# Urist-McDeveloper/nbody

Measured on AMD Instinct MI355X. Metric: particle-pair interactions/sec at N=2^20, higher is better.
Workload: dtype f32

## Files before the change

nbody_amd/__init__.py:

```python
import ctypes as C
import os

import numpy as np

PKG_DIR = os.path.dirname(os.path.abspath(__file__))
ROOT = os.path.dirname(PKG_DIR)
LIB_DIR = os.path.join(PKG_DIR, "lib")
HIP_SO = os.environ.get("NBODY_HIP_SO") or os.path.join(LIB_DIR, "libnbody_hip.so")
NBODY_SO = os.path.join(LIB_DIR, "libnbody.so")



def _nb_g_from_header():
    import re
    with open(os.path.join(ROOT, "include", "nbody.h")) as f:
        return float(re.search(r"^#define\s+NB_G\s+([0-9.eE+-]+)f?\s*$", f.read(), re.M).group(1))


NB_G = _nb_g_from_header()
UNIQUE_ID_BYTES = 128
CLOCK_SAMPLER_MAX_MS = 20000.0


class WorldData(C.Structure):
    _fields_ = [("total_len", C.c_uint32), ("mass_len", C.c_uint32), ("dt", C.c_float)]


class WorldEnergy(C.Structure):
    _fields_ = [("kinetic", C.c_double), ("potential", C.c_double), ("mass", C.c_double), ("momentum", C.c_double * 2),
                ("angular_momentum", C.c_double), ("center_of_mass", C.c_double * 2)]

    def as_dict(self):
        return {"kinetic": self.kinetic, "potential": self.potential, "total": self.kinetic + self.potential,
                "mass": self.mass, "momentum": (self.momentum[0], self.momentum[1]),
                "angular_momentum": self.angular_momentum,
                "center_of_mass": (self.center_of_mass[0], self.center_of_mass[1])}


def energy_row(row):
    e = WorldEnergy()
    C.memmove(C.byref(e), np.ascontiguousarray(row, dtype=np.float64).ctypes.data, C.sizeof(WorldEnergy))
    return e.as_dict()


def trace_rows(n, every):
    return int(hip_lib().nb_hip_ensemble_trace_rows(int(n), int(every)))


class RenderView(C.Structure):
    _fields_ = [("target", C.c_float * 2), ("offset", C.c_float * 2), ("zoom", C.c_float), ("width", C.c_uint32),
                ("height", C.c_uint32), ("core_mass", C.c_float)]

    @classmethod
    def make(cls, target, offset, zoom, width, height, core_mass):
        return cls((C.c_float * 2)(*target), (C.c_float * 2)(*offset), zoom, width, height, core_mass)

    def as_dict(self):
        return {"target": (self.target[0], self.target[1]), "offset": (self.offset[0], self.offset[1]), "zoom": self.zoom,
                "width": self.width, "height": self.height, "core_mass": self.core_mass}


class RenderPalette(C.Structure):
    _fields_ = [("background", C.c_uint8 * 4), ("color", (C.c_uint8 * 4) * 3), ("saturation", C.c_uint32)]

    @classmethod
    def make(cls, background, color, saturation):
        return cls((C.c_uint8 * 4)(*background), ((C.c_uint8 * 4) * 3)(*[(C.c_uint8 * 4)(*c) for c in color]), saturation)


def default_palette():
    p = RenderPalette()
    nbody_lib().DefaultRenderPalette(C.byref(p))
    return p


class NbAdaptive(C.Structure):
    _fields_ = [("eta", C.c_float), ("dt_min", C.c_float), ("dt_max", C.c_float), ("flags", C.c_uint32), ("span", C.c_double),
                ("chunk", C.c_uint32), ("reserved", C.c_uint32)]


class NbAdaptiveResult(C.Structure):
    _fields_ = [("elapsed", C.c_double), ("steps", C.c_uint32), ("idle_steps", C.c_uint32), ("dt_last", C.c_float),
                ("dt_smallest", C.c_float)]

    def as_dict(self):
        return {"elapsed": self.elapsed, "steps": int(self.steps), "idle_steps": int(self.idle_steps), "dt_last": self.dt_last,
                "dt_smallest": self.dt_smallest}


NB_ADAPT_PRIME = 1
NB_ADAPT_CONTINUE = 2
NB_ADAPT_LEAPFROG = 4


def adaptive_cfg(eta, dt_max, dt_min=0.0, span=float("inf"), prime=False, chunk=0, resume=False, leapfrog=False):
    flags = (NB_ADAPT_PRIME if prime else 0) | (NB_ADAPT_CONTINUE if resume else 0) | (NB_ADAPT_LEAPFROG if leapfrog else 0)
    return NbAdaptive(float(eta), float(dt_min), float(dt_max), flags, float(span), int(chunk), 0)


class NbShardPlan(C.Structure):
    _fields_ = [(n, C.c_uint32) for n in ("mass_chunk", "zero_chunk", "mass_begin", "mass_count",
                                          "zero_begin", "zero_count", "src_padded")]


ALLGATHER_FN = C.CFUNCTYPE(None, C.c_void_p, C.c_void_p, C.c_uint64, C.c_int, C.c_int)

HIP_API = {
    "CreateSimPipeline": (C.c_void_p, [WorldData]),
    "DestroySimPipeline": (None, [C.c_void_p]),
    "GetSimulationData": (None, [C.c_void_p, C.c_void_p]),
    "SetSimulationData": (None, [C.c_void_p, C.c_void_p]),
    "PerformSimUpdate": (None, [C.c_void_p, C.c_uint32, C.c_float]),
    "nb_hip_device_count": (C.c_int, []),
    "nb_hip_set_device": (None, [C.c_int]),
    "nb_hip_device_info": (None, [C.c_char_p, C.c_uint32]),
    "nb_hip_step_async": (None, [C.c_void_p, C.c_uint32, C.c_float]),
    "nb_hip_sync": (None, [C.c_void_p]),
    "nb_hip_last_step_ms": (C.c_double, [C.c_void_p, C.POINTER(C.c_uint32)]),
    "nb_hip_last_finish_launches": (C.c_uint32, [C.c_void_p]),
    "nb_hip_last_step_breakdown": (C.c_uint32, [C.c_void_p, C.POINTER(C.c_double), C.POINTER(C.c_double)]),
    "nb_hip_comm_info": (C.c_int, [C.c_void_p, C.POINTER(C.c_int), C.POINTER(C.c_int), C.POINTER(C.c_int),
                                   C.POINTER(C.c_int), C.POINTER(C.c_double), C.c_char_p, C.c_uint32]),
    "nb_hip_comm_bringup": (C.c_int, [C.c_void_p, C.POINTER(C.c_double), C.POINTER(C.c_double), C.POINTER(C.c_double)]),
    "nb_hip_preflight_peers": (C.c_int, [C.POINTER(C.c_int), C.c_int]),
    "nb_hip_preflight_ipc_export": (C.c_int, [C.c_void_p, C.c_uint32]),
    "nb_hip_preflight_ipc_open": (C.c_int, [C.c_void_p, C.c_uint32, C.POINTER(C.c_double)]),
    "nb_hip_preflight_ipc_release": (None, []),
    "nb_hip_error_string": (C.c_char_p, [C.c_int]),
    "nb_hip_graph_stats": (C.c_uint32, [C.c_void_p, C.POINTER(C.c_uint32)]),
    "nb_hip_runtime_version": (C.c_int, []),
    "nb_hip_probe_clock": (C.c_int, [C.c_double] + [C.POINTER(C.c_double)] * 5),
    "nb_hip_clock_sampler_begin": (C.c_int, [C.c_double, C.c_double]),
    "nb_hip_clock_sampler_end": (C.c_int, [C.POINTER(C.c_double)] * 6 + [C.POINTER(C.c_uint32)]),
    "nb_hip_note_host_array": (None, [C.c_void_p, C.c_void_p, C.c_uint64]),
    "nb_hip_configure": (C.c_int, [C.c_void_p, C.c_char_p, C.c_int]),
    "nb_hip_launch_shape": (None, [C.c_void_p, C.POINTER(C.c_int), C.POINTER(C.c_int), C.POINTER(C.c_int),
                                   C.POINTER(C.c_int), C.POINTER(C.c_uint32)]),
    "nb_hip_plan_launch": (None, [C.c_uint32, C.c_uint32, C.c_int, C.POINTER(C.c_int), C.POINTER(C.c_int),
                                  C.POINTER(C.c_int), C.POINTER(C.c_uint32)]),
    "nb_hip_comm_unique_id": (None, [C.c_void_p]),
    "CreateSimPipelineSharded": (C.c_void_p, [WorldData, C.c_int, C.c_int, C.c_void_p]),
    "CreateSimPipelineShardedWith": (C.c_void_p, [WorldData, C.c_int, C.c_int, ALLGATHER_FN, C.c_void_p]),
    "CreateSimPipelineShardedDirect": (C.c_void_p, [WorldData, C.c_int, C.c_int, ALLGATHER_FN, C.c_void_p]),
    "nb_hip_shard_plan": (NbShardPlan, [C.c_uint32, C.c_uint32, C.c_int, C.c_int]),
    "nb_hip_local_group_create": (C.c_int, [WorldData, C.c_int, C.POINTER(C.c_void_p)]),
    "nb_hip_local_group_step": (None, [C.POINTER(C.c_void_p), C.c_int, C.c_uint32, C.c_float]),
    "nb_hip_energy": (None, [C.c_void_p, C.POINTER(WorldEnergy)]),
    "nb_hip_potential": (None, [C.c_void_p, C.c_void_p]),
    "nb_hip_bounds": (None, [C.c_void_p, C.c_void_p]),
    "nb_hip_render_counts": (None, [C.c_void_p, C.POINTER(RenderView), C.c_void_p]),
    "nb_hip_render_rgba": (None, [C.c_void_p, C.POINTER(RenderView), C.POINTER(RenderPalette), C.c_void_p]),
    "nb_hip_potential_at": (None, [C.c_void_p, C.c_void_p, C.c_uint32, C.c_float, C.c_void_p]),
    "nb_hip_potential_map": (None, [C.c_void_p, C.POINTER(RenderView), C.c_float, C.c_void_p]),
    "nb_hip_acceleration_at": (None, [C.c_void_p, C.c_void_p, C.c_uint32, C.c_float, C.c_void_p]),
    "nb_hip_acceleration_map": (None, [C.c_void_p, C.POINTER(RenderView), C.c_float, C.c_void_p]),
    "nb_hip_batch_create": (C.c_void_p, [C.c_uint32, C.c_uint32, C.POINTER(C.c_uint32)]),
    "nb_hip_batch_destroy": (None, [C.c_void_p]),
    "nb_hip_batch_set_data": (None, [C.c_void_p, C.c_void_p]),
    "nb_hip_batch_get_data": (None, [C.c_void_p, C.c_void_p]),
    "nb_hip_batch_get_member": (None, [C.c_void_p, C.c_uint32, C.c_void_p]),
    "nb_hip_batch_update": (None, [C.c_void_p, C.c_uint32, C.c_float]),
    "nb_hip_batch_update_dts": (None, [C.c_void_p, C.c_uint32, C.POINTER(C.c_float)]),
    "nb_hip_batch_step_async": (None, [C.c_void_p, C.c_uint32, C.POINTER(C.c_float)]),
    "nb_hip_batch_sync": (None, [C.c_void_p]),
    "nb_hip_batch_last_ms": (C.c_double, [C.c_void_p]),
    "nb_hip_batch_dt_uploads": (C.c_uint32, [C.c_void_p]),
    "nb_hip_batch_launch_shape": (None, [C.c_void_p, C.POINTER(C.c_int), C.POINTER(C.c_int), C.POINTER(C.c_int),
                                         C.POINTER(C.c_int), C.POINTER(C.c_uint32)]),
    "nb_hip_ensemble_energy": (None, [C.c_void_p, C.POINTER(WorldEnergy)]),
    "nb_hip_ensemble_potential": (None, [C.c_void_p, C.c_void_p]),
    "nb_hip_ensemble_trace_rows": (C.c_uint32, [C.c_uint32, C.c_uint32]),
    "nb_hip_ensemble_trace": (None, [C.c_void_p, C.c_uint32, C.c_float, C.c_uint32, C.c_void_p]),
    "nb_hip_ensemble_trace_dts": (None, [C.c_void_p, C.c_uint32, C.POINTER(C.c_float), C.c_uint32, C.c_void_p]),
    "nb_hip_ensemble_bounds": (None, [C.c_void_p, C.c_void_p]),
    "nb_hip_ensemble_render_counts": (None, [C.c_void_p, C.POINTER(RenderView), C.c_void_p]),
    "nb_hip_ensemble_render_rgba": (None, [C.c_void_p, C.POINTER(RenderView), C.POINTER(RenderPalette), C.c_void_p]),
    "nb_hip_ragged_create": (C.c_void_p, [C.c_uint32, C.POINTER(C.c_uint32), C.POINTER(C.c_uint32)]),
    "nb_hip_ragged_layout": (None, [C.c_void_p, C.POINTER(C.c_uint32), C.POINTER(C.c_uint64)]),
    "nb_hip_ragged_launch_shape": (C.c_uint32, [C.c_void_p, C.c_uint32, C.POINTER(C.c_int), C.POINTER(C.c_int), C.POINTER(C.c_int),
                                                C.POINTER(C.c_int), C.POINTER(C.c_uint32), C.POINTER(C.c_uint32)]),
    "nb_hip_ragged_member_shape": (None, [C.c_void_p, C.c_uint32, C.POINTER(C.c_uint32), C.POINTER(C.c_int), C.POINTER(C.c_int),
                                          C.POINTER(C.c_int)]),
    "nb_hip_ensemble_potential_at": (None, [C.c_void_p, C.c_void_p, C.c_uint32, C.c_float, C.c_void_p]),
    "nb_hip_ensemble_potential_map": (None, [C.c_void_p, C.POINTER(RenderView), C.c_float, C.c_void_p]),
    "nb_hip_ensemble_acceleration_at": (None, [C.c_void_p, C.c_void_p, C.c_uint32, C.c_float, C.c_void_p]),
    "nb_hip_ensemble_acceleration_map": (None, [C.c_void_p, C.POINTER(RenderView), C.c_float, C.c_void_p]),
    "nb_hip_adaptive_steps": (None, [C.c_void_p, C.c_uint32, C.POINTER(NbAdaptive), C.c_void_p, C.POINTER(NbAdaptiveResult)]),
    "nb_hip_adaptive_steps_async": (None, [C.c_void_p, C.c_uint32, C.POINTER(NbAdaptive)]),
    "nb_hip_adaptive_collect": (None, [C.c_void_p, C.c_void_p, C.POINTER(NbAdaptiveResult)]),
    "nb_hip_timestep": (None, [C.c_void_p, C.POINTER(NbAdaptive), C.POINTER(C.c_float)]),
    "nb_hip_ensemble_adaptive_steps": (None, [C.c_void_p, C.c_uint32, C.POINTER(NbAdaptive), C.c_void_p, C.c_void_p]),
    "nb_hip_leapfrog_steps": (None, [C.c_void_p, C.c_uint32, C.c_float]),
    "nb_hip_leapfrog_steps_async": (None, [C.c_void_p, C.c_uint32, C.c_float]),
    "nb_hip_ensemble_leapfrog": (None, [C.c_void_p, C.c_uint32, C.c_float]),
    "nb_hip_ensemble_leapfrog_dts": (None, [C.c_void_p, C.c_uint32, C.POINTER(C.c_float)]),
    "nb_hip_version": (C.c_int, []),
}

TUNE_API = {
    "nb_hip_tune": (C.c_int, [C.c_void_p, C.c_char_p, C.c_int]),
    "nb_hip_tuning_build": (C.c_int, []),
    "nb_hip_launch_unit": (C.c_int, [C.c_void_p]),
    "nb_hip_last_fused_steps": (C.c_uint32, [C.c_void_p]),
    "nb_hip_launch_lanes": (C.c_int, [C.c_void_p]),
    "nb_hip_plan_launch_unit": (C.c_int, [C.c_uint32, C.c_uint32, C.c_int]),
    "nb_hip_plan_fused_finish": (C.c_int, [C.c_uint32, C.c_uint32, C.c_int]),
    "nb_hip_plan_launch_lanes": (C.c_int, [C.c_uint32, C.c_uint32, C.POINTER(C.c_int)]),
    "nb_hip_last_diag_ms": (C.c_double, [C.c_void_p]),
    "nb_hip_last_render_ms": (C.c_double, [C.c_void_p, C.POINTER(C.c_double)]),
    "nb_hip_ensemble_last_diag_ms": (C.c_double, [C.c_void_p]),
    "nb_hip_ensemble_trace_mode": (None, [C.c_void_p, C.c_int]),
    "nb_hip_ensemble_last_trace_info": (None, [C.c_void_p, C.POINTER(C.c_int), C.POINTER(C.c_uint32)]),
    "nb_hip_ensemble_render_mode": (None, [C.c_void_p, C.c_int]),
    "nb_hip_ensemble_last_render_info": (None, [C.c_void_p, C.POINTER(C.c_int), C.POINTER(C.c_uint32)]),
    "nb_hip_ensemble_last_render_ms": (C.c_double, [C.c_void_p]),
    "nb_hip_last_leapfrog_info": (None, [C.c_void_p, C.POINTER(C.c_uint32), C.POINTER(C.c_int)]),
    "nb_hip_ensemble_last_leapfrog_info": (None, [C.c_void_p, C.POINTER(C.c_uint32), C.POINTER(C.c_int)]),
    "nb_hip_live_resources": (None, [C.POINTER(C.c_uint32), C.POINTER(C.c_uint32)]),
}
PUBLIC_KNOBS = ("variant", "graph", "timing", "overlap", "sharded_graph")

NBODY_API = {
    "CreateWorld": (C.c_void_p, [C.c_void_p, C.c_uint32]),
    "DestroyWorld": (None, [C.c_void_p]),
    "GetWorldParticles": (C.c_void_p, [C.c_void_p, C.POINTER(C.c_uint32)]),
    "UpdateWorld_CPU": (None, [C.c_void_p, C.c_float, C.c_uint32]),
    "UpdateWorld_GPU": (None, [C.c_void_p, C.c_float, C.c_uint32]),
    "CreateWorldSharded": (C.c_void_p, [C.c_void_p, C.c_uint32, C.c_int, C.c_int, C.c_void_p]),
    "CreateWorldShardedWith": (C.c_void_p, [C.c_void_p, C.c_uint32, C.c_int, C.c_int, ALLGATHER_FN, C.c_void_p]),
    "CreateWorldShardedDirect": (C.c_void_p, [C.c_void_p, C.c_uint32, C.c_int, C.c_int, ALLGATHER_FN, C.c_void_p]),
    "GetWorldPipeline": (C.c_void_p, [C.c_void_p]),
    "MakeGalaxies": (C.c_void_p, [C.c_uint32, C.c_uint32]),
    "MakeGalaxiesSeeded": (C.c_void_p, [C.c_uint32, C.c_uint32, C.c_uint64]),
    "GetWorldEnergy": (None, [C.c_void_p, C.POINTER(WorldEnergy)]),
    "GetWorldPotential": (None, [C.c_void_p, C.c_void_p]),
    "DefaultRenderPalette": (None, [C.POINTER(RenderPalette)]),
    "GetWorldBounds": (None, [C.c_void_p, C.c_void_p]),
    "FitWorldView": (None, [C.c_void_p, C.c_uint32, C.c_uint32, C.POINTER(RenderView)]),
    "RenderWorldCounts": (None, [C.c_void_p, C.POINTER(RenderView), C.c_void_p]),
    "RenderWorld": (None, [C.c_void_p, C.POINTER(RenderView), C.POINTER(RenderPalette), C.c_void_p]),
    "GetWorldPotentialAt": (None, [C.c_void_p, C.c_void_p, C.c_uint32, C.c_float, C.c_void_p]),
    "RenderWorldPotential": (None, [C.c_void_p, C.POINTER(RenderView), C.c_float, C.c_void_p]),
    "GetWorldAccelerationAt": (None, [C.c_void_p, C.c_void_p, C.c_uint32, C.c_float, C.c_void_p]),
    "RenderWorldAcceleration": (None, [C.c_void_p, C.POINTER(RenderView), C.c_float, C.c_void_p]),
    "CreateWorldBatch": (C.c_void_p, [C.c_void_p, C.c_uint32, C.c_uint32]),
    "DestroyWorldBatch": (None, [C.c_void_p]),
    "GetWorldBatchParticles": (C.c_void_p, [C.c_void_p, C.c_uint32, C.POINTER(C.c_uint32)]),
    "UpdateWorldBatch_GPU": (None, [C.c_void_p, C.c_float, C.c_uint32]),
    "UpdateWorldBatch_GPU_dts": (None, [C.c_void_p, C.POINTER(C.c_float), C.c_uint32]),
    "GetWorldBatchEnergy": (None, [C.c_void_p, C.POINTER(WorldEnergy)]),
    "GetWorldBatchPotential": (None, [C.c_void_p, C.c_void_p]),
    "UpdateWorldBatch_GPU_Traced": (None, [C.c_void_p, C.c_float, C.c_uint32, C.c_uint32, C.c_void_p]),
    "UpdateWorldBatch_GPU_Traced_dts": (None, [C.c_void_p, C.POINTER(C.c_float), C.c_uint32, C.c_uint32, C.c_void_p]),
    "GetWorldBatchBounds": (None, [C.c_void_p, C.c_void_p]),
    "FitWorldBatchViews": (None, [C.c_void_p, C.c_uint32, C.c_uint32, C.POINTER(RenderView)]),
    "RenderWorldBatchCounts": (None, [C.c_void_p, C.POINTER(RenderView), C.c_void_p]),
    "RenderWorldBatch": (None, [C.c_void_p, C.POINTER(RenderView), C.POINTER(RenderPalette), C.c_void_p]),
    "CreateWorldBatchRagged": (C.c_void_p, [C.c_void_p, C.POINTER(C.c_uint32), C.c_uint32]),
    "GetWorldBatchPotentialAt": (None, [C.c_void_p, C.c_void_p, C.c_uint32, C.c_float, C.c_void_p]),
    "RenderWorldBatchPotential": (None, [C.c_void_p, C.POINTER(RenderView), C.c_float, C.c_void_p]),
    "GetWorldBatchAccelerationAt": (None, [C.c_void_p, C.c_void_p, C.c_uint32, C.c_float, C.c_void_p]),
    "RenderWorldBatchAcceleration": (None, [C.c_void_p, C.POINTER(RenderView), C.c_float, C.c_void_p]),
    "UpdateWorld_GPU_Adaptive": (None, [C.c_void_p, C.c_uint32, C.POINTER(NbAdaptive), C.c_void_p, C.POINTER(NbAdaptiveResult)]),
    "UpdateWorld_CPU_Adaptive": (None, [C.c_void_p, C.c_uint32, C.POINTER(NbAdaptive), C.c_void_p, C.POINTER(NbAdaptiveResult)]),
    "GetWorldTimestep": (None, [C.c_void_p, C.POINTER(NbAdaptive), C.POINTER(C.c_float)]),
    "AdvanceWorld_GPU": (None, [C.c_void_p, C.c_double, C.POINTER(NbAdaptive), C.c_uint32, C.c_void_p, C.POINTER(NbAdaptiveResult)]),
    "UpdateWorldBatch_GPU_Adaptive": (None, [C.c_void_p, C.c_uint32, C.POINTER(NbAdaptive), C.c_void_p, C.c_void_p]),
    "AdvanceWorldBatch_GPU": (None, [C.c_void_p, C.c_double, C.POINTER(NbAdaptive), C.c_uint32, C.c_void_p, C.c_void_p]),
    "UpdateWorld_GPU_Leapfrog": (None, [C.c_void_p, C.c_float, C.c_uint32]),
    "UpdateWorld_CPU_Leapfrog": (None, [C.c_void_p, C.c_float, C.c_uint32]),
    "UpdateWorldBatch_GPU_Leapfrog": (None, [C.c_void_p, C.c_float, C.c_uint32]),
    "UpdateWorldBatch_GPU_Leapfrog_dts": (None, [C.c_void_p, C.POINTER(C.c_float), C.c_uint32]),
}

_hip = None
_nbody = None


def _bind(lib, api):
    for name, (res, args) in api.items():
        f = getattr(lib, name)
        f.restype = res
        f.argtypes = args
    return lib


def _build_if_missing(path):
    if os.path.exists(path) or os.environ.get("NBODY_HIP_SO"):
        return
    import sys
    from . import build as _build
    print(f"[nbody_amd] {path} missing: building the product libraries (hipcc, gfx950)", file=sys.stderr, flush=True)
    _build.build_product()


def hip_lib():
    global _hip
    if _hip is None:
        _build_if_missing(HIP_SO)
        if not os.path.exists(HIP_SO):
            raise OSError(f"{HIP_SO} not built: run `python -c 'import __graft_entry__ as g; g.build()'`")
        _hip = _bind(_bind(C.CDLL(HIP_SO, mode=C.RTLD_GLOBAL), HIP_API), TUNE_API)
    return _hip


def nbody_lib():
    global _nbody
    if _nbody is None:
        hip_lib()
        _build_if_missing(NBODY_SO)
        if not os.path.exists(NBODY_SO):
            raise OSError(f"{NBODY_SO} not built: run `python -c 'import __graft_entry__ as g; g.build()'`")
        _nbody = _bind(C.CDLL(NBODY_SO, mode=C.RTLD_GLOBAL), NBODY_API)
    return _nbody


def as_particles(a):
    a = np.ascontiguousarray(a, dtype=np.float32)
    if a.ndim != 2 or a.shape[1] != 8:
        raise ValueError("particles must have shape (n, 8)")
    return a


def as_points(points):
    a = np.ascontiguousarray(points, dtype=np.float32)
    if a.ndim != 2 or a.shape[1] != 2:
        raise ValueError("points must have shape (n, 2)")
    return a


def device_count():
    return int(hip_lib().nb_hip_device_count())


def live_resources():
    buffers, events = C.c_uint32(0), C.c_uint32(0)
    hip_lib().nb_hip_live_resources(C.byref(buffers), C.byref(events))
    return int(buffers.value), int(events.value)


def device_info():
    buf = C.create_string_buffer(256)
    hip_lib().nb_hip_device_info(buf, 256)
    return buf.value.decode()


def probe_clock(target_ms=40.0):
    v = [C.c_double(0.0) for _ in range(5)]
    waves = hip_lib().nb_hip_probe_clock(float(target_ms), *[C.byref(x) for x in v])
    return {"clock_ghz": v[0].value, "clock_ghz_min": v[1].value, "clock_ghz_max": v[2].value,
            "cycles_per_wave_interaction": v[3].value, "elapsed_ms": v[4].value, "waves": int(waves)}


def clock_sampler_begin(period_ms=0.5, max_ms=6000.0):
    return int(hip_lib().nb_hip_clock_sampler_begin(float(period_ms), float(max_ms)))


def clock_sampler_end():
    ghz, lo, hi, span = C.c_double(), C.c_double(), C.c_double(), C.c_double()
    per_xcd, profile = (C.c_double * 8)(), (C.c_double * 10)()
    dropped = C.c_uint32(0)
    n = hip_lib().nb_hip_clock_sampler_end(C.byref(ghz), C.byref(lo), C.byref(hi), per_xcd, profile, C.byref(span), C.byref(dropped))
    return {"clock_ghz": ghz.value, "clock_ghz_min": lo.value, "clock_ghz_max": hi.value, "per_xcd_ghz": [float(v) for v in per_xcd],
            "profile_ghz": [float(v) for v in profile], "span_ms": span.value, "intervals": int(n), "dropped_intervals": int(dropped.value)}


def preflight_peers(max_devices=16):
    row = (C.c_int * max_devices)()
    count = int(hip_lib().nb_hip_preflight_peers(row, max_devices))
    return count, [int(v) for v in row[:min(count, max_devices)]]


def preflight_ipc_export(tag):
    buf = (C.c_ubyte * 64)()
    rc = int(hip_lib().nb_hip_preflight_ipc_export(buf, int(tag) & 0xffffffff))
    return rc, bytes(buf)


def preflight_ipc_open(handle, expect_tag):
    ms = C.c_double(0.0)
    buf = (C.c_ubyte * 64).from_buffer_copy(handle)
    rc = int(hip_lib().nb_hip_preflight_ipc_open(buf, int(expect_tag) & 0xffffffff, C.byref(ms)))
    return rc, float(ms.value)


def hip_error_string(code):
    return hip_lib().nb_hip_error_string(int(code)).decode(errors="replace")


def shard_plan(total_len, mass_len, rank, nranks):
    p = hip_lib().nb_hip_shard_plan(total_len, mass_len, rank, nranks)
    return {n: int(getattr(p, n)) for n, _ in NbShardPlan._fields_}


def plan_launch(n_recv, n_src, compute_units=256):
    k, w, sp, g, lw = C.c_int(), C.c_int(), C.c_int(), C.c_uint32(), C.c_int()
    hip_lib().nb_hip_plan_launch(n_recv, n_src, compute_units, C.byref(k), C.byref(w), C.byref(sp), C.byref(g))
    lanes = int(hip_lib().nb_hip_plan_launch_lanes(n_recv, n_src, C.byref(lw)))
    return {"k": k.value, "w": w.value, "split": sp.value, "workgroups": g.value,
            "unit": int(hip_lib().nb_hip_plan_launch_unit(n_recv, n_src, compute_units)), "lanes": lanes, "lanes_w": lw.value,
            "fused_finish": int(hip_lib().nb_hip_plan_fused_finish(n_recv, n_src, compute_units))}


def comm_unique_id():
    buf = (C.c_ubyte * UNIQUE_ID_BYTES)()
    hip_lib().nb_hip_comm_unique_id(buf)
    return bytes(buf)


class SimPipeline:

    def __init__(self, total_len, mass_len, rank=0, nranks=1, unique_id=None, allgather=None, direct=False):
        L = hip_lib()
        wd = WorldData(total_len, mass_len, 0.0)
        self._cb = None
        if allgather is not None:
            def thunk(_ctx, buf, bytes_per_rank, r, n):
                try:
                    rows = np.ctypeslib.as_array(C.cast(buf, C.POINTER(C.c_uint8)), shape=(n, int(bytes_per_rank)))
                    allgather(rows, r, n)
                except BaseException:
                    import sys
                    import traceback
                    traceback.print_exc()
                    print(f"[nbody_amd] rank {r} of {n}: the caller-supplied all-gather raised; exiting (5)", file=sys.stderr,
                          flush=True)
                    os._exit(5)
            self._cb = ALLGATHER_FN(thunk)
            create = L.CreateSimPipelineShardedDirect if direct else L.CreateSimPipelineShardedWith
            self._h = create(wd, rank, nranks, self._cb, None)
        elif nranks > 1 or unique_id is not None:
            idbuf = (C.c_ubyte * UNIQUE_ID_BYTES).from_buffer_copy(unique_id)
            self._h = L.CreateSimPipelineSharded(wd, rank, nranks, idbuf)
        else:
            self._h = L.CreateSimPipeline(wd)
        self.total_len, self.mass_len = total_len, mass_len
        self.rank, self.nranks = rank, nranks
        self.configure(timing=1)

    def close(self):
        if self._h:
            hip_lib().DestroySimPipeline(self._h)
            self._h = None

    def __del__(self):
        try:
            self.close()
        except Exception:
            pass

    def set_data(self, particles):
        a = as_particles(particles)
        assert a.shape[0] == self.total_len
        hip_lib().SetSimulationData(self._h, a.ctypes.data)

    def get_data(self):
        out = np.empty((self.total_len, 8), dtype=np.float32)
        hip_lib().GetSimulationData(self._h, out.ctypes.data)
        return out

    def update(self, n, dt):
        hip_lib().PerformSimUpdate(self._h, n, dt)

    def step_async(self, n, dt):
        hip_lib().nb_hip_step_async(self._h, n, dt)

    def update_leapfrog(self, n, dt):
        hip_lib().nb_hip_leapfrog_steps(self._h, n, dt)

    def update_leapfrog_async(self, n, dt):
        hip_lib().nb_hip_leapfrog_steps_async(self._h, n, dt)

    def last_leapfrog_info(self):
        k, primed = C.c_uint32(0), C.c_int(0)
        hip_lib().nb_hip_last_leapfrog_info(self._h, C.byref(k), C.byref(primed))
        return int(k.value), bool(primed.value)

    def update_adaptive(self, n, eta, dt_max, dt_min=0.0, span=float("inf"), prime=False, resume=False, leapfrog=False):
        cfg, res, log = adaptive_cfg(eta, dt_max, dt_min, span, prime, resume=resume, leapfrog=leapfrog), NbAdaptiveResult(), np.zeros(n, dtype=np.float32)
        hip_lib().nb_hip_adaptive_steps(self._h, n, C.byref(cfg), log.ctypes.data, C.byref(res))
        return log, res.as_dict()

    def update_adaptive_async(self, n, eta, dt_max, dt_min=0.0, span=float("inf"), prime=False, resume=False, leapfrog=False):
        cfg = adaptive_cfg(eta, dt_max, dt_min, span, prime, resume=resume, leapfrog=leapfrog)
        hip_lib().nb_hip_adaptive_steps_async(self._h, n, C.byref(cfg))

    def adaptive_collect(self, n):
        res, log = NbAdaptiveResult(), np.zeros(n, dtype=np.float32)
        hip_lib().nb_hip_adaptive_collect(self._h, log.ctypes.data, C.byref(res))
        return log, res.as_dict()

    def timestep(self, eta, dt_max, dt_min=0.0):
        cfg, dt = adaptive_cfg(eta, dt_max, dt_min), C.c_float(0.0)
        hip_lib().nb_hip_timestep(self._h, C.byref(cfg), C.byref(dt))
        return float(dt.value)

    def sync(self):
        hip_lib().nb_hip_sync(self._h)

    def last_step_ms(self):
        launches = C.c_uint32(0)
        ms = hip_lib().nb_hip_last_step_ms(self._h, C.byref(launches))
        return float(ms), int(launches.value)

    def finish_launches(self):
        return int(hip_lib().nb_hip_last_finish_launches(self._h))

    def step_breakdown(self):
        k, c = C.c_double(0.0), C.c_double(0.0)
        steps = hip_lib().nb_hip_last_step_breakdown(self._h, C.byref(k), C.byref(c))
        return int(steps), float(k.value), float(c.value)

    def comm_info(self):
        n, r, d, v, ms = C.c_int(), C.c_int(), C.c_int(), C.c_int(), C.c_double()
        path = C.create_string_buffer(256)
        own = hip_lib().nb_hip_comm_info(self._h, C.byref(n), C.byref(r), C.byref(d), C.byref(v), C.byref(ms), path, 256)
        return {"owns_comm": bool(own), "nranks": n.value, "rank": r.value, "device": d.value, "rccl_version": v.value,
                "first_gather_ms": ms.value, "rccl_lib": path.value.decode()}

    def comm_bringup(self):
        a, b, c = C.c_double(), C.c_double(), C.c_double()
        own = hip_lib().nb_hip_comm_bringup(self._h, C.byref(a), C.byref(b), C.byref(c))
        return {"owns_comm": bool(own), "comm_init_ms": a.value, "first_gather_ms": b.value, "small_gather_us": c.value}

    def graph_stats(self):
        uploads = C.c_uint32(0)
        cached = hip_lib().nb_hip_graph_stats(self._h, C.byref(uploads))
        return {"cached": int(cached), "dt_uploads": int(uploads.value)}

    def energy(self):
        e = WorldEnergy()
        hip_lib().nb_hip_energy(self._h, C.byref(e))
        return e.as_dict()

    def potential(self):
        out = np.empty(self.total_len, dtype=np.float32)
        hip_lib().nb_hip_potential(self._h, out.ctypes.data)
        return out

    def potential_at(self, points, softening):
        pts = as_points(points)
        out = np.empty(pts.shape[0], dtype=np.float32)
        hip_lib().nb_hip_potential_at(self._h, pts.ctypes.data, pts.shape[0], softening, out.ctypes.data)
        return out

    def potential_map(self, view, softening):
        out = np.empty((view.height, view.width), dtype=np.float32)
        hip_lib().nb_hip_potential_map(self._h, C.byref(view), softening, out.ctypes.data)
        return out

    def acceleration_at(self, points, softening):
        pts = as_points(points)
        out = np.empty((pts.shape[0], 2), dtype=np.float32)
        hip_lib().nb_hip_acceleration_at(self._h, pts.ctypes.data, pts.shape[0], softening, out.ctypes.data)
        return out

    def acceleration_map(self, view, softening):
        out = np.empty((view.height, view.width, 2), dtype=np.float32)
        hip_lib().nb_hip_acceleration_map(self._h, C.byref(view), softening, out.ctypes.data)
        return out

    def last_diag_ms(self):
        return float(hip_lib().nb_hip_last_diag_ms(self._h))

    def bounds(self):
        out = np.empty(4, dtype=np.float32)
        hip_lib().nb_hip_bounds(self._h, out.ctypes.data)
        return out

    def render_counts(self, view):
        out = np.empty((3, view.height, view.width), dtype=np.uint32)
        hip_lib().nb_hip_render_counts(self._h, C.byref(view), out.ctypes.data)
        return out

    def render(self, view, palette=None):
        out = np.empty((view.height, view.width, 4), dtype=np.uint8)
        pal = palette if palette is not None else default_palette()
        hip_lib().nb_hip_render_rgba(self._h, C.byref(view), C.byref(pal), out.ctypes.data)
        return out

    def last_render_ms(self):
        parts = (C.c_double * 4)()
        total = hip_lib().nb_hip_last_render_ms(self._h, parts)
        return float(total), [float(v) for v in parts]

    def fused_steps(self):
        return int(hip_lib().nb_hip_last_fused_steps(self._h))

    def configure(self, **knobs):
        for k, v in knobs.items():
            fn = hip_lib().nb_hip_configure if k in PUBLIC_KNOBS else hip_lib().nb_hip_tune
            fn(self._h, k.encode(), int(v))

    def launch_shape(self):
        k, w, v, sp, g = C.c_int(), C.c_int(), C.c_int(), C.c_int(), C.c_uint32()
        hip_lib().nb_hip_launch_shape(self._h, C.byref(k), C.byref(w), C.byref(v), C.byref(sp), C.byref(g))
        return {"k": k.value, "w": w.value, "variant": "smem" if v.value else "lds", "split": sp.value,
                "workgroups": g.value, "unit": int(hip_lib().nb_hip_launch_unit(self._h)),
                "lanes": int(hip_lib().nb_hip_launch_lanes(self._h))}


def as_ensemble(a):
    a = np.ascontiguousarray(a, dtype=np.float32)
    if a.ndim != 3 or a.shape[2] != 8:
        raise ValueError("an ensemble must have shape (members, n, 8)")
    return a


def _packed(members):
    parts = [as_particles(m) for m in members]
    sizes = np.array([p.shape[0] for p in parts], dtype=np.uint32)
    flat = np.concatenate(parts, axis=0) if parts else np.zeros((0, 8), np.float32)
    return np.ascontiguousarray(flat, dtype=np.float32), sizes


def _unpacked(flat, offsets):
    return [flat[int(offsets[b]):int(offsets[b + 1])].copy() for b in range(len(offsets) - 1)]


def _dt_array(dts, count):
    a = np.ascontiguousarray(dts, dtype=np.float32)
    if a.shape != (count,):
        raise ValueError(f"expected {count} step sizes")
    return a


def _member_points(points, count):
    a = np.asarray(points, dtype=np.float32)
    if a.ndim == 2:
        a = np.broadcast_to(a, (count,) + a.shape)
    if a.ndim != 3 or a.shape[0] != count or a.shape[2] != 2:
        raise ValueError(f"points must have shape (n, 2) or ({count}, n, 2)")
    return np.ascontiguousarray(a)


def _ensemble_field(fn, handle, count, components, softening, points=None, views=None):
    tail = (2,) if components == 2 else ()
    if points is not None:
        pts = _member_points(points, count)
        out = np.empty((count, pts.shape[1]) + tail, dtype=np.float32)
        fn(handle, pts.ctypes.data, pts.shape[1], softening, out.ctypes.data)
        return out
    arr, w, h = _view_array(views, count)
    out = np.empty((count, h, w) + tail, dtype=np.float32)
    fn(handle, arr, softening, out.ctypes.data)
    return out


def _view_array(views, count):
    if isinstance(views, RenderView):
        views = [views] * count
    views = list(views)
    if len(views) != count:
        raise ValueError(f"expected one RenderView or {count} of them")
    arr = (RenderView * count)()
    for b, v in enumerate(views):
        C.memmove(C.byref(arr[b]), C.byref(v), C.sizeof(RenderView))
    return arr, int(arr[0].width), int(arr[0].height)


def contact_sheet(frames, columns):
    frames = np.asarray(frames)
    if frames.ndim != 4 or columns < 1:
        raise ValueError("frames must have shape (B, h, w, channels) and columns must be at least 1")
    count, h, w, ch = frames.shape
    rows = -(-count // columns)
    sheet = np.zeros((rows * columns, h, w, ch), dtype=frames.dtype)
    sheet[:count] = frames
    return sheet.reshape(rows, columns, h, w, ch).transpose(0, 2, 1, 3, 4).reshape(rows * h, columns * w, ch)


class SimBatch:

    is_ragged = False

    def __init__(self, total_len, mass_len):
        m = np.ascontiguousarray(mass_len, dtype=np.uint32)
        if m.ndim != 1:
            raise ValueError("mass_len must be a sequence with one entry per member")
        self.count, self.total_len, self.mass_len = int(m.shape[0]), int(total_len), m.copy()
        self._h = hip_lib().nb_hip_batch_create(self.count, self.total_len, m.ctypes.data_as(C.POINTER(C.c_uint32)))

    @classmethod
    def ragged(cls, total_lens, mass_lens):
        n = np.ascontiguousarray(total_lens, dtype=np.uint32)
        m = np.ascontiguousarray(mass_lens, dtype=np.uint32)
        if n.ndim != 1 or m.shape != n.shape:
            raise ValueError("total_lens and mass_lens must be sequences with one entry per member")
        self = cls.__new__(cls)
        self.is_ragged = True
        self.count, self.total_lens, self.mass_len = int(n.shape[0]), n.copy(), m.copy()
        self.total_len = int(n.max()) if n.size else 0
        self._h = hip_lib().nb_hip_ragged_create(self.count, n.ctypes.data_as(C.POINTER(C.c_uint32)),
                                                 m.ctypes.data_as(C.POINTER(C.c_uint32)))
        self.offsets = self.layout()[1]
        return self

    def layout(self):
        sizes, offsets = np.empty(self.count, np.uint32), np.empty(self.count + 1, np.uint64)
        hip_lib().nb_hip_ragged_layout(self._h, sizes.ctypes.data_as(C.POINTER(C.c_uint32)), offsets.ctypes.data_as(C.POINTER(C.c_uint64)))
        return sizes, offsets

    def sizes(self):
        return [int(x) for x in self.layout()[0]]

    def close(self):
        if self._h:
            hip_lib().nb_hip_batch_destroy(self._h)
            self._h = None

    def __del__(self):
        try:
            self.close()
        except Exception:
            pass

    def set_data(self, particles):
        if self.is_ragged:
            flat, sizes = _packed(particles)
            assert np.array_equal(sizes, self.total_lens)
            hip_lib().nb_hip_batch_set_data(self._h, flat.ctypes.data)
            return
        a = as_ensemble(particles)
        assert a.shape[:2] == (self.count, self.total_len)
        hip_lib().nb_hip_batch_set_data(self._h, a.ctypes.data)

    def get_data(self):
        if self.is_ragged:
            flat = np.empty((int(self.offsets[-1]), 8), dtype=np.float32)
            hip_lib().nb_hip_batch_get_data(self._h, flat.ctypes.data)
            return _unpacked(flat, self.offsets)
        out = np.empty((self.count, self.total_len, 8), dtype=np.float32)
        hip_lib().nb_hip_batch_get_data(self._h, out.ctypes.data)
        return out

    def get_member(self, b):
        n = int(self.total_lens[b]) if self.is_ragged and 0 <= int(b) < self.count else self.total_len
        out = np.empty((n, 8), dtype=np.float32)
        hip_lib().nb_hip_batch_get_member(self._h, int(b), out.ctypes.data)
        return out

    def update(self, n, dt):
        if np.ndim(dt) == 0:
            hip_lib().nb_hip_batch_update(self._h, n, float(dt))
        else:
            hip_lib().nb_hip_batch_update_dts(self._h, n, _dt_array(dt, self.count).ctypes.data_as(C.POINTER(C.c_float)))

    def step_async(self, n, dts):
        hip_lib().nb_hip_batch_step_async(self._h, n, _dt_array(dts, self.count).ctypes.data_as(C.POINTER(C.c_float)))

    def update_leapfrog(self, n, dt):
        if np.ndim(dt) == 0:
            hip_lib().nb_hip_ensemble_leapfrog(self._h, n, float(dt))
        else:
            hip_lib().nb_hip_ensemble_leapfrog_dts(self._h, n, _dt_array(dt, self.count).ctypes.data_as(C.POINTER(C.c_float)))

    def last_leapfrog_info(self):
        k, primed = C.c_uint32(0), C.c_int(0)
        hip_lib().nb_hip_ensemble_last_leapfrog_info(self._h, C.byref(k), C.byref(primed))
        return int(k.value), bool(primed.value)

    def update_adaptive(self, n, eta, dt_max, dt_min=0.0, span=float("inf"), prime=False, resume=False, leapfrog=False):
        cfg, res = adaptive_cfg(eta, dt_max, dt_min, span, prime, resume=resume, leapfrog=leapfrog), (NbAdaptiveResult * self.count)()
        log = np.zeros((n, self.count), dtype=np.float32)
        hip_lib().nb_hip_ensemble_adaptive_steps(self._h, n, C.byref(cfg), log.ctypes.data, C.byref(res))
        return log, [r.as_dict() for r in res]

    def sync(self):
        hip_lib().nb_hip_batch_sync(self._h)

    def last_ms(self):
        return float(hip_lib().nb_hip_batch_last_ms(self._h))

    def dt_uploads(self):
        return int(hip_lib().nb_hip_batch_dt_uploads(self._h))

    def trace(self, n, dt, every):
        out = np.empty((trace_rows(n, every), self.count, 8), dtype=np.float64)
        if np.ndim(dt) == 0:
            hip_lib().nb_hip_ensemble_trace(self._h, n, float(dt), every, out.ctypes.data)
        else:
            hip_lib().nb_hip_ensemble_trace_dts(self._h, n, _dt_array(dt, self.count).ctypes.data_as(C.POINTER(C.c_float)), every,
                                             out.ctypes.data)
        return out

    def trace_mode(self, mode):
        hip_lib().nb_hip_ensemble_trace_mode(self._h, int(mode))

    def last_trace_info(self):
        fused, launches = C.c_int(0), C.c_uint32(0)
        hip_lib().nb_hip_ensemble_last_trace_info(self._h, C.byref(fused), C.byref(launches))
        return {"fused": fused.value, "launches": launches.value}

    def energy(self):
        out = (WorldEnergy * self.count)()
        hip_lib().nb_hip_ensemble_energy(self._h, out)
        return [e.as_dict() for e in out]

    def potential(self):
        if self.is_ragged:
            flat = np.empty(int(self.offsets[-1]), dtype=np.float32)
            hip_lib().nb_hip_ensemble_potential(self._h, flat.ctypes.data)
            return _unpacked(flat, self.offsets)
        out = np.empty((self.count, self.total_len), dtype=np.float32)
        hip_lib().nb_hip_ensemble_potential(self._h, out.ctypes.data)
        return out

    def potential_at(self, points, softening):
        return _ensemble_field(hip_lib().nb_hip_ensemble_potential_at, self._h, self.count, 1, softening, points=points)

    def potential_map(self, views, softening):
        return _ensemble_field(hip_lib().nb_hip_ensemble_potential_map, self._h, self.count, 1, softening, views=views)

    def acceleration_at(self, points, softening):
        return _ensemble_field(hip_lib().nb_hip_ensemble_acceleration_at, self._h, self.count, 2, softening, points=points)

    def acceleration_map(self, views, softening):
        return _ensemble_field(hip_lib().nb_hip_ensemble_acceleration_map, self._h, self.count, 2, softening, views=views)

    def last_diag_ms(self):
        return float(hip_lib().nb_hip_ensemble_last_diag_ms(self._h))

    def bounds(self):
        out = np.empty((self.count, 4), dtype=np.float32)
        hip_lib().nb_hip_ensemble_bounds(self._h, out.ctypes.data)
        return out

    def render_counts(self, views):
        arr, w, h = _view_array(views, self.count)
        out = np.empty((self.count, 3, h, w), dtype=np.uint32)
        hip_lib().nb_hip_ensemble_render_counts(self._h, arr, out.ctypes.data)
        return out

    def render(self, views, palette=None):
        arr, w, h = _view_array(views, self.count)
        out = np.empty((self.count, h, w, 4), dtype=np.uint8)
        pal = palette if palette is not None else default_palette()
        hip_lib().nb_hip_ensemble_render_rgba(self._h, arr, C.byref(pal), out.ctypes.data)
        return out

    def render_mode(self, mode):
        hip_lib().nb_hip_ensemble_render_mode(self._h, int(mode))

    def last_render_info(self):
        tile, launches = C.c_int(0), C.c_uint32(0)
        hip_lib().nb_hip_ensemble_last_render_info(self._h, C.byref(tile), C.byref(launches))
        return {"tile_path": tile.value, "launches": launches.value}

    def last_render_ms(self):
        return float(hip_lib().nb_hip_ensemble_last_render_ms(self._h))

    def launch_shape(self):
        path, k, w, lanes, g = C.c_int(), C.c_int(), C.c_int(), C.c_int(), C.c_uint32()
        if self.is_ragged:
            groups, i, total = [], 0, 1
            members = C.c_uint32()
            while i < total:
                total = int(hip_lib().nb_hip_ragged_launch_shape(self._h, i, C.byref(path), C.byref(k), C.byref(w), C.byref(lanes),
                                                                 C.byref(members), C.byref(g)))
                groups.append({"path": "lanes" if path.value else "chain", "k": k.value, "w": w.value, "lanes": lanes.value,
                               "members": members.value, "workgroups": g.value})
                i += 1
            per = []
            grp = C.c_uint32()
            for b in range(self.count):
                hip_lib().nb_hip_ragged_member_shape(self._h, b, C.byref(grp), C.byref(k), C.byref(w), C.byref(lanes))
                per.append((grp.value, k.value, w.value, lanes.value))
            return {"groups": groups, "members": per}
        hip_lib().nb_hip_batch_launch_shape(self._h, C.byref(path), C.byref(k), C.byref(w), C.byref(lanes), C.byref(g))
        return {"path": "lanes" if path.value else "chain", "k": k.value, "w": w.value, "lanes": lanes.value,
                "workgroups": g.value}

    def pinned_knobs(self):
        s = self.launch_shape()
        if s["path"] == "chain":
            return dict(k=s["k"], w=s["w"], split=1, unit=8, fused_chain=0)
        return dict(lanes=s["lanes"], w=s["w"], fused_chain=0)


class WorldBatch:

    is_ragged = False

    def __init__(self, particles):
        a = as_ensemble(particles)
        self.count, self.size = int(a.shape[0]), int(a.shape[1])
        self._h = nbody_lib().CreateWorldBatch(a.ctypes.data, self.size, self.count)

    @classmethod
    def ragged(cls, members):
        flat, sizes = _packed(members)
        self = cls.__new__(cls)
        self.is_ragged = True
        self.count, self._sizes = int(sizes.shape[0]), sizes
        self.size = int(sizes.max()) if sizes.size else 0
        self.offsets = np.concatenate([[0], np.cumsum(sizes, dtype=np.uint64)]).astype(np.uint64)
        self._h = nbody_lib().CreateWorldBatchRagged(flat.ctypes.data, sizes.ctypes.data_as(C.POINTER(C.c_uint32)), self.count)
        return self

    def sizes(self):
        return [int(x) for x in self._sizes] if self.is_ragged else [self.size] * self.count

    def close(self):
        if self._h:
            nbody_lib().DestroyWorldBatch(self._h)
            self._h = None

    def __del__(self):
        try:
            self.close()
        except Exception:
            pass

    def member(self, b):
        n = C.c_uint32(0)
        p = nbody_lib().GetWorldBatchParticles(self._h, int(b), C.byref(n))
        return np.ctypeslib.as_array(C.cast(p, C.POINTER(C.c_float)), shape=(n.value, 8)).copy()

    def particles(self):
        if self.is_ragged:
            return [self.member(b) for b in range(self.count)]
        return np.stack([self.member(b) for b in range(self.count)])

    def update_gpu(self, dt, n):
        if np.ndim(dt) == 0:
            nbody_lib().UpdateWorldBatch_GPU(self._h, float(dt), n)
        else:
            nbody_lib().UpdateWorldBatch_GPU_dts(self._h, _dt_array(dt, self.count).ctypes.data_as(C.POINTER(C.c_float)), n)

    def update_gpu_leapfrog(self, dt, n):
        if np.ndim(dt) == 0:
            nbody_lib().UpdateWorldBatch_GPU_Leapfrog(self._h, float(dt), n)
        else:
            nbody_lib().UpdateWorldBatch_GPU_Leapfrog_dts(self._h, _dt_array(dt, self.count).ctypes.data_as(C.POINTER(C.c_float)), n)

    def update_gpu_adaptive(self, n, eta, dt_max, dt_min=0.0, span=float("inf"), prime=False, leapfrog=False):
        cfg, res = adaptive_cfg(eta, dt_max, dt_min, span, prime, leapfrog=leapfrog), (NbAdaptiveResult * self.count)()
        log = np.zeros((n, self.count), dtype=np.float32)
        nbody_lib().UpdateWorldBatch_GPU_Adaptive(self._h, n, C.byref(cfg), log.ctypes.data, C.byref(res))
        return log, [r.as_dict() for r in res]

    def advance_gpu(self, span, eta, dt_max, dt_min=0.0, prime=False, chunk=0, max_steps=4096, leapfrog=False):
        cfg, res = adaptive_cfg(eta, dt_max, dt_min, prime=prime, chunk=chunk, leapfrog=leapfrog), (NbAdaptiveResult * self.count)()
        log = np.zeros((max_steps, self.count), dtype=np.float32)
        nbody_lib().AdvanceWorldBatch_GPU(self._h, float(span), C.byref(cfg), max_steps, log.ctypes.data, C.byref(res))
        made = max((r.steps + r.idle_steps for r in res), default=0)
        return log[:made].copy(), [r.as_dict() for r in res]

    def update_gpu_traced(self, dt, n, every):
        out = np.empty((trace_rows(n, every), self.count, 8), dtype=np.float64)
        if np.ndim(dt) == 0:
            nbody_lib().UpdateWorldBatch_GPU_Traced(self._h, float(dt), n, every, out.ctypes.data)
        else:
            nbody_lib().UpdateWorldBatch_GPU_Traced_dts(self._h, _dt_array(dt, self.count).ctypes.data_as(C.POINTER(C.c_float)), n,
                                                        every, out.ctypes.data)
        return out

    def energy(self):
        out = (WorldEnergy * self.count)()
        nbody_lib().GetWorldBatchEnergy(self._h, out)
        return [e.as_dict() for e in out]

    def potential(self):
        if self.is_ragged:
            flat = np.empty(int(self.offsets[-1]), dtype=np.float32)
            nbody_lib().GetWorldBatchPotential(self._h, flat.ctypes.data)
            return _unpacked(flat, self.offsets)
        out = np.empty((self.count, self.size), dtype=np.float32)
        nbody_lib().GetWorldBatchPotential(self._h, out.ctypes.data)
        return out

    def potential_at(self, points, softening):
        return _ensemble_field(nbody_lib().GetWorldBatchPotentialAt, self._h, self.count, 1, softening, points=points)

    def potential_map(self, views, softening):
        return _ensemble_field(nbody_lib().RenderWorldBatchPotential, self._h, self.count, 1, softening, views=views)

    def acceleration_at(self, points, softening):
        return _ensemble_field(nbody_lib().GetWorldBatchAccelerationAt, self._h, self.count, 2, softening, points=points)

    def acceleration_map(self, views, softening):
        return _ensemble_field(nbody_lib().RenderWorldBatchAcceleration, self._h, self.count, 2, softening, views=views)

    def bounds(self):
        out = np.empty((self.count, 4), dtype=np.float32)
        nbody_lib().GetWorldBatchBounds(self._h, out.ctypes.data)
        return out

    def fit_views(self, width, height):
        arr = (RenderView * self.count)()
        nbody_lib().FitWorldBatchViews(self._h, width, height, arr)
        return [RenderView.from_buffer_copy(v) for v in arr]

    def render_counts(self, views):
        arr, w, h = _view_array(views, self.count)
        out = np.empty((self.count, 3, h, w), dtype=np.uint32)
        nbody_lib().RenderWorldBatchCounts(self._h, arr, out.ctypes.data)
        return out

    def render(self, views, palette=None):
        arr, w, h = _view_array(views, self.count)
        out = np.empty((self.count, h, w, 4), dtype=np.uint8)
        nbody_lib().RenderWorldBatch(self._h, arr, C.byref(palette) if palette is not None else None, out.ctypes.data)
        return out


class LocalShardGroup:

    def __init__(self, total_len, mass_len, nranks, **knobs):
        L = hip_lib()
        self.nranks = nranks
        self._arr = (C.c_void_p * nranks)()
        L.nb_hip_local_group_create(WorldData(total_len, mass_len, 0.0), nranks, self._arr)
        self.members = []
        for r in range(nranks):
            m = SimPipeline.__new__(SimPipeline)
            m._h = self._arr[r]
            m.total_len, m.mass_len, m.rank, m.nranks = total_len, mass_len, r, nranks
            m.configure(timing=1, **knobs)
            self.members.append(m)

    def set_data(self, particles):
        for m in self.members:
            m.set_data(particles)

    def step(self, n, dt):
        hip_lib().nb_hip_local_group_step(self._arr, self.nranks, n, dt)

    def get_data(self, rank=0):
        return self.members[rank].get_data()

    def close(self):
        for m in self.members:
            m.close()
        self.members = []


class World:

    def __init__(self, particles, rank=None, nranks=1, unique_id=None):
        a = as_particles(particles)
        self.size = a.shape[0]
        if rank is None:
            self._h = nbody_lib().CreateWorld(a.ctypes.data, self.size)
        else:
            idbuf = (C.c_ubyte * UNIQUE_ID_BYTES).from_buffer_copy(unique_id) if unique_id is not None else None
            self._h = nbody_lib().CreateWorldSharded(a.ctypes.data, self.size, rank, nranks, idbuf)

    def close(self):
        if self._h:
            nbody_lib().DestroyWorld(self._h)
            self._h = None

    def __del__(self):
        try:
            self.close()
        except Exception:
            pass

    def particles(self):
        n = C.c_uint32(0)
        p = nbody_lib().GetWorldParticles(self._h, C.byref(n))
        if n.value == 0:
            return np.empty((0, 8), dtype=np.float32)
        return np.ctypeslib.as_array(C.cast(p, C.POINTER(C.c_float)), shape=(n.value, 8)).copy()

    def pipeline(self):
        return nbody_lib().GetWorldPipeline(self._h)

    def tune(self, **knobs):
        old = {}
        for k, v in knobs.items():
            fn = hip_lib().nb_hip_configure if k in PUBLIC_KNOBS else hip_lib().nb_hip_tune
            old[k] = int(fn(self.pipeline(), k.encode(), int(v)))
        return old

    def update_cpu(self, dt, n):
        nbody_lib().UpdateWorld_CPU(self._h, dt, n)

    def update_gpu(self, dt, n):
        nbody_lib().UpdateWorld_GPU(self._h, dt, n)

    def _adaptive(self, fn, n, cfg):
        res, log = NbAdaptiveResult(), np.zeros(n, dtype=np.float32)
        fn(self._h, n, C.byref(cfg), log.ctypes.data, C.byref(res))
        return log, res.as_dict()

    def update_gpu_leapfrog(self, dt, n):
        nbody_lib().UpdateWorld_GPU_Leapfrog(self._h, dt, n)

    def update_cpu_leapfrog(self, dt, n):
        nbody_lib().UpdateWorld_CPU_Leapfrog(self._h, dt, n)

    def update_gpu_adaptive(self, n, eta, dt_max, dt_min=0.0, span=float("inf"), prime=False, leapfrog=False):
        return self._adaptive(nbody_lib().UpdateWorld_GPU_Adaptive, n, adaptive_cfg(eta, dt_max, dt_min, span, prime, leapfrog=leapfrog))

    def update_cpu_adaptive(self, n, eta, dt_max, dt_min=0.0, span=float("inf"), prime=False, leapfrog=False):
        return self._adaptive(nbody_lib().UpdateWorld_CPU_Adaptive, n, adaptive_cfg(eta, dt_max, dt_min, span, prime, leapfrog=leapfrog))

    def timestep(self, eta, dt_max, dt_min=0.0):
        cfg, dt = adaptive_cfg(eta, dt_max, dt_min), C.c_float(0.0)
        nbody_lib().GetWorldTimestep(self._h, C.byref(cfg), C.byref(dt))
        return float(dt.value)

    def advance_gpu(self, span, eta, dt_max, dt_min=0.0, prime=False, chunk=0, max_steps=4096, leapfrog=False):
        cfg, res = adaptive_cfg(eta, dt_max, dt_min, prime=prime, chunk=chunk, leapfrog=leapfrog), NbAdaptiveResult()
        log = np.zeros(max_steps, dtype=np.float32)
        nbody_lib().AdvanceWorld_GPU(self._h, float(span), C.byref(cfg), max_steps, log.ctypes.data, C.byref(res))
        return log[:res.steps + res.idle_steps].copy(), res.as_dict()

    def energy(self):
        e = WorldEnergy()
        nbody_lib().GetWorldEnergy(self._h, C.byref(e))
        return e.as_dict()

    def potential(self):
        out = np.empty(self.size, dtype=np.float32)
        nbody_lib().GetWorldPotential(self._h, out.ctypes.data)
        return out

    def potential_at(self, points, softening):
        pts = as_points(points)
        out = np.empty(pts.shape[0], dtype=np.float32)
        nbody_lib().GetWorldPotentialAt(self._h, pts.ctypes.data, pts.shape[0], softening, out.ctypes.data)
        return out

    def potential_map(self, view, softening):
        out = np.empty((view.height, view.width), dtype=np.float32)
        nbody_lib().RenderWorldPotential(self._h, C.byref(view), softening, out.ctypes.data)
        return out

    def acceleration_at(self, points, softening):
        pts = as_points(points)
        out = np.empty((pts.shape[0], 2), dtype=np.float32)
        nbody_lib().GetWorldAccelerationAt(self._h, pts.ctypes.data, pts.shape[0], softening, out.ctypes.data)
        return out

    def acceleration_map(self, view, softening):
        out = np.empty((view.height, view.width, 2), dtype=np.float32)
        nbody_lib().RenderWorldAcceleration(self._h, C.byref(view), softening, out.ctypes.data)
        return out

    def bounds(self):
        out = np.empty(4, dtype=np.float32)
        nbody_lib().GetWorldBounds(self._h, out.ctypes.data)
        return out

    def fit_view(self, width, height):
        v = RenderView()
        nbody_lib().FitWorldView(self._h, width, height, C.byref(v))
        return v

    def render_counts(self, view):
        out = np.empty((3, view.height, view.width), dtype=np.uint32)
        nbody_lib().RenderWorldCounts(self._h, C.byref(view), out.ctypes.data)
        return out

    def render(self, view, palette=None):
        out = np.empty((view.height, view.width, 4), dtype=np.uint8)
        nbody_lib().RenderWorld(self._h, C.byref(view), C.byref(palette) if palette is not None else None, out.ctypes.data)
        return out


_cpu_best = None


def cpu_best_lib():
    global _cpu_best
    if _cpu_best is None:
        path = os.path.join(LIB_DIR, "libnbody_cpu_best.so")
        _build_if_missing(path)
        lib = C.CDLL(path)
        lib.nb_cpu_variant_count.restype = C.c_int
        lib.nb_cpu_variant_name.restype = C.c_char_p
        lib.nb_cpu_variant_name.argtypes = [C.c_int, C.POINTER(C.c_int), C.POINTER(C.c_char_p)]
        lib.nb_cpu_variant_update.restype = C.c_int
        lib.nb_cpu_variant_update.argtypes = [C.c_char_p, C.c_void_p, C.c_uint32, C.c_uint32, C.c_float, C.c_uint32]
        _cpu_best = lib
    return _cpu_best


def cpu_variants():
    lib, out = cpu_best_lib(), []
    for i in range(lib.nb_cpu_variant_count()):
        ok, what = C.c_int(0), C.c_char_p()
        name = lib.nb_cpu_variant_name(i, C.byref(ok), C.byref(what))
        out.append((name.decode(), bool(ok.value), what.value.decode()))
    return out


def cpu_variant_update(isa, particles, mass_len, dt, n=1):
    a = as_particles(particles).copy()
    if cpu_best_lib().nb_cpu_variant_update(isa.encode(), a.ctypes.data, a.shape[0], mass_len, dt, n) != 0:
        raise RuntimeError(f"CPU variant {isa!r} is unknown or not supported by this CPU")
    return a


def make_galaxies(particle_count, galaxy_count, seed=None, own_rng=False):
    L = nbody_lib()
    libc = C.CDLL(None)
    libc.free.argtypes = [C.c_void_p]
    if own_rng:
        p = L.MakeGalaxiesSeeded(particle_count, galaxy_count, int(seed))
    else:
        if seed is not None:
            libc.srand(C.c_uint(seed))
        p = L.MakeGalaxies(particle_count, galaxy_count)
    a = np.ctypeslib.as_array(C.cast(p, C.POINTER(C.c_float)), shape=(particle_count, 8)).copy()
    libc.free(p)
    return a
```

nbody_amd/csrc/kernels.h:

```cpp
#pragma once

#include <hip/hip_runtime.h>
#include <stdint.h>

namespace nb {

enum : uint32_t {
    STEP_ACC_IN = 1u,
    STEP_NO_FINALIZE = 2u,
};

enum : int {
    VARIANT_LDS = 0,
    VARIANT_SMEM = 1,
};

struct StepParams {
    const float2 *src_pos;
    const float *src_gm;
    uint32_t src_begin[2];
    uint32_t src_end[2];
    const float2 *pos_in;
    float2 *pos_out;
    float2 *vel;
    float2 *acc;
    const float *radius;
    uint32_t n_recv;
    uint32_t recv_split;
    uint32_t recv_gap;
    float2 *mirror;
    uint32_t n_mirror;
    const float *dt;
    uint32_t flags;
    float2 *parts;
    uint32_t split;
    uint32_t *tickets;
    uint32_t unit;
};

__host__ __device__ inline StepParams plain_step(const float2 *src_pos, const float *src_gm, uint32_t n_src, const float2 *pos_in,
                                                 float2 *pos_out, float2 *vel, float2 *acc, const float *radius, uint32_t n_recv,
                                                 const float *dt, uint32_t unit) {
    return StepParams{.src_pos = src_pos, .src_gm = src_gm, .src_begin = {0, 0}, .src_end = {n_src, 0}, .pos_in = pos_in,
                      .pos_out = pos_out, .vel = vel, .acc = acc, .radius = radius, .n_recv = n_recv, .recv_split = n_recv,
                      .dt = dt, .split = 1, .unit = unit};
}

struct ChainParams {
    float2 *pos;
    float2 *vel;
    float2 *acc;
    const float *radius;
    const float *src_gm;
    uint32_t n_recv;
    uint32_t n_src;
    uint32_t steps;
    uint32_t tiles;
    const float *dt;
};

constexpr uint32_t CHAIN_K = 2;
constexpr uint32_t CHAIN_MAX_RECV = 512;

struct BatchParams {
    float2 *pos_in;
    float2 *pos_out;
    float2 *vel;
    float2 *acc;
    const float *radius;
    const float *gm;
    const uint32_t *mass_len;
    const float *dt;
    uint32_t n_recv;
    uint32_t stride;
    uint32_t steps;
    uint32_t tiles;
};

struct RaggedParams : BatchParams {
    const uint32_t *n_len;
    const uint32_t *members;
};

struct TraceParams {
    const float *mass;
    double *rows;
    uint32_t count;
    uint32_t every;
    uint32_t done;
};

constexpr int MAX_SPLIT = 16;

struct LaunchShape;

const void *step_kernel_fn(LaunchShape s);
const void *step_kernel_fused_fn(LaunchShape s);
const void *finish_kernel_fn();

void launch_chain(hipStream_t st, const ChainParams &p);

const void *batch_lane_split_fn(int w, int lanes, bool listed);
void launch_batch_chain(hipStream_t st, const RaggedParams &p, uint32_t workgroups);
void launch_batch_trace_chain(hipStream_t st, const RaggedParams &p, const TraceParams &t, uint32_t workgroups);

}
```

nbody_amd/csrc/kernels.hip:

```cpp
#include "kernels.h"
#include "diag_common.h"
#include "interaction_asm.h"
#include "launch_shape.h"

#include <hip/hip_runtime.h>

#include <type_traits>

namespace nb {
namespace {

constexpr int WAVE = 64;
constexpr int CHUNK = 64;
constexpr int CLOSE_EVERY = 4;

typedef float v16f __attribute__((ext_vector_type(16)));
typedef float v8f __attribute__((ext_vector_type(8)));
typedef float v4f __attribute__((ext_vector_type(4)));

typedef float f2v __attribute__((ext_vector_type(2)));

template <int K>
struct Receivers {
    f2v p[K];
    float r[K];
    f2v a[K];
    f2v s[K];
    f2v c[K];
    __device__ __forceinline__ void clear() {
#pragma unroll
        for (int k = 0; k < K; k++) a[k] = s[k] = c[k] = f2v{0.0f, 0.0f};
    }
    __device__ __forceinline__ void close_chunk() {
#pragma unroll
        for (int k = 0; k < K; k++) {
            const f2v y = a[k] - c[k];
            const f2v t = s[k] + y;
            const f2v cn = (t - s[k]) - y;
            const bool lx = a[k].x != 0.0f, ly = a[k].y != 0.0f;
            const bool fx = __builtin_fabsf(t.x) < __builtin_inff(), fy = __builtin_fabsf(t.y) < __builtin_inff();
            c[k].x = lx ? (fx ? cn.x : 0.0f) : c[k].x;
            c[k].y = ly ? (fy ? cn.y : 0.0f) : c[k].y;
            s[k].x = lx ? t.x : s[k].x;
            s[k].y = ly ? t.y : s[k].y;
            a[k] = f2v{0.0f, 0.0f};
        }
    }
};


#define NB_INTERACT2(SRC)                                                                                                       \
    asm(NB_INTERACTION2_ASM                                                                                                     \
        : [ax0] "+v"(R.a[0].x), [ay0] "+v"(R.a[0].y), [ax1] "+v"(R.a[1].x), [ay1] "+v"(R.a[1].y)                                \
        : [sx] SRC(sxy.x), [sy] SRC(sxy.y), [g] SRC(sg), [px0] "v"(R.p[0].x), [py0] "v"(R.p[0].y), [r0] "v"(R.r[0]),            \
          [px1] "v"(R.p[1].x), [py1] "v"(R.p[1].y), [r1] "v"(R.r[1])                                                            \
        : NB_CLOBBERS2)
#define NB_INTERACT1(SRC)                                                                                                       \
    asm(NB_INTERACTION_ASM                                                                                                      \
        : [ax] "+v"(R.a[k].x), [ay] "+v"(R.a[k].y)                                                                              \
        : [sx] SRC(sxy.x), [sy] SRC(sxy.y), [g] SRC(sg), [px] "v"(R.p[k].x), [py] "v"(R.p[k].y), [r] "v"(R.r[k])                \
        : NB_CLOBBERS)
template <int K, bool SRC_IN_SGPR>
__device__ __forceinline__ void interact(Receivers<K> &R, f2v sxy, float sg) {
    if constexpr (K == 2) {
        if constexpr (SRC_IN_SGPR) NB_INTERACT2("s");
        else NB_INTERACT2("v");
        return;
    }
#pragma unroll
    for (int k = 0; k < K; k++) {
        if constexpr (SRC_IN_SGPR) NB_INTERACT1("s");
        else NB_INTERACT1("v");
    }
}
#undef NB_INTERACT2
#undef NB_INTERACT1

#ifndef NB_INTERACT8_OVERRIDE
template <int K, bool SRC_IN_SGPR, typename VP, typename VG>
__device__ __forceinline__ void interact8(Receivers<K> &R, const VP &P, const VG &G) {
#pragma unroll
    for (int u = 0; u < 8; u++) interact<K, SRC_IN_SGPR>(R, f2v{P[2 * u], P[2 * u + 1]}, G[u]);
}
#else
NB_INTERACT8_OVERRIDE
#endif

template <typename V>
__device__ __forceinline__ V src_load(const float *ptr) {
    return *reinterpret_cast<const V *>(ptr);
}

__device__ __forceinline__ uint32_t receiver_slot(const StepParams &p, uint32_t i) {
    return i + (i >= p.recv_split ? p.recv_gap : 0u);
}

__device__ __forceinline__ uint32_t source_index(const StepParams &p, uint32_t v, uint32_t n0) {
    return v < n0 ? p.src_begin[0] + v : p.src_begin[1] + (v - n0);
}


__device__ __forceinline__ float2 add_rn(float2 a, float2 b) { return make_float2(__fadd_rn(a.x, b.x), __fadd_rn(a.y, b.y)); }

__device__ __forceinline__ void integrate(float2 a, float dt, float2 &v, float2 &q) {
    v.x = __fadd_rn(v.x, __fmul_rn(a.x, dt));
    v.y = __fadd_rn(v.y, __fmul_rn(a.y, dt));
    q.x = __fadd_rn(q.x, __fmul_rn(v.x, dt));
    q.y = __fadd_rn(q.y, __fmul_rn(v.y, dt));
}

__device__ __forceinline__ void store_moved(const StepParams &p, uint32_t i, float2 v, float2 q) {
    p.vel[i] = v;
    p.pos_out[i] = q;
    if (i < p.n_mirror) p.mirror[i] = q;
}

__device__ __forceinline__ void finish_loaded(const StepParams &p, uint32_t i, float2 a, float2 a0, float2 v, float2 q, float dt) {
    if (p.flags & STEP_ACC_IN) a = add_rn(a0, a);
    p.acc[i] = a;
    if (p.flags & STEP_NO_FINALIZE) return;
    integrate(a, dt, v, q);
    store_moved(p, i, v, q);
}

__device__ __forceinline__ void add_part(float &sx, float &sy, float2 part, bool live) {
    const float nx = __fadd_rn(sx, part.x), ny = __fadd_rn(sy, part.y);
    sx = live ? nx : sx;
    sy = live ? ny : sy;
}

__device__ __forceinline__ float2 wave_sum(const float2 *first, uint32_t stride, uint32_t n) {
    float sx = 0.0f, sy = 0.0f;
    for (uint32_t s = 0; s < n; s++) {
        const float2 t = first[s * stride];
        sx = __fadd_rn(sx, t.x);
        sy = __fadd_rn(sy, t.y);
    }
    return make_float2(sx, sy);
}

struct SourceSlice {
    uint32_t lo, hi;
};
__device__ __forceinline__ SourceSlice source_slice(uint32_t total, uint32_t unit, uint32_t parts, uint32_t part, uint32_t n,
                                                    uint32_t i) {
    const uint32_t nunits = (total + unit - 1) / unit;
    const uint32_t per_part = (nunits + parts - 1) / parts;
    const uint32_t part_lo = min(part * per_part, nunits);
    const uint32_t part_hi = min(part_lo + per_part, nunits);
    const uint32_t per = (part_hi - part_lo + n - 1) / n;
    const uint32_t u_lo = min(part_lo + i * per, part_hi);
    const uint32_t u_hi = min(u_lo + per, part_hi);
    const uint32_t lo = u_lo * unit;
    return {lo, max(min(u_hi * unit, total), lo)};
}

__device__ __forceinline__ void finish_receiver(const StepParams &p, uint32_t logical, float sx, float sy, float dt) {
    if (logical >= p.n_recv) return;
    const uint32_t i = receiver_slot(p, logical);
    float2 a = make_float2(sx, sy);
    if (p.flags & STEP_ACC_IN) a = add_rn(p.acc[i], a);
    p.acc[i] = a;
    if (p.flags & STEP_NO_FINALIZE) return;
    float2 v = p.vel[i], q = p.pos_in[i];
    integrate(a, dt, v, q);
    store_moved(p, i, v, q);
}

__global__ __launch_bounds__(256) void finish_kernel(const StepParams p) {
    const uint32_t logical = blockIdx.x * blockDim.x + threadIdx.x;
    if (logical >= p.n_recv) return;
    const uint32_t i = receiver_slot(p, logical);
    float2 part[MAX_SPLIT];
#pragma unroll
    for (uint32_t s = 0; s < (uint32_t)MAX_SPLIT; s++)
        part[s] = p.parts[(size_t)(s < p.split ? s : p.split - 1) * p.n_recv + logical];
    const float2 a0 = p.acc[i];
    const float2 v0 = p.vel[i];
    const float2 q0 = p.pos_in[i];
    const float dt = *p.dt;
    float sx = 0.0f, sy = 0.0f;
#pragma unroll
    for (uint32_t s = 0; s < (uint32_t)MAX_SPLIT; s++) add_part(sx, sy, part[s], s < p.split);
    finish_loaded(p, i, make_float2(sx, sy), a0, v0, q0, dt);
}

template <int K, int W, int VARIANT, bool FUSED = false>
__global__ __launch_bounds__(WAVE *W, 8) void step_kernel(const StepParams p) {
    const uint32_t tid = threadIdx.x;
    const uint32_t lane = tid & (WAVE - 1);
    const uint32_t wid = __builtin_amdgcn_readfirstlane(tid >> 6);
    const uint32_t tile_x = blockIdx.x, part_y = blockIdx.y;

    __shared__ __attribute__((aligned(16))) float tile[VARIANT == VARIANT_LDS ? W : 1][2][3 * CHUNK];
    __shared__ float2 partial[W > 1 ? W : 1][W > 1 ? WAVE * K : 1];

    const float dt = *p.dt;

    const uint32_t recv_base = tile_x * (WAVE * K);
    Receivers<K> R;
#pragma unroll
    for (int k = 0; k < K; k++) {
        uint32_t i = recv_base + k * WAVE + lane;
        i = i < p.n_recv ? i : p.n_recv - 1;
        i = receiver_slot(p, i);
        const float2 q = p.pos_in[i];
        R.p[k] = f2v{q.x, q.y};
        R.r[k] = p.radius[i];
    }
    R.clear();

    const uint32_t n0 = p.src_end[0] - p.src_begin[0];
    const uint32_t n1 = p.src_end[1] - p.src_begin[1];
    const uint32_t total = n0 + n1;
    const SourceSlice wave_src = source_slice(total, p.unit, p.split, part_y, W, wid);
    const uint32_t v_lo = wave_src.lo;
    const uint32_t v_hi = wave_src.hi;

    if constexpr (VARIANT == VARIANT_LDS) {
        float(*T)[3 * CHUNK] = tile[wid];
        float2 sp = make_float2(0.f, 0.f);
        float sg = 0.f;
        auto fetch = [&](uint32_t c) {
            const uint32_t v = c * CHUNK + lane;
            const bool live = v < total;
            const uint32_t j = source_index(p, live ? v : total - 1, n0);
            sp = p.src_pos[j];
            sg = live ? p.src_gm[j] : 0.0f;
        };
        const uint32_t c_lo = v_lo / CHUNK, c_hi = (v_hi + CHUNK - 1) / CHUNK;
        if (c_lo < c_hi) fetch(c_lo);
        int buf = 0;
        for (uint32_t c = c_lo; c < c_hi; c++) {
            *reinterpret_cast<float2 *>(&T[buf][2 * lane]) = sp;
            T[buf][2 * CHUNK + lane] = sg;
            if (c + 1 < c_hi) fetch(c + 1);
            __builtin_amdgcn_fence(__ATOMIC_RELEASE, "wavefront");
            __builtin_amdgcn_wave_barrier();
            __builtin_amdgcn_fence(__ATOMIC_ACQUIRE, "wavefront");
            for (int jj = 0; jj < CHUNK; jj += 4) {
                const v8f P = *reinterpret_cast<const v8f *>(&T[buf][2 * jj]);
                const v4f G = *reinterpret_cast<const v4f *>(&T[buf][2 * CHUNK + jj]);
#pragma unroll
                for (int u = 0; u < 4; u++) interact<K, false>(R, f2v{P[2 * u], P[2 * u + 1]}, G[u]);
            }
            if (((c - c_lo) & (CLOSE_EVERY - 1)) == CLOSE_EVERY - 1) R.close_chunk();
            buf ^= 1;
        }
        if ((c_hi - c_lo) & (CLOSE_EVERY - 1)) R.close_chunk();
    } else {
#pragma unroll
        for (int range = 0; range < 2; range++) {
            const uint32_t r_lo = range == 0 ? 0u : n0;
            const uint32_t r_hi = range == 0 ? n0 : total;
            const uint32_t a = max(v_lo, r_lo), b = min(v_hi, r_hi);
            if (a >= b) continue;
            uint32_t j = p.src_begin[range] + (a - r_lo);
            const uint32_t j_end = p.src_begin[range] + (b - r_lo);
            const float *sp = reinterpret_cast<const float *>(p.src_pos), *sg = p.src_gm;
            const uint32_t groups = (j_end - j) / 8;
            const uint32_t g0 = (a - v_lo) / 8;
            if (groups > 0) {
                const uint32_t j_last = j + (groups - 1) * 8;
                v16f PA = src_load<v16f>(sp + 2 * (size_t)j);
                v8f GA = src_load<v8f>(sg + j);
                uint32_t g = 0;
                while (g + 2 <= groups) {
                    const uint32_t to_close = (8u * CLOSE_EVERY - ((g0 + g) & (8u * CLOSE_EVERY - 1))) / 2;
                    const uint32_t pairs = min(to_close, (groups - g) / 2);
                    for (uint32_t i = 0; i < pairs; i++) {
                        asm("" : "+s"(j) : "s"(PA), "s"(GA));
                        const v16f PB = src_load<v16f>(sp + 2 * (size_t)(j + 8));
                        const v8f GB = src_load<v8f>(sg + j + 8);
                        __builtin_amdgcn_sched_barrier(0);
                        interact8<K, true>(R, PA, GA);
                        __builtin_amdgcn_sched_barrier(0);
                        j = min(j + 16, j_last);
                        asm("" : "+s"(j) : "s"(PB), "s"(GB));
                        PA = src_load<v16f>(sp + 2 * (size_t)j);
                        GA = src_load<v8f>(sg + j);
                        __builtin_amdgcn_sched_barrier(0);
                        interact8<K, true>(R, PB, GB);
                    }
                    g += 2 * pairs;
                    if (pairs == to_close) R.close_chunk();
                }
                if (g < groups) interact8<K, true>(R, PA, GA);
                j = j_last + 8;
            }
            for (; j < j_end; j++) interact<K, true>(R, f2v{sp[2 * (size_t)j], sp[2 * (size_t)j + 1]}, sg[j]);
        }
        if ((v_hi - v_lo) & (CHUNK * CLOSE_EVERY - 1)) R.close_chunk();
    }

    auto finish = [&](uint32_t logical, float sx, float sy) {
        if (p.split > 1) {
            if (logical < p.n_recv) {
                float2 *slot = &p.parts[(size_t)part_y * p.n_recv + logical];
                if constexpr (FUSED) {
                    const uint64_t bits = (uint64_t)__float_as_uint(sx) | ((uint64_t)__float_as_uint(sy) << 32);
                    __hip_atomic_store(reinterpret_cast<uint64_t *>(slot), bits, __ATOMIC_RELAXED, __HIP_MEMORY_SCOPE_AGENT);
                } else {
                    *slot = make_float2(sx, sy);
                }
            }
        } else {
            finish_receiver(p, logical, sx, sy, dt);
        }
    };

    if constexpr (W == 1) {
#pragma unroll
        for (int k = 0; k < K; k++) finish(recv_base + k * WAVE + lane, R.s[k].x, R.s[k].y);
    } else {
#pragma unroll
        for (int k = 0; k < K; k++) partial[wid][k * WAVE + lane] = make_float2(R.s[k].x, R.s[k].y);
        __syncthreads();
#pragma unroll
        for (uint32_t slot = tid; slot < WAVE * K; slot += WAVE * W) {
            const float2 a = wave_sum(&partial[0][slot], WAVE * K, W);
            finish(recv_base + slot, a.x, a.y);
        }
    }

    if constexpr (FUSED) {
        if (p.split > 1) {
            __shared__ uint32_t is_last;
            asm volatile("s_waitcnt vmcnt(0)" ::: "memory");
            __syncthreads();
            if (tid == 0) {
                const uint32_t t = __hip_atomic_fetch_add(&p.tickets[tile_x], 1u, __ATOMIC_RELAXED, __HIP_MEMORY_SCOPE_AGENT);
                is_last = t == p.split - 1 ? 1u : 0u;
                if (is_last) __hip_atomic_store(&p.tickets[tile_x], 0u, __ATOMIC_RELAXED, __HIP_MEMORY_SCOPE_AGENT);
            }
            __syncthreads();
            if (is_last) {
                for (uint32_t slot = tid; slot < WAVE * K; slot += WAVE * W) {
                    const uint32_t logical = recv_base + slot;
                    if (logical >= p.n_recv) continue;
                    float2 part[MAX_SPLIT];
#pragma unroll
                    for (uint32_t s = 0; s < (uint32_t)MAX_SPLIT; s++) {
                        const uint64_t bits = __hip_atomic_load(reinterpret_cast<const uint64_t *>(&p.parts[(size_t)(s < p.split ? s : p.split - 1) * p.n_recv + logical]),
                                                                __ATOMIC_RELAXED, __HIP_MEMORY_SCOPE_AGENT);
                        part[s] = make_float2(__uint_as_float((uint32_t)bits), __uint_as_float((uint32_t)(bits >> 32)));
                    }
                    const uint32_t i = receiver_slot(p, logical);
                    const float2 a0 = p.acc[i], v0 = p.vel[i], q0 = p.pos_in[i];
                    float sx = 0.0f, sy = 0.0f;
#pragma unroll
                    for (uint32_t s = 0; s < (uint32_t)MAX_SPLIT; s++) add_part(sx, sy, part[s], s < p.split);
                    finish_loaded(p, i, make_float2(sx, sy), a0, v0, q0, dt);
                }
            }
        }
    }
}

template <int W, int H>
__device__ __forceinline__ void lane_split_body(const StepParams &p) {
    constexpr uint32_t R = WAVE / H;
    constexpr uint32_t V = W * H;
    constexpr uint32_t T = 2 * WAVE * W;
    extern __shared__ __attribute__((aligned(16))) unsigned char lds_raw[];
    float2 *sxy = reinterpret_cast<float2 *>(lds_raw);
    float *sgm = reinterpret_cast<float *>(sxy + T);
    float2 *partial = reinterpret_cast<float2 *>(sgm + T);
    const uint32_t n0 = p.src_end[0] - p.src_begin[0];
    const uint32_t ntiles = (n0 + T - 1) / T;

    const uint32_t tid = threadIdx.x;
    const uint32_t lane = tid & (WAVE - 1);
    const uint32_t wid = tid >> 6;
    const uint32_t r = lane % R, h = lane / R;
    const uint32_t v = wid * H + h;
    const float dt = *p.dt;

    float2 q0 = make_float2(0.f, 0.f), q1 = q0;
    float m0 = 0.f, m1 = 0.f;
    auto fetch = [&](uint32_t t) {
        const uint32_t last = p.src_begin[0] + n0 - 1;
        const uint32_t j0 = min(p.src_begin[0] + t * T + tid, last), j1 = min(j0 + WAVE * W, last);
        q0 = p.src_pos[j0];
        q1 = p.src_pos[j1];
        m0 = p.src_gm[j0];
        m1 = p.src_gm[j1];
    };
    if (ntiles > 0) fetch(0);

    Receivers<1> Rv;
    {
        uint32_t i = blockIdx.x * R + r;
        i = i < p.n_recv ? i : p.n_recv - 1;
        i = receiver_slot(p, i);
        const float2 q = p.pos_in[i];
        Rv.p[0] = f2v{q.x, q.y};
        Rv.r[0] = p.radius[i];
    }
    Rv.clear();
    const uint32_t my_logical = blockIdx.x * R + lane;
    const bool integrates = wid == 0 && lane < R && my_logical < p.n_recv && p.flags == 0;
    float2 vel0 = make_float2(0.f, 0.f);
    if (integrates) vel0 = p.vel[receiver_slot(p, my_logical)];
    uint32_t open_groups = 0;

    for (uint32_t t = 0; t < ntiles; t++) {
        if (t > 0) __syncthreads();
        sxy[tid] = q0;
        sxy[tid + WAVE * W] = q1;
        sgm[tid] = m0;
        sgm[tid + WAVE * W] = m1;
        if (t + 1 < ntiles) fetch(t + 1);
        __syncthreads();

        const SourceSlice lane_src = source_slice(min(T, n0 - t * T), 8u, 1, 0, V, v);
        const uint32_t v_lo = lane_src.lo, v_hi = lane_src.hi;

        uint32_t j = v_lo;
        const uint32_t groups = (v_hi - v_lo) / 4u;
        v4f P01 = {0.f, 0.f, 0.f, 0.f}, P23 = {0.f, 0.f, 0.f, 0.f}, G4 = {0.f, 0.f, 0.f, 0.f};
        if (groups > 0) {
            P01 = *reinterpret_cast<const v4f *>(&sxy[j]);
            P23 = *reinterpret_cast<const v4f *>(&sxy[j + 2]);
            G4 = *reinterpret_cast<const v4f *>(&sgm[j]);
        }
        for (uint32_t g = 0; g < groups; g++) {
            const v4f A01 = P01, A23 = P23, AG = G4;
            const uint32_t jn = g + 1 < groups ? j + 4 : j;
            P01 = *reinterpret_cast<const v4f *>(&sxy[jn]);
            P23 = *reinterpret_cast<const v4f *>(&sxy[jn + 2]);
            G4 = *reinterpret_cast<const v4f *>(&sgm[jn]);
            interact<1, false>(Rv, f2v{A01[0], A01[1]}, AG[0]);
            interact<1, false>(Rv, f2v{A01[2], A01[3]}, AG[1]);
            interact<1, false>(Rv, f2v{A23[0], A23[1]}, AG[2]);
            interact<1, false>(Rv, f2v{A23[2], A23[3]}, AG[3]);
            j += 4;
            if (++open_groups == 32) {
                Rv.close_chunk();
                open_groups = 0;
            }
        }
        for (; j < v_hi; j++) {
            const float2 a0 = sxy[j];
            interact<1, false>(Rv, f2v{a0.x, a0.y}, sgm[j]);
        }
    }
    Rv.close_chunk();

    partial[v * R + r] = make_float2(Rv.s[0].x, Rv.s[0].y);
    __syncthreads();
    constexpr uint32_t S = WAVE / R;
    constexpr uint32_t PER = V / S;
    if (wid == 0) {
        const uint32_t c = lane / R, rr = lane % R;
        float sx = 0.0f, sy = 0.0f;
#pragma unroll
        for (uint32_t s2 = 0; s2 < PER; s2++) {
            const float2 t = partial[(c * PER + s2) * R + rr];
            sx = __fadd_rn(sx, t.x);
            sy = __fadd_rn(sy, t.y);
        }
        __builtin_amdgcn_fence(__ATOMIC_RELEASE, "wavefront");
        partial[V * R + lane] = make_float2(sx, sy);
        __builtin_amdgcn_fence(__ATOMIC_RELEASE, "wavefront");
        __builtin_amdgcn_wave_barrier();
        __builtin_amdgcn_fence(__ATOMIC_ACQUIRE, "wavefront");
        if (lane < R) {
            float ax = 0.0f, ay = 0.0f;
#pragma unroll
            for (uint32_t c2 = 0; c2 < S; c2++) {
                const float2 t = partial[V * R + c2 * R + lane];
                ax = __fadd_rn(ax, t.x);
                ay = __fadd_rn(ay, t.y);
            }
            if (integrates) {
                finish_loaded(p, receiver_slot(p, my_logical), make_float2(ax, ay), make_float2(0.f, 0.f), vel0,
                              make_float2(Rv.p[0].x, Rv.p[0].y), dt);
            } else {
                finish_receiver(p, my_logical, ax, ay, dt);
            }
        }
    }
}

template <int W, int H>
__global__ __launch_bounds__(WAVE *W) void lane_split_kernel(const StepParams p) {
    lane_split_body<W, H>(p);
}

struct ChainTrace {
    const float *mass;
    double *row;
    size_t pitch;
    uint32_t until;
    uint32_t every;
    bool entry;
};

template <bool TRACE>
__device__ __forceinline__ void chain_body(const ChainParams &p, const ChainTrace &tr) {
    constexpr int K = CHAIN_K;
    static_assert(CHAIN_K == nbd::K && WAVE * CHAIN_K == nbd::TILE, "a chain tile is a diagnostics tile");
    __shared__ __attribute__((aligned(16))) float spos[2][2 * CHAIN_MAX_RECV];
    __shared__ __attribute__((aligned(16))) float sgm[CHAIN_MAX_RECV];
    __shared__ float2 partial[16][WAVE * K];
    __shared__ float smass[TRACE ? CHAIN_MAX_RECV : 1];
    __shared__ float2 svel[TRACE ? CHAIN_MAX_RECV : 1];
    __shared__ double srow[TRACE ? CHAIN_MAX_RECV / (WAVE * K) : 1][nbd::QTY];

    const uint32_t tid = threadIdx.x;
    const uint32_t lane = tid & (WAVE - 1);
    const uint32_t wid = __builtin_amdgcn_readfirstlane(tid >> 6);
    const uint32_t W = 16u / p.tiles;
    const uint32_t tile = wid / W, slice = wid % W;
    const uint32_t tile_base = tile * (WAVE * K);
    const float dt = *p.dt;

    for (uint32_t i = tid; i < p.n_recv; i += 1024) {
        const float2 q = p.pos[i];
        spos[0][2 * i] = q.x;
        spos[0][2 * i + 1] = q.y;
        if (i < p.n_src) sgm[i] = p.src_gm[i];
        if constexpr (TRACE)
            if (i < p.n_src) smass[i] = tr.mass[i];
    }
    Receivers<K> R;
    uint32_t ridx[K];
#pragma unroll
    for (int k = 0; k < K; k++) {
        uint32_t i = tile_base + k * WAVE + lane;
        i = i < p.n_recv ? i : p.n_recv - 1;
        ridx[k] = i;
        R.r[k] = p.radius[i];
    }
    const uint32_t local = tid - tile * W * WAVE;
    const uint32_t mine = tile_base + local;
    const bool integrates = local < WAVE * K && mine < p.n_recv;
    float2 v = make_float2(0.f, 0.f), a = make_float2(0.f, 0.f);
    if (integrates) v = p.vel[mine];

    const SourceSlice wave_src = source_slice(p.n_src, 8u, 1, 0, W, slice);
    const uint32_t v_lo = wave_src.lo, v_hi = wave_src.hi;

    double *row = tr.row;
    auto record = [&](const float *S) {
        const uint32_t rb = tile_base;
        if (slice == 0 && rb < p.n_src) {
            float px[K], py[K];
            uint32_t ri[K];
#pragma unroll
            for (int k = 0; k < K; k++) {
                const uint32_t i = rb + k * WAVE + lane;
                ri[k] = i < p.n_src ? i : p.n_src - 1;
                px[k] = S[2 * ri[k]];
                py[k] = S[2 * ri[k] + 1];
            }
            double sum[K], e[K][nbd::QTY], t[nbd::QTY];
            nbd::tile_potential(sum, px, py, R.r, ri, rb, p.n_src, nbd::LdsSources{S, sgm});
#pragma unroll
            for (int k = 0; k < K; k++) {
                const uint32_t i = rb + k * WAVE + lane;
                nbd::energy_terms(e[k], i < p.n_src, -sum[k], smass, reinterpret_cast<const float2 *>(S), svel, i);
            }
            nbd::tile_tree(t, e);
            if (lane == 0) {
#pragma unroll
                for (int q = 0; q < nbd::QTY; q++) srow[tile][q] = t[q];
            }
        }
        __syncthreads();
        if (tid < (uint32_t)nbd::REDUCE_THREADS)
            nbd::reduce_rows_shfl(&srow[0][0], (p.n_src + nbd::TILE - 1) / nbd::TILE, row, tid);
        row += tr.pitch;
    };
    uint32_t until = tr.until;
    if constexpr (TRACE)
        if (tr.entry && integrates) svel[mine] = v;
    __syncthreads();
    if constexpr (TRACE)
        if (tr.entry) record(spos[0]);

    int cur = 0;
    for (uint32_t step = 0; step < p.steps; step++) {
        const bool due = TRACE && --until == 0;
        const float *S = spos[cur];
#pragma unroll
        for (int k = 0; k < K; k++) R.p[k] = f2v{S[2 * ridx[k]], S[2 * ridx[k] + 1]};
        R.clear();
        uint32_t j = v_lo;
        const uint32_t groups = (v_hi - v_lo) / 8u;
        for (uint32_t g = 0; g < groups; g++, j += 8) {
            const v16f P = *reinterpret_cast<const v16f *>(&S[2 * j]);
            const v8f G = *reinterpret_cast<const v8f *>(&sgm[j]);
            interact8<K, false>(R, P, G);
            if ((g & (8u * CLOSE_EVERY - 1)) == 8u * CLOSE_EVERY - 1) R.close_chunk();
        }
        for (; j < v_hi; j++) interact<K, false>(R, f2v{S[2 * j], S[2 * j + 1]}, sgm[j]);
        if ((v_hi - v_lo) & (CHUNK * CLOSE_EVERY - 1)) R.close_chunk();
#pragma unroll
        for (int k = 0; k < K; k++) partial[wid][k * WAVE + lane] = make_float2(R.s[k].x, R.s[k].y);
        __syncthreads();
        if (integrates) {
            a = wave_sum(&partial[tile * W][local], WAVE * K, W);
            float2 q = make_float2(S[2 * mine], S[2 * mine + 1]);
            integrate(a, dt, v, q);
            spos[cur ^ 1][2 * mine] = q.x;
            spos[cur ^ 1][2 * mine + 1] = q.y;
            if constexpr (TRACE)
                if (due) svel[mine] = v;
        }
        __syncthreads();
        cur ^= 1;
        if constexpr (TRACE) {
            if (due) {
                record(spos[cur]);
                until = tr.every;
            }
        }
    }
    if (integrates && (!TRACE || p.steps > 0)) {
        p.pos[mine] = make_float2(spos[cur][2 * mine], spos[cur][2 * mine + 1]);
        p.vel[mine] = v;
        p.acc[mine] = a;
    }
}

__global__ __launch_bounds__(1024) void chain_kernel(const ChainParams p) { chain_body<false>(p, ChainTrace{}); }

__device__ __forceinline__ uint32_t uniform_u32(uint32_t v) { return __builtin_amdgcn_readfirstlane(v); }

struct Member {
    uint32_t index, n, tiles;
};

__device__ __forceinline__ Member member_of(const BatchParams &bp, uint32_t block) { return {block, bp.n_recv, bp.tiles}; }

__device__ __forceinline__ Member member_of(const RaggedParams &rp, uint32_t block) {
    const uint32_t index = uniform_u32(rp.members[block]);
    const uint32_t n = uniform_u32(rp.n_len[index]);
    return {index, n, n <= WAVE * CHAIN_K ? 1u : n <= 2 * WAVE * CHAIN_K ? 2u : 4u};
}

__device__ __forceinline__ ChainParams member_chain(const BatchParams &bp, const Member &m) {
    const size_t base = (size_t)m.index * bp.stride;
    ChainParams p;
    p.pos = bp.pos_in + base;
    p.vel = bp.vel + base;
    p.acc = bp.acc + base;
    p.radius = bp.radius + base;
    p.src_gm = bp.gm + base;
    p.n_recv = m.n;
    p.n_src = uniform_u32(bp.mass_len[m.index]);
    p.steps = bp.steps;
    p.tiles = m.tiles;
    p.dt = bp.dt + m.index;
    return p;
}

template <class P>
__global__ __launch_bounds__(1024) void batch_chain_kernel(const P bp) {
    chain_body<false>(member_chain(bp, member_of(bp, blockIdx.x)), ChainTrace{});
}

template <class P>
__global__ __launch_bounds__(1024) void batch_trace_chain_kernel(const P bp, const TraceParams tp) {
    const Member m = member_of(bp, blockIdx.x);
    ChainTrace tr;
    tr.mass = tp.mass + (size_t)m.index * bp.stride;
    tr.pitch = (size_t)tp.count * nbd::QTY;
    tr.entry = tp.done == 0;
    tr.every = tp.every;
    tr.until = tp.every - tp.done % tp.every;
    tr.row = tp.rows + ((size_t)(tp.done == 0 ? 0u : 1u + tp.done / tp.every) * tp.count + m.index) * nbd::QTY;
    chain_body<true>(member_chain(bp, m), tr);
}

template <int W, int H, class P>
__global__ __launch_bounds__(WAVE *W) void batch_lane_split_kernel(const P bp) {
    const Member m = member_of(bp, blockIdx.y);
    if constexpr (std::is_same_v<P, RaggedParams>)
        if (blockIdx.x * (WAVE / H) >= m.n) return;
    const size_t base = (size_t)m.index * bp.stride;
    const StepParams p = plain_step(bp.pos_in + base, bp.gm + base, uniform_u32(bp.mass_len[m.index]), bp.pos_in + base,
                                    bp.pos_out + base, bp.vel + base, bp.acc + base, bp.radius + base, m.n, bp.dt + m.index, 8);
    lane_split_body<W, H>(p);
}

#define NB_CASE(KERNEL, A, B, ...) \
    if (a == A && b == B) return reinterpret_cast<const void *>(&KERNEL<A, B, ##__VA_ARGS__>);

template <int VARIANT>
const void *pick(int a, int b) {
    NB_CASE(step_kernel, 1, 1, VARIANT) NB_CASE(step_kernel, 1, 4, VARIANT) NB_CASE(step_kernel, 1, 8, VARIANT) NB_CASE(step_kernel, 1, 16, VARIANT)
    NB_CASE(step_kernel, 2, 1, VARIANT) NB_CASE(step_kernel, 2, 4, VARIANT) NB_CASE(step_kernel, 2, 8, VARIANT) NB_CASE(step_kernel, 2, 16, VARIANT)
#ifdef NB_TUNING_SHAPES
    NB_CASE(step_kernel, 1, 2, VARIANT) NB_CASE(step_kernel, 2, 2, VARIANT) NB_CASE(step_kernel, 4, 1, VARIANT) NB_CASE(step_kernel, 4, 2, VARIANT)
    NB_CASE(step_kernel, 4, 4, VARIANT) NB_CASE(step_kernel, 4, 8, VARIANT) NB_CASE(step_kernel, 4, 16, VARIANT)
#endif
    return nullptr;
}

const void *pick_fused(int a, int b) {
    NB_CASE(step_kernel, 1, 4, VARIANT_SMEM, true) NB_CASE(step_kernel, 1, 8, VARIANT_SMEM, true) NB_CASE(step_kernel, 1, 16, VARIANT_SMEM, true)
    NB_CASE(step_kernel, 2, 4, VARIANT_SMEM, true) NB_CASE(step_kernel, 2, 8, VARIANT_SMEM, true) NB_CASE(step_kernel, 2, 16, VARIANT_SMEM, true)
    return nullptr;
}

const void *pick_lane_split(int a, int b) {
    NB_CASE(lane_split_kernel, 4, 2) NB_CASE(lane_split_kernel, 8, 2) NB_CASE(lane_split_kernel, 16, 2) NB_CASE(lane_split_kernel, 4, 4)
    NB_CASE(lane_split_kernel, 8, 4) NB_CASE(lane_split_kernel, 16, 4) NB_CASE(lane_split_kernel, 8, 8) NB_CASE(lane_split_kernel, 16, 8)
    return nullptr;
}

}

const void *step_kernel_fn(LaunchShape s) {
    if (s.lanes > 1) return pick_lane_split(s.w, s.lanes);
    return s.variant == VARIANT_SMEM ? pick<VARIANT_SMEM>(s.k, s.w) : pick<VARIANT_LDS>(s.k, s.w);
}

const void *step_kernel_fused_fn(LaunchShape s) {
    if (s.lanes > 1 || s.variant != VARIANT_SMEM) return nullptr;
    return pick_fused(s.k, s.w);
}

const void *finish_kernel_fn() { return reinterpret_cast<const void *>(&finish_kernel); }

const void *batch_lane_split_fn(int a, int b, bool listed) {
    if (listed) {
        NB_CASE(batch_lane_split_kernel, 8, 8, RaggedParams) NB_CASE(batch_lane_split_kernel, 16, 4, RaggedParams)
    } else {
        NB_CASE(batch_lane_split_kernel, 8, 8, BatchParams) NB_CASE(batch_lane_split_kernel, 16, 4, BatchParams)
    }
    return nullptr;
}
#undef NB_CASE

void launch_chain(hipStream_t st, const ChainParams &p) {
    hipLaunchKernelGGL(chain_kernel, dim3(1), dim3(1024), 0, st, p);
}

void launch_batch_chain(hipStream_t st, const RaggedParams &p, uint32_t workgroups) {
    if (p.members)
        hipLaunchKernelGGL(batch_chain_kernel<RaggedParams>, dim3(workgroups), dim3(1024), 0, st, p);
    else
        hipLaunchKernelGGL(batch_chain_kernel<BatchParams>, dim3(workgroups), dim3(1024), 0, st, static_cast<const BatchParams &>(p));
}

void launch_batch_trace_chain(hipStream_t st, const RaggedParams &p, const TraceParams &t, uint32_t workgroups) {
    if (p.members)
        hipLaunchKernelGGL(batch_trace_chain_kernel<RaggedParams>, dim3(workgroups), dim3(1024), 0, st, p, t);
    else
        hipLaunchKernelGGL(batch_trace_chain_kernel<BatchParams>, dim3(workgroups), dim3(1024), 0, st, static_cast<const BatchParams &>(p), t);
}

}
```

nbody_amd/csrc/launch_shape.h:

```cpp
#pragma once

#include "kernels.h"

namespace nb {

constexpr uint32_t BATCH_MAX_RECV = 3000;

struct LaunchShape {
    int k = 0;
    int w = 0;
    int variant = VARIANT_SMEM;
    int split = 0;
    int unit = 0;
    int lanes = 0;
};

inline bool operator==(const LaunchShape &a, const LaunchShape &b) {
    return a.k == b.k && a.w == b.w && a.variant == b.variant && a.split == b.split && a.unit == b.unit && a.lanes == b.lanes;
}

inline bool shape_on_auto(const LaunchShape &want) { return want == LaunchShape{}; }

constexpr uint32_t LANE_SPLIT_MAX_SRC = 1u << 18;

int lane_split_rule(uint32_t n_recv, uint32_t n_src, int *w);

LaunchShape choose_shape(LaunchShape want, uint32_t n_recv, uint32_t n_src, int compute_units);

bool fused_finish_rule(uint32_t n_recv, uint32_t n_src);

dim3 step_grid(LaunchShape s, uint32_t n_recv);
dim3 step_block(LaunchShape s);
size_t step_lds_bytes(LaunchShape s, uint32_t n_src);
dim3 finish_grid(uint32_t n_recv);
dim3 finish_block();

uint32_t chain_tiles(uint32_t n_recv);

int batch_lane_shape(uint32_t n_recv, int *w);

}
```

nbody_amd/csrc/launch_shape.hip:

```cpp
#include "launch_shape.h"

namespace nb {
namespace {

constexpr int WAVE = 64;
constexpr int CHUNK = 64;

double small_launch_cost_us(uint32_t n_recv, uint32_t n_src, int k, int w, int sp, int unit, int cus) {
    constexpr double LAT = 1.575, THR = 0.7545, K1 = 0.987, K1A = 0.178, A = 0.179, MIX = 0.874;
    constexpr double FINISH = 2.08, W4 = 1.035, UFIX = 0.15, BASE = 2.27;
    const uint32_t granules = (n_src + unit - 1) / unit;
    const uint64_t groups = ((uint64_t)n_recv + WAVE * k - 1) / (WAVE * k) * (uint64_t)sp;
    const uint64_t capacity = (uint64_t)cus * (32 / w);
    const uint64_t full = groups / capacity, left = groups % capacity;
    const uint32_t part_granules = (granules + sp - 1) / sp;
    const uint32_t wave_granules = (part_granules + w - 1) / w;
    const double units = (double)k * (wave_granules ? wave_granules : 1) * (double)unit / (double)CHUNK + UFIX;
    auto chunk_time = [&](double occ) {
        const double f = k == 1 ? K1 + K1A * (8.0 - occ) / 8.0 : 1.0;
        const double busy = occ * THR * f * (1.0 + A * (8.0 - occ) / 8.0);
        return LAT > busy ? LAT : busy;
    };
    double t = (double)full * units * chunk_time(8.0);
    if (left) {
        double occ = (w / 4.0) * (double)((left + cus - 1) / cus);
        if (occ > 8.0) occ = 8.0;
        const double lock = units * chunk_time(occ);
        const double fluid = units * chunk_time(8.0) * (double)left / (double)capacity;
        t += full ? MIX * lock + (1.0 - MIX) * fluid : lock;
    }
    if (sp > 1) t += FINISH;
    if (w == 4) t *= W4;
    return t + BASE;
}

}

int lane_split_rule(uint32_t n_recv, uint32_t n_src, int *w) {
    const double pairs = (double)n_recv * (double)n_src;
    *w = 16;
    if (n_src == 0 || n_recv == 0 || n_src > LANE_SPLIT_MAX_SRC || pairs > 9.0e6) return 1;
    if (pairs <= 1.5e5) {
        *w = 8;
        return 4;
    }
    if (pairs <= 2.5e6) {
        *w = 8;
        return 8;
    }
    return 4;
}

LaunchShape choose_shape(LaunchShape want, uint32_t n_recv, uint32_t n_src, int compute_units) {
    if (compute_units <= 0) compute_units = 256;
    if (shape_on_auto(want)) {
        int w = 16;
        const int lanes = lane_split_rule(n_recv, n_src, &w);
        if (lanes > 1) {
            want.lanes = lanes;
            want.w = w;
        }
    }
    if (want.lanes > 1) {
        LaunchShape sh = want;
        sh.k = 1;
        sh.w = (want.w == 4 || want.w == 8 || want.w == 16) ? want.w : 16;
        if (sh.lanes == 8 && sh.w == 4) sh.w = 8;
        if (sh.lanes != 2 && sh.lanes != 4 && sh.lanes != 8) sh.lanes = 4;
        sh.split = 1;
        sh.unit = 8;
        sh.variant = VARIANT_LDS;
        return sh;
    }
    if (want.variant == VARIANT_LDS) want.unit = CHUNK;
    const uint32_t chunks = (n_src + CHUNK - 1) / CHUNK;
    const bool small = ((uint64_t)n_recv + 2 * WAVE - 1) / (2 * WAVE) < (uint64_t)compute_units * 2;
    LaunchShape best = want;
    best.lanes = 1;
    double best_cost = -1.0;
    for (int k = 2; k >= 1; k--) {
        if (want.k != 0 && want.k != k) continue;
        for (int w = 16; w >= 4; w /= 2) {
            if (want.w != 0 && want.w != w) continue;
            for (int sp = 1; sp <= MAX_SPLIT; sp++) {
                if (want.split != 0 && want.split != sp) continue;
                const bool few_unsplit_tiles = sp == 1 && ((uint64_t)n_recv + WAVE * k - 1) / (WAVE * k) <= 24;
                const int tiny_w = n_src <= 128 ? 8 : 16;
                if (small && want.w == 0 && (few_unsplit_tiles ? w != tiny_w : w == 16)) continue;
                for (int unit = CHUNK; unit >= 8; unit /= 2) {
                    if (want.unit != 0 && want.unit != unit) continue;
                    if (!small && want.unit == 0 && unit != CHUNK) continue;
                    double cost;
                    if (small) {
                        cost = small_launch_cost_us(n_recv, n_src, k, w, sp, unit, compute_units);
                    } else {
                        const uint64_t groups = ((uint64_t)n_recv + WAVE * k - 1) / (WAVE * k) * (uint64_t)sp;
                        const uint64_t capacity = (uint64_t)compute_units * (32 / w);
                        const uint64_t rounds = (groups + capacity - 1) / capacity;
                        const uint32_t part_chunks = (chunks + sp - 1) / sp;
                        const uint32_t wave_chunks = (part_chunks + w - 1) / w;
                        constexpr double TAIL = 0.13;
                        cost = ((double)rounds + TAIL) * ((double)k * (wave_chunks ? wave_chunks : 1) + 1.0);
                        if (sp > 1) cost += 3.0 + 0.02 * sp;
                        if (w < 16) cost *= 1.01;
                        if (k == 1) cost *= 1.02;
                    }
                    if (best_cost < 0.0 || cost < best_cost * 0.999) {
                        best_cost = cost;
                        best.k = k;
                        best.w = w;
                        best.split = sp;
                        best.unit = unit;
                    }
                }
            }
        }
    }
    if (best_cost < 0.0) {
        best.k = want.k ? want.k : 2;
        best.w = want.w ? want.w : 16;
        best.split = want.split ? want.split : 1;
        best.unit = want.unit ? want.unit : CHUNK;
    }
    return best;
}

dim3 step_grid(LaunchShape s, uint32_t n_recv) {
    if (s.lanes > 1) return dim3((n_recv + WAVE / s.lanes - 1) / (WAVE / s.lanes), 1);
    return dim3((n_recv + WAVE * s.k - 1) / (WAVE * s.k), s.split > 1 ? s.split : 1);
}

size_t step_lds_bytes(LaunchShape s, uint32_t n_src) {
    if (s.lanes <= 1) return 0;
    (void)n_src;
    return (size_t)2 * WAVE * s.w * 12 + ((size_t)s.w + 1) * WAVE * sizeof(float2);
}
dim3 finish_grid(uint32_t n_recv) { return dim3((n_recv + 255u) / 256u); }
dim3 finish_block() { return dim3(256); }
dim3 step_block(LaunchShape s) { return dim3(WAVE * s.w); }

uint32_t chain_tiles(uint32_t n_recv) {
    for (uint32_t t = 1; t <= 4; t *= 2)
        if (n_recv <= t * WAVE * CHAIN_K) return t;
    return 0;
}

int batch_lane_shape(uint32_t n_recv, int *w) { return lane_split_rule(n_recv, n_recv, w); }

constexpr double FUSED_FINISH_MIN_PAIRS = 4.0e7;
constexpr uint32_t FUSED_FINISH_MAX_RECV = 200000;

bool fused_finish_rule(uint32_t n_recv, uint32_t n_src) {
    return (double)n_recv * (double)n_src >= FUSED_FINISH_MIN_PAIRS && n_recv <= FUSED_FINISH_MAX_RECV;
}

}
```

nbody_amd/csrc/nbody_hip_tuning.h:

```cpp
#ifndef NBODY_AMD_NBODY_HIP_TUNING_H
#define NBODY_AMD_NBODY_HIP_TUNING_H

#include "nbody_hip.h"

#ifdef __cplusplus
extern "C" {
#endif

int nb_hip_tune(SimPipeline *sim, const char *key, int value);

int nb_hip_tuning_build(void);

uint32_t nb_hip_last_fused_steps(const SimPipeline *sim);

int nb_hip_launch_lanes(const SimPipeline *sim);
int nb_hip_launch_unit(const SimPipeline *sim);

int nb_hip_plan_launch_lanes(uint32_t n_recv, uint32_t n_src, int *w);
int nb_hip_plan_fused_finish(uint32_t n_recv, uint32_t n_src, int compute_units);
int nb_hip_plan_launch_unit(uint32_t n_recv, uint32_t n_src, int compute_units);

double nb_hip_last_diag_ms(SimPipeline *sim);

double nb_hip_ensemble_last_diag_ms(SimBatch *batch);

void nb_hip_ensemble_trace_mode(SimBatch *batch, int mode);
void nb_hip_ensemble_last_trace_info(const SimBatch *batch, int *fused, uint32_t *launches);

double nb_hip_last_render_ms(SimPipeline *sim, double *parts);

void nb_hip_ensemble_render_mode(SimBatch *batch, int mode);
void nb_hip_ensemble_last_render_info(const SimBatch *batch, int *tile_path, uint32_t *launches);
double nb_hip_ensemble_last_render_ms(SimBatch *batch);

void nb_hip_last_leapfrog_info(const SimPipeline *sim, uint32_t *force_launches, int *primed);
void nb_hip_ensemble_last_leapfrog_info(const SimBatch *batch, uint32_t *force_launches, int *primed);

void nb_hip_live_resources(uint32_t *buffers, uint32_t *events);

#ifdef __cplusplus
}
#endif

#endif
```

nbody_amd/csrc/pipeline.hip:

```cpp
#include "pipeline_internal.h"
#include "nbody_hip_tuning.h"

using namespace nbi;

namespace {

void unpin_host(SimPipeline *s) {
    if (s->host_pinned) {
        (void)hipHostUnregister(s->host_array);
        s->host_pinned = false;
        s->host_dev = nullptr;
        s->host_current = false;
    }
}

void pin_host(SimPipeline *s) {
    if (s->host_pinned || s->host_array == nullptr || s->host_bytes == 0) return;
    if (hipHostRegister(s->host_array, s->host_bytes, hipHostRegisterMapped | hipHostRegisterPortable) == hipSuccess) {
        s->host_pinned = true;
        if (hipHostGetDevicePointer(&s->host_dev, s->host_array, 0) != hipSuccess) {
            (void)hipGetLastError();
            s->host_dev = nullptr;
        }
    } else {
        (void)hipGetLastError();
    }
}

void release_device(SimPipeline *s) {
    if (!s->on_device) return;
    use_device();
    ASSERT_HIP(hipStreamSynchronize(s->stream), "sync before release");
    if (s->comm_stream) ASSERT_HIP(hipStreamSynchronize(s->comm_stream), "sync before release");
    if (s->direct) {
        uint64_t tag[64] = {0};
        tag[s->rank < 64 ? s->rank : 0] = ~0ull;
        s->host_gather(s->host_gather_ctx, tag, sizeof(uint64_t), s->rank, s->nranks);
        for (int b = 0; b < 2; b++)
            for (int q = 0; q < (int)s->peer_src[b].size(); q++)
                if (q != s->rank && s->peer_src[b][q]) ASSERT_HIP(hipIpcCloseMemHandle(s->peer_src[b][q]), "hipIpcCloseMemHandle(rank %d)", q);
        tag[s->rank < 64 ? s->rank : 0] = ~1ull;
        s->host_gather(s->host_gather_ctx, tag, sizeof(uint64_t), s->rank, s->nranks);
    }
    unpin_host(s);
    for (auto &g : s->graphs) destroy_graph(g);
    if (s->stage) ASSERT_HIP(hipHostFree(s->stage), "hipHostFree staging");
    if (s->comm_stream) ASSERT_HIP(hipStreamDestroy(s->comm_stream), "stream");
    if (!s->group) ASSERT_HIP(hipStreamDestroy(s->stream), "stream");
}

void set_simulation_data(SimPipeline *s, const Particle *ps);

void materialize(SimPipeline *s) {
    use_device();
    if (s->on_device) return;
    if (s->group)
        s->stream = s->group->stream;
    else
        ASSERT_HIP(hipStreamCreateWithFlags(&s->stream, hipStreamNonBlocking), "stream");

    const uint32_t N = s->data.total_len, M = s->data.mass_len;
    if (!s->sharded) {
        s->slots = N;
        s->n_real = N;
        s->n_src = M;
    } else {
        s->n_real = s->plan.mass_count + s->plan.zero_count;
        if (!s->group) ASSERT_HIP(hipStreamCreateWithFlags(&s->comm_stream, hipStreamNonBlocking), "comm stream");
        s->slots = s->plan.mass_chunk + s->plan.zero_chunk;
        s->n_src = s->plan.src_padded;
    }
    const uint32_t cap = s->slots ? s->slots : 1;
    for (int b = 0; b < 2; b++) s->pos[b].alloc(cap);
    s->vel.alloc(cap);
    s->acc.alloc(cap);
    s->radius.alloc(cap);
    s->mass.alloc(cap);
    s->src_gm.alloc(s->n_src);
    s->dt_dev.alloc(1);
    s->aos.alloc(N);
    if (!s->sharded) {
        s->src_pos[0] = s->pos[0];
        s->src_pos[1] = s->pos[1];
    } else {
        for (int b = 0; b < 2; b++) s->src_pos[b] = s->gathered[b].alloc(s->n_src);
        s->aos_shard.alloc((size_t)s->slots * (size_t)s->nranks);
        if (s->host_gather) {
            const size_t a = (size_t)s->n_src * sizeof(float2), b = (size_t)s->slots * (size_t)s->nranks * sizeof(Particle);
            s->stage_bytes = a > b ? a : b;
            ASSERT_HIP(hipHostMalloc(&s->stage, s->stage_bytes ? s->stage_bytes : 1, hipHostMallocDefault), "staging of %zu bytes",
                       s->stage_bytes);
        }
        if (s->direct) {
            NB_ASSERT(s->nranks <= 64, "direct transport: at most 64 ranks");
            struct Handles {
                hipIpcMemHandle_t h[2];
            };
            std::vector<Handles> all((size_t)s->nranks);
            for (int b = 0; b < 2; b++)
                ASSERT_HIP(hipIpcGetMemHandle(&all[(size_t)s->rank].h[b], s->src_pos[b]), "hipIpcGetMemHandle of the gathered array %d", b);
            s->host_gather(s->host_gather_ctx, all.data(), sizeof(Handles), s->rank, s->nranks);
            for (int b = 0; b < 2; b++) {
                s->peer_src[b].assign((size_t)s->nranks, nullptr);
                for (int q = 0; q < s->nranks; q++) {
                    if (q == s->rank) {
                        s->peer_src[b][(size_t)q] = s->src_pos[b];
                        continue;
                    }
                    void *mapped = nullptr;
                    ASSERT_HIP(hipIpcOpenMemHandle(&mapped, all[(size_t)q].h[b], hipIpcMemLazyEnablePeerAccess),
                               "hipIpcOpenMemHandle of rank %d's gathered array %d", q, b);
                    s->peer_src[b][(size_t)q] = static_cast<float2 *>(mapped);
                }
            }
        }
    }
    s->on_device = true;
    pin_host(s);
    static bool graph_machinery_warm = false;
    if (!graph_machinery_warm && s->use_graph != 0) {
        graph_machinery_warm = true;
        hipGraph_t g = nullptr;
        hipGraphExec_t e = nullptr;
        if (hipStreamBeginCapture(s->stream, hipStreamCaptureModeThreadLocal) == hipSuccess) {
            nb::launch_set_scalar(s->stream, s->dt_dev, 0.0f);
            if (hipStreamEndCapture(s->stream, &g) == hipSuccess && g != nullptr &&
                hipGraphInstantiate(&e, g, nullptr, nullptr, 0) == hipSuccess) {
                (void)hipGraphLaunch(e, s->stream);
                (void)hipStreamSynchronize(s->stream);
            }
        }
        if (e) (void)hipGraphExecDestroy(e);
        if (g) (void)hipGraphDestroy(g);
        (void)hipGetLastError();
    }
}

}

extern "C" {

SimPipeline *CreateSimPipeline(WorldData data) {
    NB_ASSERT(data.mass_len <= data.total_len, "mass_len %u > total_len %u", data.mass_len, data.total_len);
    SimPipeline *s = new SimPipeline();
    s->data = data;
    s->plan = nb_hip_shard_plan(data.total_len, data.mass_len, 0, 1);
    const char *v = getenv("NB_HIP_VARIANT");
    if (v) s->want.variant = atoi(v) ? nb::VARIANT_SMEM : nb::VARIANT_LDS;
    const char *gr = getenv("NB_HIP_GRAPH");
    if (gr) s->use_graph = atoi(gr) < 0 || atoi(gr) > 2 ? 2 : atoi(gr);
#ifdef NB_TUNING_SHAPES
    struct { const char *env, *key; } presets[] = {
        {"NB_HIP_K", "k"}, {"NB_HIP_W", "w"}, {"NB_HIP_SPLIT", "split"}, {"NB_HIP_UNIT", "unit"}, {"NB_HIP_PASSES", "passes"},
        {"NB_HIP_LANES", "lanes"}, {"NB_HIP_FUSED_CHAIN", "fused_chain"}, {"NB_HIP_FUSED_FINISH", "fused_finish"},
        {"NB_HIP_READBACK", "readback"}, {"NB_HIP_ZERO_COPY_UPLOAD", "zero_copy_upload"},
    };
    for (const auto &p : presets)
        if (const char *e = getenv(p.env)) nb_hip_tune(s, p.key, atoi(e));
    if (const char *tm = getenv("NB_HIP_TIMING")) s->timing = atoi(tm) ? 1 : 0;
#endif
    return s;
}

SimPipeline *CreateSimPipelineSharded(WorldData data, int rank, int nranks, const void *unique_id128) {
    NB_ASSERT(nranks >= 1 && rank >= 0 && rank < nranks, "rank %d of %d", rank, nranks);
    const char *force = getenv("NB_HIP_FORCE_SHARDED");
    if (nranks == 1 && !(force && atoi(force))) return CreateSimPipeline(data);
    NB_ASSERT(unique_id128 != nullptr, "sharded pipeline needs the RCCL unique id");
    SimPipeline *s = CreateSimPipeline(data);
    s->rank = rank;
    s->nranks = nranks;
    s->sharded = true;
    s->plan = nb_hip_shard_plan(data.total_len, data.mass_len, rank, nranks);
    const char *ov = getenv("NB_HIP_OVERLAP");
    if (ov) s->overlap = atoi(ov) ? 1 : 0;
    const char *sg = getenv("NB_HIP_SHARDED_GRAPH");
    if (sg) s->sharded_graph = atoi(sg) ? 1 : 0;
    comm_create(s, unique_id128);
    return s;
}

SimPipeline *CreateSimPipelineShardedWith(WorldData data, int rank, int nranks, NbAllGatherFn allgather, void *ctx) {
    NB_ASSERT(nranks >= 1 && rank >= 0 && rank < nranks, "rank %d of %d", rank, nranks);
    NB_ASSERT(allgather != nullptr, "NULL all-gather callback");
    SimPipeline *s = CreateSimPipeline(data);
    s->rank = rank;
    s->nranks = nranks;
    s->sharded = true;
    s->plan = nb_hip_shard_plan(data.total_len, data.mass_len, rank, nranks);
    s->host_gather = allgather;
    s->host_gather_ctx = ctx;
    const char *ov = getenv("NB_HIP_OVERLAP");
    if (ov) s->overlap = atoi(ov) ? 1 : 0;
    return s;
}

SimPipeline *CreateSimPipelineShardedDirect(WorldData data, int rank, int nranks, NbAllGatherFn control, void *ctx) {
    SimPipeline *s = CreateSimPipelineShardedWith(data, rank, nranks, control, ctx);
    s->direct = true;
    return s;
}

void nb_hip_plan_launch(uint32_t n_recv, uint32_t n_src, int compute_units, int *k, int *w, int *split, uint32_t *workgroups) {
    const nb::LaunchShape sh = nb::choose_shape({.lanes = 1}, n_recv, n_src, compute_units);
    if (k) *k = sh.k;
    if (w) *w = sh.w;
    if (split) *split = sh.split;
    if (workgroups) {
        const dim3 g = nb::step_grid(sh, n_recv);
        *workgroups = g.x * g.y;
    }
}

int nb_hip_plan_launch_lanes(uint32_t n_recv, uint32_t n_src, int *w) {
    int ww = 16;
    const int lanes = n_src <= nb::LANE_SPLIT_MAX_SRC ? nb::lane_split_rule(n_recv, n_src, &ww) : 1;
    if (w) *w = ww;
    return lanes;
}

int nb_hip_plan_fused_finish(uint32_t n_recv, uint32_t n_src, int compute_units) {
    const nb::LaunchShape sh = nb::choose_shape({.lanes = 1}, n_recv, n_src, compute_units);
    return sh.split > 1 && nb_hip_plan_launch_lanes(n_recv, n_src, nullptr) <= 1 && nb::fused_finish_rule(n_recv, n_src) ? 1 : 0;
}

int nb_hip_plan_launch_unit(uint32_t n_recv, uint32_t n_src, int compute_units) {
    return nb::choose_shape({.lanes = 1}, n_recv, n_src, compute_units).unit;
}

void DestroySimPipeline(SimPipeline *sim) {
    if (sim == nullptr) return;
    release_device(sim);
    if (sim->group) {
        LocalGroup *g = sim->group;
        for (auto &m : g->members)
            if (m == sim) m = nullptr;
        bool empty = true;
        for (auto m : g->members) empty = empty && m == nullptr;
        if (empty) {
            ASSERT_HIP(hipStreamDestroy(g->stream), "group stream");
            delete g;
        }
    }
    comm_destroy(sim);
    delete sim;
}

void SetSimulationData(SimPipeline *s, const Particle *ps) {
    NB_ASSERT(s != nullptr, "NULL pipeline");
    NB_ASSERT(ps != nullptr || s->data.total_len == 0, "NULL particle array");
    if (!s->on_device) {
        RandGuard keep_callers_rand_stream;
        materialize(s);
        set_simulation_data(s, ps);
        return;
    }
    use_device();
    set_simulation_data(s, ps);
}

}

namespace {

void set_simulation_data(SimPipeline *s, const Particle *ps) {
    const uint32_t N = s->data.total_len, M = s->data.mass_len;
    if (N == 0) return;
    hipStream_t st = s->stream;
    s->cur = 0;
    s->host_current = false;
    s->acc_current = false;
    s->updates_since_get = 0;
    zero_tickets(s);
    const bool zero_copy = !s->sharded && ps == s->host_array && s->host_dev != nullptr && s->zero_copy_upload &&
                           s->host_bytes >= (size_t)N * sizeof(Particle);
    if (!zero_copy)
        ASSERT_HIP(hipMemcpyAsync(s->aos, ps, (size_t)N * sizeof(Particle), hipMemcpyHostToDevice, st), "H2D of %u particles", N);
    if (!s->sharded) {
        nb::launch_split(st, zero_copy ? s->host_dev : s->aos, 0, N, s->pos[0], s->vel, s->acc, s->radius, s->mass, 0);
        nb::launch_make_gm(st, s->mass, s->src_gm, M, NB_G);
    } else {
        const NbShardPlan &pl = s->plan;
        nb::launch_fill_pad(st, s->pos[0], s->vel, s->acc, s->radius, s->mass, 0, s->slots);
        nb::launch_split(st, s->aos, pl.mass_begin, pl.mass_count, s->pos[0], s->vel, s->acc, s->radius, s->mass, 0);
        nb::launch_split(st, s->aos, pl.zero_begin, pl.zero_count, s->pos[0], s->vel, s->acc, s->radius, s->mass,
                         pl.mass_chunk);
        nb::launch_split_sources(st, s->aos, M, s->n_src, s->src_pos[0], s->src_pos[1], s->src_gm, NB_G);
        if (s->overlap) s->ev_gather.record(s->group ? s->stream : s->comm_stream);
    }
    ASSERT_HIP(hipStreamSynchronize(st), "sync after SetSimulationData");
    if (s->direct) {
        uint64_t ready[64] = {0};
        ready[s->rank] = 1;
        s->host_gather(s->host_gather_ctx, ready, sizeof(uint64_t), s->rank, s->nranks);
    }
    if (wants_canonical(s)) (void)find_or_build_graph(s, CANON_STEPS, 0.0f, resolve_shape(s));
}

}

extern "C" {

void GetSimulationData(const SimPipeline *cs, Particle *ps) {
    SimPipeline *s = const_cast<SimPipeline *>(cs);
    NB_ASSERT(s != nullptr && ps != nullptr, "NULL argument");
    NB_ASSERT(s->on_device, "GetSimulationData before SetSimulationData");
    const uint32_t N = s->data.total_len;
    if (N == 0) return;
    if (!s->sharded) {
        if (ps == s->host_array && s->updates_since_get == 1)
            s->frame_streak++;
        else
            s->frame_streak = 0;
        s->updates_since_get = 0;
        if (s->host_current) {
            if (ps != s->host_array) memcpy(ps, s->host_array, (size_t)N * sizeof(Particle));
            return;
        }
    }
    use_device();
    hipStream_t st = s->stream;
    if (!s->sharded) {
        nb::launch_merge(st, s->aos, 0, N, s->pos[s->cur], s->vel, s->acc, s->radius, s->mass, 0);
    } else {
        const NbShardPlan &pl = s->plan;
        Particle *shard = s->aos_shard;
        Particle *mine = shard + (size_t)s->rank * s->slots;
        if (s->group) {
            for (SimPipeline *q : s->group->members)
                nb::launch_merge(st, shard + (size_t)q->rank * s->slots, 0, q->slots, q->pos[q->cur], q->vel, q->acc,
                                 q->radius, q->mass, 0);
        } else {
            nb::launch_merge(st, mine, 0, s->slots, s->pos[s->cur], s->vel, s->acc, s->radius, s->mass, 0);
            const size_t floats = (size_t)s->slots * (sizeof(Particle) / sizeof(float));
            if (s->host_gather)
                host_allgather(s, shard, floats * sizeof(float), st);
            else
                comm_allgather_f32(s, shard, floats, st, "particle slices");
        }
        for (int q = 0; q < s->nranks; q++) {
            const NbShardPlan pq = nb_hip_shard_plan(N, s->data.mass_len, q, s->nranks);
            const Particle *from = shard + (size_t)q * s->slots;
            if (pq.mass_count)
                ASSERT_HIP(hipMemcpyAsync(s->aos + pq.mass_begin, from,
                                          (size_t)pq.mass_count * sizeof(Particle), hipMemcpyDeviceToDevice, st),
                           "unpack massive slice of rank %d", q);
            if (pq.zero_count)
                ASSERT_HIP(hipMemcpyAsync(s->aos + pq.zero_begin, from + pl.mass_chunk,
                                          (size_t)pq.zero_count * sizeof(Particle), hipMemcpyDeviceToDevice, st),
                           "unpack massless slice of rank %d", q);
        }
    }
    ASSERT_HIP(hipMemcpyAsync(ps, s->aos, (size_t)N * sizeof(Particle), hipMemcpyDeviceToHost, st), "D2H of %u particles", N);
    if (s->comm) {
        Watchdog dog("the collective GetSimulationData", s->rank, s->nranks);
        ASSERT_HIP(hipStreamSynchronize(st), "sync after GetSimulationData");
    } else {
        ASSERT_HIP(hipStreamSynchronize(st), "sync after GetSimulationData");
    }
}

void nb_hip_step_async(SimPipeline *s, uint32_t n, float dt) {
    NB_ASSERT(s != nullptr, "NULL pipeline");
    enqueue_steps(s, n, dt);
}

void nb_hip_sync(SimPipeline *s) {
    NB_ASSERT(s != nullptr, "NULL pipeline");
    if (!s->on_device) return;
    use_device();
    if (s->comm) {
        Watchdog dog("the step chain's all-gathers (stream sync)", s->rank, s->nranks);
        ASSERT_HIP(hipStreamSynchronize(s->stream), "stream sync");
        if (s->comm_stream) ASSERT_HIP(hipStreamSynchronize(s->comm_stream), "comm stream sync");
        return;
    }
    ASSERT_HIP(hipStreamSynchronize(s->stream), "stream sync");
    if (s->comm_stream) ASSERT_HIP(hipStreamSynchronize(s->comm_stream), "comm stream sync");
}

void PerformSimUpdate(SimPipeline *s, uint32_t n, float dt) {
    nb_hip_step_async(s, n, dt);
    if (n > 0 && s->on_device && !s->sharded && s->slots > 0) {
        if (s->updates_since_get > 0) s->frame_streak = 0;
        s->updates_since_get++;
        const bool eager = s->host_dev != nullptr && s->host_bytes >= (size_t)s->data.total_len * sizeof(Particle) &&
                           (s->readback == 1 || (s->readback == 2 && s->frame_streak >= 2));
        if (eager) {
            nb::launch_merge(s->stream, s->host_dev, 0, s->data.total_len, s->pos[s->cur], s->vel, s->acc, s->radius, s->mass, 0);
            s->host_current = true;
        }
    }
    nb_hip_sync(s);
}

double nb_hip_last_step_ms(SimPipeline *s, uint32_t *launches) {
    NB_ASSERT(s != nullptr, "NULL pipeline");
    if (launches) *launches = 0;
    if (!s->on_device || !s->step_iv.valid()) return 0.0;
    if (launches) *launches = s->timed_launches;
    return s->step_iv.ms();
}

uint32_t nb_hip_last_finish_launches(const SimPipeline *s) {
    NB_ASSERT(s != nullptr, "NULL pipeline");
    return s->step_iv.valid() ? s->timed_finish_launches : 0;
}

uint32_t nb_hip_last_step_breakdown(SimPipeline *s, double *kernel_ms, double *comm_ms) {
    NB_ASSERT(s != nullptr, "NULL pipeline");
    if (kernel_ms) *kernel_ms = 0.0;
    if (comm_ms) *comm_ms = 0.0;
    if (!s->on_device || (!s->step_iv.valid() && !s->group) || s->detail_steps == 0) return 0;
    use_device();
    ASSERT_HIP(hipStreamSynchronize(s->stream), "stream sync");
    if (s->comm_stream) ASSERT_HIP(hipStreamSynchronize(s->comm_stream), "comm stream sync");
    auto total = [](const std::vector<std::pair<hipEvent_t, hipEvent_t>> &iv) {
        double sum = 0.0;
        for (const auto &p : iv) sum += elapsed_ms(p.first, p.second);
        return sum;
    };
    if (kernel_ms) *kernel_ms = total(s->kernel_iv);
    if (comm_ms) *comm_ms = total(s->comm_iv);
    return s->detail_steps;
}

uint32_t nb_hip_graph_stats(const SimPipeline *s, uint32_t *dt_uploads) {
    NB_ASSERT(s != nullptr, "NULL pipeline");
    if (dt_uploads) *dt_uploads = s->dt_uploads;
    return (uint32_t)s->graphs.size();
}

uint32_t nb_hip_last_fused_steps(const SimPipeline *s) {
    NB_ASSERT(s != nullptr, "NULL pipeline");
    return s->fused_steps;
}

int nb_hip_launch_lanes(const SimPipeline *s) {
    NB_ASSERT(s != nullptr, "NULL pipeline");
    return s->last_shape.lanes > 1 ? s->last_shape.lanes : 1;
}

int nb_hip_launch_unit(const SimPipeline *s) {
    NB_ASSERT(s != nullptr, "NULL pipeline");
    return s->last_shape.unit;
}

void nb_hip_note_host_array(SimPipeline *s, void *array, uint64_t bytes) {
    NB_ASSERT(s != nullptr, "NULL pipeline");
    if (s->on_device) use_device();
    if (s->on_device) ASSERT_HIP(hipStreamSynchronize(s->stream), "sync before re-registering the host array");
    unpin_host(s);
    s->host_array = array;
    s->host_bytes = (size_t)bytes;
    if (s->on_device) pin_host(s);
}

int nb_hip_configure(SimPipeline *s, const char *key, int value) {
    NB_ASSERT(s != nullptr && key != nullptr, "NULL argument");
    int old = 0;
    if (!strcmp(key, "variant")) {
        NB_ASSERT(value == 0 || value == 1, "variant must be 0 (lds) or 1 (smem), got %d", value);
        old = s->want.variant;
        s->want.variant = value;
    } else if (!strcmp(key, "graph")) {
        NB_ASSERT(value >= 0 && value <= 2, "graph must be 0 (never), 1 (always) or 2 (from the second use), got %d", value);
        old = s->use_graph;
        s->use_graph = value;
    } else if (!strcmp(key, "timing")) {
        old = s->timing;
        s->timing = value ? 1 : 0;
    } else if (!strcmp(key, "sharded_graph")) {
        old = s->sharded_graph;
        s->sharded_graph = value ? 1 : 0;
    } else if (!strcmp(key, "overlap")) {
        old = s->overlap;
        if (s->on_device && s->sharded) nb_hip_sync(s);
        s->overlap = value ? 1 : 0;
        if (s->on_device && s->overlap && s->sharded)
            s->ev_gather.record(s->group ? s->stream : s->comm_stream);
    } else {
        NB_FAIL("unknown knob \"%s\" (include/nbody_hip.h lists the knobs; launch-shape hooks: nbody_hip_tuning.h)", key);
    }
    return old;
}

int nb_hip_tuning_build(void) {
#ifdef NB_TUNING_SHAPES
    return 1;
#else
    return 0;
#endif
}

int nb_hip_tune(SimPipeline *s, const char *key, int value) {
    NB_ASSERT(s != nullptr && key != nullptr, "NULL argument");
    int old = 0;
    if (!strcmp(key, "k")) {
        NB_ASSERT(value == 0 || value == 1 || value == 2 || value == 4, "k must be 0, 1, 2 or 4, got %d", value);
        old = s->want.k;
        s->want.k = value;
    } else if (!strcmp(key, "w")) {
        NB_ASSERT(value == 0 || value == 1 || value == 2 || value == 4 || value == 8 || value == 16,
                  "w must be 0, 1, 2, 4, 8 or 16, got %d", value);
        old = s->want.w;
        s->want.w = value;
    } else if (!strcmp(key, "split")) {
        NB_ASSERT(value >= 0 && value <= nb::MAX_SPLIT, "split must be 0 (auto) .. %d, got %d", nb::MAX_SPLIT, value);
        old = s->want.split;
        s->want.split = value;
    } else if (!strcmp(key, "unit")) {
        NB_ASSERT(value == 0 || value == 8 || value == 16 || value == 32 || value == 64, "unit must be 0, 8, 16, 32 or 64, got %d", value);
        old = s->want.unit;
        s->want.unit = value;
    } else if (!strcmp(key, "lanes")) {
        NB_ASSERT(value == 0 || value == 1 || value == 2 || value == 4 || value == 8, "lanes must be 0 (auto), 1, 2, 4 or 8, got %d", value);
        old = s->want.lanes;
        s->want.lanes = value;
    } else if (!strcmp(key, "fused_chain")) {
        NB_ASSERT(value >= 0 && value <= 2, "fused_chain must be 0 (never), 1 (whenever the world fits one workgroup) or 2 (auto), got %d", value);
        old = s->fused_chain;
        s->fused_chain = value;
    } else if (!strcmp(key, "fused_finish")) {
        NB_ASSERT(value >= 0 && value <= 2, "fused_finish must be 0 (never), 1 (whenever the shape allows) or 2 (auto), got %d", value);
        old = s->fused_finish;
        if (s->on_device && old != value) {
            ASSERT_HIP(hipStreamSynchronize(s->stream), "sync before switching the finish mode");
            for (auto &g : s->graphs) destroy_graph(g);
            s->graphs.clear();
        }
        s->fused_finish = value;
    } else if (!strcmp(key, "passes")) {
        NB_ASSERT(value >= 0 && value <= 64, "passes must be 0 (auto) .. 64, got %d", value);
        old = s->want_passes;
        s->want_passes = value;
    } else if (!strcmp(key, "readback")) {
        NB_ASSERT(value >= 0 && value <= 2, "readback must be 0 (lazy), 1 (eager) or 2 (auto), got %d", value);
        old = s->readback;
        s->readback = value;
        s->frame_streak = 0;
    } else if (!strcmp(key, "render_merge")) {
        NB_ASSERT(value == 0 || value == 1, "render_merge must be 0 (one atomic per lane) or 1 (merged), got %d", value);
        old = s->render_merge;
        s->render_merge = value;
    } else if (!strcmp(key, "field_shape")) {
        NB_ASSERT(value >= 0 && value <= 2, "field_shape must be 0 (auto), 1 (source split) or 2 (one wave per tile), got %d", value);
        old = s->field_shape;
        s->field_shape = value;
    } else if (!strcmp(key, "gravity_shape")) {
        NB_ASSERT(value >= 0 && value <= 2, "gravity_shape must be 0 (auto), 1 (source split) or 2 (one wave per tile), got %d", value);
        old = s->gravity_shape;
        s->gravity_shape = value;
    } else if (!strcmp(key, "render_detail")) {
        old = s->render_detail;
        s->render_detail = value ? 1 : 0;
    } else if (!strcmp(key, "zero_copy_upload")) {
        old = s->zero_copy_upload;
        s->zero_copy_upload = value ? 1 : 0;
    } else {
        NB_FAIL("unknown tuning hook \"%s\"", key);
    }
    return old;
}

void nb_hip_launch_shape(const SimPipeline *s, int *k, int *w, int *variant, int *split, uint32_t *workgroups) {
    NB_ASSERT(s != nullptr, "NULL pipeline");
    if (split) *split = s->last_shape.split;
    if (k) *k = s->last_shape.k;
    if (w) *w = s->last_shape.w;
    if (variant) *variant = s->last_shape.variant;
    if (workgroups) *workgroups = s->last_groups;
}

}
```

nbody_amd/csrc/pipeline_internal.h:

```cpp
#pragma once

#include <hip/hip_runtime.h>

#include <stdint.h>
#include <stdio.h>
#include <stdlib.h>
#include <string.h>

#include <atomic>
#include <condition_variable>
#include <mutex>
#include <thread>
#include <utility>
#include <vector>

#include "convert.h"
#include "kernels.h"
#include "launch_shape.h"
#include "nbody_hip.h"
#include "render_kernels.h"


#define NB_FAIL(...)                                                          \
    do {                                                                      \
        fprintf(stderr, "%s:%d [%s] ", __FILE__, __LINE__, __func__);         \
        fprintf(stderr, __VA_ARGS__);                                         \
        fprintf(stderr, "\n");                                                \
        abort();                                                              \
    } while (0)

#define NB_ASSERT(COND, ...)               \
    do {                                   \
        if (!(COND)) NB_FAIL(__VA_ARGS__); \
    } while (0)

#define ASSERT_HIP(X, ...)                                                                              \
    do {                                                                                                \
        hipError_t nb_e_ = (X);                                                                         \
        if (nb_e_ != hipSuccess) {                                                                      \
            fprintf(stderr, "%s:%d [%s] hipError_t = %d, str = %s\n", __FILE__, __LINE__, __func__,     \
                    (int)nb_e_, hipGetErrorString(nb_e_));                                              \
            NB_FAIL(__VA_ARGS__);                                                                       \
        }                                                                                               \
    } while (0)

#define NB_HIDDEN __attribute__((visibility("hidden")))

typedef struct ncclComm *ncclComm_t;

namespace nbi {


struct DeviceCtx {
    bool ready = false;
    int ordinal = -1;
    int compute_units = 0;
    char info[256] = {0};
};
extern DeviceCtx g_dev;
extern int g_requested_ordinal;

void ensure_device();
void use_device();
void *dev_alloc_bytes(size_t bytes);
void dev_free(void *p);
extern NB_HIDDEN std::atomic<uint32_t> g_live_buffers, g_live_events;

class RandGuard {
  public:
    RandGuard() {
        std::lock_guard<std::mutex> l(gate());
        if (alive()++ == 0) saved() = initstate(1u, private_state(), 128);
    }
    ~RandGuard() {
        std::lock_guard<std::mutex> l(gate());
        if (--alive() == 0 && saved()) {
            setstate(saved());
            saved() = nullptr;
        }
    }
    RandGuard(const RandGuard &) = delete;
    RandGuard &operator=(const RandGuard &) = delete;

  private:
    static std::mutex &gate() {
        static std::mutex m;
        return m;
    }
    static int &alive() {
        static int n = 0;
        return n;
    }
    static char *&saved() {
        static char *p = nullptr;
        return p;
    }
    static char *private_state() {
        static char buf[128];
        return buf;
    }
};

template <typename T>
T *dev_alloc(size_t count) {
    return static_cast<T *>(dev_alloc_bytes((count ? count : 1) * sizeof(T)));
}

inline uint32_t round_up(uint32_t v, uint32_t m) { return (v + m - 1) / m * m; }


template <typename T>
class NB_HIDDEN DevBuf {
  public:
    DevBuf() = default;
    DevBuf(DevBuf &&o) noexcept : p_(o.p_), n_(o.n_) { o.p_ = nullptr, o.n_ = 0; }
    DevBuf(const DevBuf &) = delete;
    DevBuf &operator=(const DevBuf &) = delete;
    ~DevBuf() { dev_free(p_); }

    operator T *() const { return p_; }
    size_t count() const { return n_; }

    T *alloc(size_t count) {
        NB_ASSERT(p_ == nullptr, "device array made twice");
        n_ = count;
        return p_ = dev_alloc<T>(count);
    }
    bool grown(hipStream_t st, size_t need) { return regrow(st, need, 0); }
    bool grown_carrying(hipStream_t st, size_t need, size_t head) { return regrow(st, need, head); }

  private:
    bool regrow(hipStream_t st, size_t need, size_t head) {
        if (p_ && n_ >= need) return false;
        T *old = p_;
        p_ = nullptr;
        if (old && head == 0) {
            ASSERT_HIP(hipStreamSynchronize(st), "sync before regrowing a scratch buffer");
            dev_free(old);
            old = nullptr;
        }
        alloc(need);
        if (old) {
            ASSERT_HIP(hipMemcpyAsync(p_, old, head, hipMemcpyDeviceToDevice, st), "carry the head of a regrown buffer over");
            ASSERT_HIP(hipStreamSynchronize(st), "sync before freeing the old buffer");
            dev_free(old);
        }
        return true;
    }
    T *p_ = nullptr;
    size_t n_ = 0;
};

class NB_HIDDEN DevEvent {
  public:
    explicit DevEvent(unsigned flags = hipEventDefault) : flags_(flags) {}
    DevEvent(DevEvent &&o) noexcept : ev_(o.ev_), flags_(o.flags_) { o.ev_ = nullptr; }
    DevEvent(const DevEvent &) = delete;
    DevEvent &operator=(const DevEvent &) = delete;
    ~DevEvent() {
        if (!ev_) return;
        ASSERT_HIP(hipEventDestroy(ev_), "event");
        g_live_events--;
    }
    hipEvent_t get() {
        if (!ev_) {
            ASSERT_HIP(hipEventCreateWithFlags(&ev_, flags_), "event");
            g_live_events++;
        }
        return ev_;
    }
    void record(hipStream_t st) { ASSERT_HIP(hipEventRecord(get(), st), "event record"); }

  private:
    hipEvent_t ev_ = nullptr;
    unsigned flags_;
};

inline double elapsed_ms(hipEvent_t ev0, hipEvent_t ev1) {
    ASSERT_HIP(hipEventSynchronize(ev1), "end event");
    float ms = 0.0f;
    ASSERT_HIP(hipEventElapsedTime(&ms, ev0, ev1), "elapsed time");
    return (double)ms;
}

class NB_HIDDEN Interval {
  public:
    void begin(hipStream_t st) { first.record(st); }
    void end(hipStream_t st) {
        last.record(st);
        valid_ = true;
    }
    void clear() { valid_ = false; }
    bool valid() const { return valid_; }
    double ms() { return valid_ ? elapsed_ms(first.get(), last.get()) : 0.0; }
    DevEvent first, last;

  private:
    bool valid_ = false;
};


class Watchdog {
  public:
    Watchdog(const char *what, int rank, int nranks);
    ~Watchdog();
    Watchdog(const Watchdog &) = delete;
    Watchdog &operator=(const Watchdog &) = delete;

  private:
    uint64_t seq_ = 0;
};

void comm_create(::SimPipeline *s, const void *unique_id128);
void comm_destroy(::SimPipeline *s);
void comm_allgather_f32(::SimPipeline *s, void *base, size_t count_per_rank, hipStream_t st, const char *what);


struct StepGraph {
    uint32_t n = 0;
    uint32_t passes = 1;
    hipGraph_t graph = nullptr;
    hipGraphExec_t exec = nullptr;
    std::vector<hipGraphNode_t> nodes;
    std::vector<nb::StepParams> params;
    int phase = -1;
    nb::LaunchShape shape;
    uint64_t last_use = 0;
};

struct EventPool {
    std::vector<DevEvent> ev;
    size_t used = 0;
    hipEvent_t next() {
        if (used == ev.size()) ev.emplace_back();
        return ev[used++].get();
    }
};

}

struct LocalGroup {
    std::vector<SimPipeline *> members;
    hipStream_t stream = nullptr;
};

struct SimPipeline {
    WorldData data;
    int rank = 0, nranks = 1;
    bool sharded = false;
    NbShardPlan plan;
    ncclComm_t comm = nullptr;
    struct LocalGroup *group = nullptr;
    NbAllGatherFn host_gather = nullptr;
    void *host_gather_ctx = nullptr;
    void *stage = nullptr;
    size_t stage_bytes = 0;
    bool direct = false;
    std::vector<float2 *> peer_src[2];
    uint64_t direct_steps = 0;

    bool on_device = false;
    uint32_t slots = 0;
    uint32_t n_real = 0;
    uint32_t n_src = 0;

    nbi::DevBuf<float2> pos[2];
    nbi::DevBuf<float2> vel, acc;
    nbi::DevBuf<float> radius, mass;
    float2 *src_pos[2] = {nullptr, nullptr};
    nbi::DevBuf<float2> gathered[2];
    nbi::DevBuf<float> src_gm;
    nbi::DevBuf<float> dt_dev;
    float dt_enqueued = 0.0f;
    bool dt_valid = false;
    uint32_t dt_uploads = 0;
    nbi::DevBuf<Particle> aos;
    nbi::DevBuf<Particle> aos_shard;
    void *host_array = nullptr;
    size_t host_bytes = 0;
    bool host_pinned = false;
    void *host_dev = nullptr;
    int readback = 2;
    int zero_copy_upload = 1;
    bool host_current = false;
    uint32_t updates_since_get = 0, frame_streak = 0;
    int timing = 0;
    nbi::DevBuf<float2> parts;
    nbi::DevBuf<uint32_t> tickets;
    int fused_finish = 2;
    int cur = 0;

    hipStream_t stream = nullptr;
    hipStream_t comm_stream = nullptr;
    nbi::Interval step_iv;
    nbi::DevEvent ev_local{hipEventDisableTiming}, ev_gather{hipEventDisableTiming};
    uint32_t timed_launches = 0;
    uint32_t timed_finish_launches = 0;
    nbi::EventPool pool;
    std::vector<std::pair<hipEvent_t, hipEvent_t>> kernel_iv, comm_iv;
    uint32_t detail_steps = 0;
    uint64_t use_clock = 0;

    nb::LaunchShape want;
    int use_graph = 2, overlap = 0, sharded_graph = 0;
    int fused_chain = 2;
    std::vector<uint32_t> seen_chains;
    int want_passes = 0;
    double first_gather_ms = 0.0;
    double comm_init_ms = 0.0;
    double small_gather_us = 0.0;
    nb::LaunchShape last_shape = {.variant = nb::VARIANT_LDS};
    uint32_t last_groups = 0;
    uint32_t fused_steps = 0;

    std::vector<nbi::StepGraph> graphs;

    nbi::DevBuf<double> diag;
    nbi::DevBuf<float> diag_phi;
    nbi::Interval diag_iv;

    nbi::DevBuf<uint32_t> render_counts;
    nbi::DevBuf<nb::render::Disc> render_discs;
    nbi::DevBuf<uint32_t> render_words;
    nbi::DevBuf<uint32_t> render_rgba;
    nbi::Interval render_iv, bounds_iv;
    nbi::DevEvent ev_splat, ev_disc;
    bool render_detailed = false;
    int render_merge = 1, render_detail = 0;

    nbi::DevBuf<float> sample_in;
    nbi::DevBuf<float> sample_out;
    int field_shape = 0;
    int gravity_shape = 0;

    nbi::DevBuf<char> adapt;
    bool adapt_armed = false;
    uint32_t adapt_logged = 0;
    std::vector<char> adapt_host;

    bool acc_current = false;
    uint32_t lf_force_launches = 0;
    bool lf_primed = false;
};

namespace nbi {


constexpr uint32_t CANON_STEPS = 32;
constexpr uint32_t CHAIN_MAX_STEPS_PER_LAUNCH = 1u << 16;
constexpr uint32_t DETAIL_STEPS_MAX = 256;

void destroy_graph(StepGraph &g);
nb::LaunchShape resolve_shape(SimPipeline *s);
bool wants_canonical(const SimPipeline *s);
StepGraph *find_graph(SimPipeline *s, uint32_t n, uint32_t passes, nb::LaunchShape sh, int phase);
StepGraph *find_or_build_graph(SimPipeline *s, uint32_t n, float dt, nb::LaunchShape sh);
void evict_for_one_more(SimPipeline *s);
constexpr uint32_t GRAPH_CHAIN_MAX = 64;
nb::StepParams whole_step(const SimPipeline *s, int in, float dt);
uint32_t passes_for(const SimPipeline *s, const nb::StepParams &p);
void launch_step(SimPipeline *s, nb::LaunchShape sh, const nb::StepParams &p, hipStream_t st);
void upload_dt(SimPipeline *s, float dt);
void zero_tickets(SimPipeline *s);
void begin_call(SimPipeline *s);
void end_call(SimPipeline *s, uint32_t launches);
void enqueue_steps(SimPipeline *s, uint32_t n, float dt);


void sharded_step(SimPipeline *s, nb::LaunchShape sh, float dt, hipStream_t cs, bool detail = false);
void host_allgather(SimPipeline *s, void *dev_base, size_t bytes_per_rank, hipStream_t st);
void enqueue_sharded(SimPipeline *s, uint32_t n, float dt);


void check_adaptive_cfg(const void *s, uint32_t n, const NbAdaptive *cfg, const char *what);


void check_diag(SimPipeline *s, const char *what);

}
```

nbody_amd/csrc/step_chain.hip:

```cpp
#include "pipeline_internal.h"

namespace nbi {

constexpr size_t GRAPH_CACHE_MAX = 8;
constexpr uint32_t GRAPH_AUTO_MIN_CHAIN = 16;

void evict_for_one_more(SimPipeline *s) {
    while (s->graphs.size() >= GRAPH_CACHE_MAX) {
        size_t victim = 0;
        for (size_t i = 1; i < s->graphs.size(); i++)
            if (s->graphs[i].last_use < s->graphs[victim].last_use) victim = i;
        ASSERT_HIP(hipStreamSynchronize(s->stream), "sync before evicting a cached chain");
        destroy_graph(s->graphs[victim]);
        s->graphs.erase(s->graphs.begin() + (long)victim);
    }
}

void destroy_graph(StepGraph &g) {
    if (g.exec) ASSERT_HIP(hipGraphExecDestroy(g.exec), "hipGraphExecDestroy");
    if (g.graph) ASSERT_HIP(hipGraphDestroy(g.graph), "hipGraphDestroy");
    g.exec = nullptr;
    g.graph = nullptr;
    g.nodes.clear();
    g.params.clear();
}

nb::LaunchShape resolve_shape(SimPipeline *s) {
    nb::LaunchShape want = s->want;
    nb::StepParams probe;
    memset(&probe, 0, sizeof probe);
    probe.src_end[0] = s->n_src;
    const uint32_t passes = (s->sharded && s->overlap) ? 1 : passes_for(s, probe);
    if (s->sharded || passes != 1 || s->n_src > nb::LANE_SPLIT_MAX_SRC || s->n_src == 0) want.lanes = 1;
    nb::LaunchShape sh = nb::choose_shape(want, s->n_real, (s->n_src + passes - 1) / passes, g_dev.compute_units);
    NB_ASSERT(nb::step_kernel_fn(sh) != nullptr, "no step kernel for k=%d w=%d variant=%d", sh.k, sh.w, sh.variant);
    if (sh.split > 1 && s->n_real > 0 && s->parts.grown(s->stream, (size_t)sh.split * s->n_real)) {
        if (!s->tickets) {
            s->tickets.alloc((size_t)s->n_real / 64 + 2);
            zero_tickets(s);
            ASSERT_HIP(hipStreamSynchronize(s->stream), "sync after zeroing the tickets");
        }
        for (auto &g : s->graphs) destroy_graph(g);
        s->graphs.clear();
    }
    s->last_shape = sh;
    s->last_groups = nb::step_grid(sh, s->n_real).x * nb::step_grid(sh, s->n_real).y;
    return sh;
}

nb::StepParams whole_step(const SimPipeline *s, int in, float dt) {
    (void)dt;
    nb::StepParams p = nb::plain_step(s->src_pos[in], s->src_gm, s->n_src, s->pos[in], s->pos[in ^ 1], s->vel, s->acc, s->radius,
                                      s->n_real, s->dt_dev, 64);
    if (s->sharded) {
        p.recv_split = s->plan.mass_count;
        p.recv_gap = s->plan.mass_chunk - s->plan.mass_count;
        p.mirror = s->src_pos[in ^ 1] + (size_t)s->rank * s->plan.mass_chunk;
        p.n_mirror = s->plan.mass_count;
    }
    return p;
}

bool fused_finish_applies(const SimPipeline *s, nb::LaunchShape sh) {
    if (s->fused_finish == 0 || s->sharded || sh.split <= 1 || sh.lanes > 1 || !s->tickets) return false;
    if (nb::step_kernel_fused_fn(sh) == nullptr) return false;
    return s->fused_finish == 1 || nb::fused_finish_rule(s->n_real, s->n_src);
}

nb::StepParams shaped(const SimPipeline *s, nb::StepParams p, nb::LaunchShape sh) {
    p.split = sh.split > 1 ? (uint32_t)sh.split : 1u;
    p.parts = p.split > 1 ? s->parts : nullptr;
    p.tickets = s->tickets;
    p.unit = (sh.unit >= 8 && sh.unit <= 64 && p.src_end[1] == p.src_begin[1]) ? (uint32_t)sh.unit : 64u;
    return p;
}

constexpr size_t L2_SOURCE_BUDGET = 3u << 20;

uint32_t passes_for(const SimPipeline *s, const nb::StepParams &p) {
    if (p.flags != 0 || p.src_end[1] != p.src_begin[1]) return 1;
    const uint32_t n = p.src_end[0] - p.src_begin[0];
    uint32_t want = (uint32_t)s->want_passes;
    if (want == 0) want = (uint32_t)(((size_t)n * 12 + L2_SOURCE_BUDGET - 1) / L2_SOURCE_BUDGET);
    const uint32_t chunks = (n + 63) / 64;
    if (want > chunks) want = chunks;
    return want ? want : 1;
}

std::vector<nb::StepParams> step_passes(const SimPipeline *s, const nb::StepParams &whole, nb::LaunchShape sh) {
    std::vector<nb::StepParams> out;
    const uint32_t P = passes_for(s, whole);
    const uint32_t lo = whole.src_begin[0], n = whole.src_end[0] - lo;
    const uint32_t per = ((n + 63) / 64 + P - 1) / P * 64;
    for (uint32_t q = 0; q < P; q++) {
        nb::StepParams p = shaped(s, whole, sh);
        if (P > 1) {
            p.src_begin[0] = lo + (q * per < n ? q * per : n);
            p.src_end[0] = lo + ((q + 1) * per < n ? (q + 1) * per : n);
            p.flags = (q > 0 ? nb::STEP_ACC_IN : 0u) | (q + 1 < P ? nb::STEP_NO_FINALIZE : 0u);
        }
        out.push_back(p);
    }
    return out;
}

void launch_step(SimPipeline *s, nb::LaunchShape sh, const nb::StepParams &p, hipStream_t st) {
    if (s->n_real == 0) return;
    const bool fused = fused_finish_applies(s, sh);
    for (nb::StepParams &copy : step_passes(s, p, sh)) {
        void *args[] = {&copy};
        ASSERT_HIP(hipLaunchKernel(fused ? nb::step_kernel_fused_fn(sh) : nb::step_kernel_fn(sh), nb::step_grid(sh, s->n_real), nb::step_block(sh), args,
                                   nb::step_lds_bytes(sh, copy.src_end[0] - copy.src_begin[0]), st),
                   "step kernel launch (k=%d w=%d variant=%d split=%d, %u receivers)", sh.k, sh.w, sh.variant, sh.split,
                   s->n_real);
        if (copy.split > 1 && !fused)
            ASSERT_HIP(hipLaunchKernel(nb::finish_kernel_fn(), nb::finish_grid(s->n_real), nb::finish_block(), args, 0, st),
                       "finish kernel launch (%u receivers, %u parts)", s->n_real, copy.split);
    }
}

void zero_tickets(SimPipeline *s) {
    if (s->tickets) ASSERT_HIP(hipMemsetAsync(s->tickets, 0, s->tickets.count() * sizeof(uint32_t), s->stream), "zero the tile tickets");
}

void upload_dt(SimPipeline *s, float dt) {
    if (s->dt_valid && memcmp(&dt, &s->dt_enqueued, sizeof dt) == 0) return;
    nb::launch_set_scalar(s->stream, s->dt_dev, dt);
    s->dt_enqueued = dt;
    s->dt_valid = true;
    s->dt_uploads++;
}


void fill_node(hipKernelNodeParams &kp, void **args, const void *fn, dim3 grid, dim3 block, size_t lds_bytes = 0) {
    memset(&kp, 0, sizeof kp);
    kp.func = const_cast<void *>(fn);
    kp.gridDim = grid;
    kp.blockDim = block;
    kp.sharedMemBytes = (unsigned int)lds_bytes;
    kp.kernelParams = args;
    kp.extra = nullptr;
}

StepGraph *find_graph(SimPipeline *s, uint32_t n, uint32_t passes, nb::LaunchShape sh, int phase) {
    for (auto &c : s->graphs)
        if (c.n == n && c.passes == passes && c.phase == phase && c.shape == sh) return &c;
    return nullptr;
}

StepGraph *find_or_build_graph(SimPipeline *s, uint32_t n, float dt, nb::LaunchShape sh) {
    const uint32_t passes = passes_for(s, whole_step(s, s->cur, dt));
    StepGraph *g = find_graph(s, n, passes, sh, s->cur);
    const bool fused = fused_finish_applies(s, sh);
    const uint32_t per_pass = sh.split > 1 && !fused ? 2 : 1;
    const uint32_t per_step = passes * per_pass;
    const bool fresh = g == nullptr;
    if (fresh) {
        evict_for_one_more(s);
        s->graphs.emplace_back();
        g = &s->graphs.back();
        g->n = n;
        g->passes = passes;
        g->shape = sh;
        ASSERT_HIP(hipGraphCreate(&g->graph, 0), "hipGraphCreate");
        g->nodes.resize((size_t)n * per_step);
        g->params.resize((size_t)n * passes);
    }
    g->last_use = ++s->use_clock;
    if (!fresh) return g;
    if (fused) zero_tickets(s);
    hipGraphNode_t prev = nullptr;
    for (uint32_t i = 0; i < n; i++) {
        const std::vector<nb::StepParams> launches = step_passes(s, whole_step(s, (s->cur + i) & 1, dt), sh);
        for (uint32_t q = 0; q < passes; q++) {
            g->params[(size_t)i * passes + q] = launches[q];
            void *args[] = {&g->params[(size_t)i * passes + q]};
            for (uint32_t j = 0; j < per_pass; j++) {
                hipKernelNodeParams kp;
                if (j == 0)
                    fill_node(kp, args, fused ? nb::step_kernel_fused_fn(sh) : nb::step_kernel_fn(sh), nb::step_grid(sh, s->n_real), nb::step_block(sh),
                              nb::step_lds_bytes(sh, launches[q].src_end[0] - launches[q].src_begin[0]));
                else
                    fill_node(kp, args, nb::finish_kernel_fn(), nb::finish_grid(s->n_real), nb::finish_block());
                hipGraphNode_t &node = g->nodes[(size_t)i * per_step + q * per_pass + j];
                ASSERT_HIP(hipGraphAddKernelNode(&node, g->graph, prev ? &prev : nullptr, prev ? 1 : 0, &kp),
                           "hipGraphAddKernelNode step %u/%u", i, n);
                prev = node;
            }
        }
    }
    ASSERT_HIP(hipGraphInstantiate(&g->exec, g->graph, nullptr, nullptr, 0), "hipGraphInstantiate (%u steps)", n);
    g->phase = s->cur;
    return g;
}

constexpr double CANON_MAX_PAIRS = 6.0e7;

constexpr double CHAIN_MAX_PAIRS = 3.6e4;
constexpr uint32_t CHAIN_AUTO_MAX_RECV = 256;

bool wants_fused_chain(const SimPipeline *s) {
    if (s->sharded || s->fused_chain == 0 || s->n_real == 0 || nb::chain_tiles(s->n_real) == 0) return false;
    if (s->fused_chain == 1) return true;
    return nb::shape_on_auto(s->want) && s->want_passes == 0 && s->n_real <= CHAIN_AUTO_MAX_RECV &&
           (double)s->n_real * (double)(s->n_src ? s->n_src : 1) <= CHAIN_MAX_PAIRS;
}

void enqueue_fused(SimPipeline *s, uint32_t n) {
    nb::ChainParams p;
    memset(&p, 0, sizeof p);
    p.pos = s->pos[s->cur];
    p.vel = s->vel;
    p.acc = s->acc;
    p.radius = s->radius;
    p.src_gm = s->src_gm;
    p.n_recv = s->n_real;
    p.n_src = s->n_src;
    p.tiles = nb::chain_tiles(s->n_real);
    p.dt = s->dt_dev;
    for (uint32_t left = n; left > 0;) {
        p.steps = left > CHAIN_MAX_STEPS_PER_LAUNCH ? CHAIN_MAX_STEPS_PER_LAUNCH : left;
        nb::launch_chain(s->stream, p);
        left -= p.steps;
    }
    s->fused_steps = n;
    s->last_shape = {.k = 2, .w = (int)(16u / p.tiles), .variant = nb::VARIANT_LDS, .split = 1, .unit = 8, .lanes = 1};
    s->last_groups = 1;
}

bool wants_canonical(const SimPipeline *s) {
    if (s->fused_chain == 2 && wants_fused_chain(s)) return false;
    return !s->sharded && s->use_graph == 2 && s->n_real > 0 &&
           (double)s->n_real * (double)(s->n_src ? s->n_src : 1) <= CANON_MAX_PAIRS;
}

void enqueue_single(SimPipeline *s, uint32_t n, float dt) {
    if (n >= 2 && wants_fused_chain(s)) {
        enqueue_fused(s, n);
        return;
    }
    const nb::LaunchShape sh = resolve_shape(s);
    if (!s->use_graph || n == 1 || (s->use_graph == 2 && n < GRAPH_AUTO_MIN_CHAIN)) {
        for (uint32_t i = 0; i < n; i++) {
            launch_step(s, sh, whole_step(s, s->cur, dt), s->stream);
            s->cur ^= 1;
        }
        return;
    }
    uint32_t left = n;
    if (wants_canonical(s)) {
        if (s->cur == 1 && left > 0) {
            launch_step(s, sh, whole_step(s, s->cur, dt), s->stream);
            s->cur ^= 1;
            left--;
        }
        while (left >= CANON_STEPS) {
            StepGraph *g = find_or_build_graph(s, CANON_STEPS, dt, sh);
            ASSERT_HIP(hipGraphLaunch(g->exec, s->stream), "hipGraphLaunch (canonical %u steps)", CANON_STEPS);
            left -= CANON_STEPS;
        }
        for (; left > 0; left--) {
            launch_step(s, sh, whole_step(s, s->cur, dt), s->stream);
            s->cur ^= 1;
        }
        return;
    }
    while (left > 0) {
        const uint32_t chunk = left > GRAPH_CHAIN_MAX ? GRAPH_CHAIN_MAX : left;
        if (s->use_graph == 2 && !find_graph(s, chunk, passes_for(s, whole_step(s, s->cur, dt)), sh, s->cur)) {
            bool seen = false;
            for (uint32_t c : s->seen_chains) seen = seen || c == chunk;
            if (!seen) {
                if (s->seen_chains.size() >= 64) s->seen_chains.clear();
                s->seen_chains.push_back(chunk);
                for (uint32_t i = 0; i < chunk; i++) {
                    launch_step(s, sh, whole_step(s, s->cur, dt), s->stream);
                    s->cur ^= 1;
                }
                left -= chunk;
                continue;
            }
        }
        StepGraph *g = find_or_build_graph(s, chunk, dt, sh);
        ASSERT_HIP(hipGraphLaunch(g->exec, s->stream), "hipGraphLaunch (%u steps)", chunk);
        if (chunk & 1) s->cur ^= 1;
        left -= chunk;
    }
}


void begin_call(SimPipeline *s) {
    s->pool.used = 0;
    s->kernel_iv.clear();
    s->comm_iv.clear();
    s->detail_steps = 0;
    s->fused_steps = 0;
    s->host_current = false;
}

void end_call(SimPipeline *s, uint32_t launches) {
    if (s->timing)
        s->step_iv.end(s->stream);
    else
        s->step_iv.clear();
    s->timed_launches = launches;
    s->timed_finish_launches = s->last_shape.split > 1 && !fused_finish_applies(s, s->last_shape) ? s->timed_launches : 0;
}

void enqueue_steps(SimPipeline *s, uint32_t n, float dt) {
    NB_ASSERT(s->on_device, "PerformSimUpdate before SetSimulationData");
    if (s->slots == 0 || n == 0) return;
    use_device();
    begin_call(s);
    s->acc_current = false;
    upload_dt(s, dt);
    if (s->timing) s->step_iv.begin(s->stream);
    if (!s->sharded)
        enqueue_single(s, n, dt);
    else
        enqueue_sharded(s, n, dt);
    uint32_t launches = (s->sharded && s->overlap) ? 2 * n : n * passes_for(s, whole_step(s, s->cur, dt));
    if (s->fused_steps) launches = (n + CHAIN_MAX_STEPS_PER_LAUNCH - 1) / CHAIN_MAX_STEPS_PER_LAUNCH;
    end_call(s, launches);
    s->data.dt = dt;
}

}
```

Measured before the change: 5650 billion.

## Add dealt step kernel that draws tile work items from an atomic ticket counter

New measurement: 5719 billion, median of 6. 1.01x the previous value.

```diff
diff --git a/nbody_amd/__init__.py b/nbody_amd/__init__.py
--- a/nbody_amd/__init__.py
+++ b/nbody_amd/__init__.py
@@ -205,6 +205,10 @@
     "nb_hip_launch_lanes": (C.c_int, [C.c_void_p]),
     "nb_hip_plan_launch_unit": (C.c_int, [C.c_uint32, C.c_uint32, C.c_int]),
     "nb_hip_plan_fused_finish": (C.c_int, [C.c_uint32, C.c_uint32, C.c_int]),
+    "nb_hip_last_deal": (C.c_int, [C.c_void_p, C.POINTER(C.c_uint32), C.POINTER(C.c_uint32)]),
+    "nb_hip_plan_deal": (C.c_int, [C.c_uint32, C.c_uint32, C.c_int]),
+    "nb_hip_deal_item": (C.c_int, [C.c_uint32, C.c_uint32, C.c_uint32, C.POINTER(C.c_uint32), C.POINTER(C.c_uint32)]),
+    "nb_hip_deal_counter": (C.c_uint32, [C.c_void_p]),
     "nb_hip_plan_launch_lanes": (C.c_int, [C.c_uint32, C.c_uint32, C.POINTER(C.c_int)]),
     "nb_hip_last_diag_ms": (C.c_double, [C.c_void_p]),
     "nb_hip_last_render_ms": (C.c_double, [C.c_void_p, C.POINTER(C.c_double)]),
@@ -402,6 +406,16 @@
             "fused_finish": int(hip_lib().nb_hip_plan_fused_finish(n_recv, n_src, compute_units))}
 
 
+def plan_deal(n_recv, n_src, compute_units=256):
+    return bool(hip_lib().nb_hip_plan_deal(n_recv, n_src, compute_units))
+
+
+def deal_item(ticket, tiles, split):
+    tile, part = C.c_uint32(0), C.c_uint32(0)
+    live = hip_lib().nb_hip_deal_item(ticket, tiles, split, C.byref(tile), C.byref(part))
+    return (int(tile.value), int(part.value)) if live else None
+
+
 def comm_unique_id():
     buf = (C.c_ubyte * UNIQUE_ID_BYTES)()
     hip_lib().nb_hip_comm_unique_id(buf)
@@ -587,6 +601,14 @@
     def fused_steps(self):
         return int(hip_lib().nb_hip_last_fused_steps(self._h))
 
+    def last_deal(self):
+        items, extra = C.c_uint32(0), C.c_uint32(0)
+        dealt = hip_lib().nb_hip_last_deal(self._h, C.byref(items), C.byref(extra))
+        return bool(dealt), int(items.value), int(extra.value)
+
+    def deal_counter(self):
+        return int(hip_lib().nb_hip_deal_counter(self._h))
+
     def configure(self, **knobs):
         for k, v in knobs.items():
             fn = hip_lib().nb_hip_configure if k in PUBLIC_KNOBS else hip_lib().nb_hip_tune
diff --git a/nbody_amd/csrc/kernels.h b/nbody_amd/csrc/kernels.h
--- a/nbody_amd/csrc/kernels.h
+++ b/nbody_amd/csrc/kernels.h
@@ -36,7 +36,18 @@
     uint32_t split;
     uint32_t *tickets;
     uint32_t unit;
+    uint32_t *deal;
+    uint32_t deal_items;
 };
+
+struct DealItem {
+    uint32_t tile, part;
+    bool live;
+};
+__host__ __device__ inline DealItem deal_item(uint32_t ticket, uint32_t tiles, uint32_t split) {
+    if (tiles == 0 || ticket / tiles >= split) return DealItem{0, 0, false};
+    return DealItem{ticket % tiles, ticket / tiles, true};
+}
 
 __host__ __device__ inline StepParams plain_step(const float2 *src_pos, const float *src_gm, uint32_t n_src, const float2 *pos_in,
                                                  float2 *pos_out, float2 *vel, float2 *acc, const float *radius, uint32_t n_recv,
@@ -96,6 +107,7 @@
 
 const void *step_kernel_fn(LaunchShape s);
 const void *step_kernel_fused_fn(LaunchShape s);
+const void *dealt_kernel_fn(LaunchShape s);
 const void *finish_kernel_fn();
 
 void launch_chain(hipStream_t st, const ChainParams &p);
diff --git a/nbody_amd/csrc/kernels.hip b/nbody_amd/csrc/kernels.hip
--- a/nbody_amd/csrc/kernels.hip
+++ b/nbody_amd/csrc/kernels.hip
@@ -86,9 +86,10 @@
 NB_INTERACT8_OVERRIDE
 #endif
 
-template <typename V>
+template <typename V, bool CONSTANT = false>
 __device__ __forceinline__ V src_load(const float *ptr) {
-    return *reinterpret_cast<const V *>(ptr);
+    if constexpr (CONSTANT) return *(const __attribute__((address_space(4))) V *)(ptr);
+    else return *reinterpret_cast<const V *>(ptr);
 }
 
 __device__ __forceinline__ uint32_t receiver_slot(const StepParams &p, uint32_t i) {
@@ -187,174 +188,28 @@
 
 template <int K, int W, int VARIANT, bool FUSED = false>
 __global__ __launch_bounds__(WAVE *W, 8) void step_kernel(const StepParams p) {
-    const uint32_t tid = threadIdx.x;
-    const uint32_t lane = tid & (WAVE - 1);
-    const uint32_t wid = __builtin_amdgcn_readfirstlane(tid >> 6);
+    constexpr bool SRC_CONSTANT = false;
     const uint32_t tile_x = blockIdx.x, part_y = blockIdx.y;
-
-    __shared__ __attribute__((aligned(16))) float tile[VARIANT == VARIANT_LDS ? W : 1][2][3 * CHUNK];
-    __shared__ float2 partial[W > 1 ? W : 1][W > 1 ? WAVE * K : 1];
-
-    const float dt = *p.dt;
-
-    const uint32_t recv_base = tile_x * (WAVE * K);
-    Receivers<K> R;
-#pragma unroll
-    for (int k = 0; k < K; k++) {
-        uint32_t i = recv_base + k * WAVE + lane;
-        i = i < p.n_recv ? i : p.n_recv - 1;
-        i = receiver_slot(p, i);
-        const float2 q = p.pos_in[i];
-        R.p[k] = f2v{q.x, q.y};
-        R.r[k] = p.radius[i];
-    }
-    R.clear();
-
-    const uint32_t n0 = p.src_end[0] - p.src_begin[0];
-    const uint32_t n1 = p.src_end[1] - p.src_begin[1];
-    const uint32_t total = n0 + n1;
-    const SourceSlice wave_src = source_slice(total, p.unit, p.split, part_y, W, wid);
-    const uint32_t v_lo = wave_src.lo;
-    const uint32_t v_hi = wave_src.hi;
-
-    if constexpr (VARIANT == VARIANT_LDS) {
-        float(*T)[3 * CHUNK] = tile[wid];
-        float2 sp = make_float2(0.f, 0.f);
-        float sg = 0.f;
-        auto fetch = [&](uint32_t c) {
-            const uint32_t v = c * CHUNK + lane;
-            const bool live = v < total;
-            const uint32_t j = source_index(p, live ? v : total - 1, n0);
-            sp = p.src_pos[j];
-            sg = live ? p.src_gm[j] : 0.0f;
-        };
-        const uint32_t c_lo = v_lo / CHUNK, c_hi = (v_hi + CHUNK - 1) / CHUNK;
-        if (c_lo < c_hi) fetch(c_lo);
-        int buf = 0;
-        for (uint32_t c = c_lo; c < c_hi; c++) {
-            *reinterpret_cast<float2 *>(&T[buf][2 * lane]) = sp;
-            T[buf][2 * CHUNK + lane] = sg;
-            if (c + 1 < c_hi) fetch(c + 1);
-            __builtin_amdgcn_fence(__ATOMIC_RELEASE, "wavefront");
-            __builtin_amdgcn_wave_barrier();
-            __builtin_amdgcn_fence(__ATOMIC_ACQUIRE, "wavefront");
-            for (int jj = 0; jj < CHUNK; jj += 4) {
-                const v8f P = *reinterpret_cast<const v8f *>(&T[buf][2 * jj]);
-                const v4f G = *reinterpret_cast<const v4f *>(&T[buf][2 * CHUNK + jj]);
-#pragma unroll
-                for (int u = 0; u < 4; u++) interact<K, false>(R, f2v{P[2 * u], P[2 * u + 1]}, G[u]);
-            }
-            if (((c - c_lo) & (CLOSE_EVERY - 1)) == CLOSE_EVERY - 1) R.close_chunk();
-            buf ^= 1;
-        }
-        if ((c_hi - c_lo) & (CLOSE_EVERY - 1)) R.close_chunk();
-    } else {
-#pragma unroll
-        for (int range = 0; range < 2; range++) {
-            const uint32_t r_lo = range == 0 ? 0u : n0;
-            const uint32_t r_hi = range == 0 ? n0 : total;
-            const uint32_t a = max(v_lo, r_lo), b = min(v_hi, r_hi);
-            if (a >= b) continue;
-            uint32_t j = p.src_begin[range] + (a - r_lo);
-            const uint32_t j_end = p.src_begin[range] + (b - r_lo);
-            const float *sp = reinterpret_cast<const float *>(p.src_pos), *sg = p.src_gm;
-            const uint32_t groups = (j_end - j) / 8;
-            const uint32_t g0 = (a - v_lo) / 8;
-            if (groups > 0) {
-                const uint32_t j_last = j + (groups - 1) * 8;
-                v16f PA = src_load<v16f>(sp + 2 * (size_t)j);
-                v8f GA = src_load<v8f>(sg + j);
-                uint32_t g = 0;
-                while (g + 2 <= groups) {
-                    const uint32_t to_close = (8u * CLOSE_EVERY - ((g0 + g) & (8u * CLOSE_EVERY - 1))) / 2;
-                    const uint32_t pairs = min(to_close, (groups - g) / 2);
-                    for (uint32_t i = 0; i < pairs; i++) {
-                        asm("" : "+s"(j) : "s"(PA), "s"(GA));
-                        const v16f PB = src_load<v16f>(sp + 2 * (size_t)(j + 8));
-                        const v8f GB = src_load<v8f>(sg + j + 8);
-                        __builtin_amdgcn_sched_barrier(0);
-                        interact8<K, true>(R, PA, GA);
-                        __builtin_amdgcn_sched_barrier(0);
-                        j = min(j + 16, j_last);
-                        asm("" : "+s"(j) : "s"(PB), "s"(GB));
-                        PA = src_load<v16f>(sp + 2 * (size_t)j);
-                        GA = src_load<v8f>(sg + j);
-                        __builtin_amdgcn_sched_barrier(0);
-                        interact8<K, true>(R, PB, GB);
-                    }
-                    g += 2 * pairs;
-                    if (pairs == to_close) R.close_chunk();
-                }
-                if (g < groups) interact8<K, true>(R, PA, GA);
-                j = j_last + 8;
-            }
-            for (; j < j_end; j++) interact<K, true>(R, f2v{sp[2 * (size_t)j], sp[2 * (size_t)j + 1]}, sg[j]);
-        }
-        if ((v_hi - v_lo) & (CHUNK * CLOSE_EVERY - 1)) R.close_chunk();
-    }
-
-    auto finish = [&](uint32_t logical, float sx, float sy) {
-        if (p.split > 1) {
-            if (logical < p.n_recv) {
-                float2 *slot = &p.parts[(size_t)part_y * p.n_recv + logical];
-                if constexpr (FUSED) {
-                    const uint64_t bits = (uint64_t)__float_as_uint(sx) | ((uint64_t)__float_as_uint(sy) << 32);
-                    __hip_atomic_store(reinterpret_cast<uint64_t *>(slot), bits, __ATOMIC_RELAXED, __HIP_MEMORY_SCOPE_AGENT);
-                } else {
-                    *slot = make_float2(sx, sy);
-                }
-            }
-        } else {
-            finish_receiver(p, logical, sx, sy, dt);
-        }
-    };
-
-    if constexpr (W == 1) {
-#pragma unroll
-        for (int k = 0; k < K; k++) finish(recv_base + k * WAVE + lane, R.s[k].x, R.s[k].y);
-    } else {
-#pragma unroll
-        for (int k = 0; k < K; k++) partial[wid][k * WAVE + lane] = make_float2(R.s[k].x, R.s[k].y);
-        __syncthreads();
-#pragma unroll
-        for (uint32_t slot = tid; slot < WAVE * K; slot += WAVE * W) {
-            const float2 a = wave_sum(&partial[0][slot], WAVE * K, W);
-            finish(recv_base + slot, a.x, a.y);
-        }
-    }
-
-    if constexpr (FUSED) {
-        if (p.split > 1) {
-            __shared__ uint32_t is_last;
-            asm volatile("s_waitcnt vmcnt(0)" ::: "memory");
-            __syncthreads();
-            if (tid == 0) {
-                const uint32_t t = __hip_atomic_fetch_add(&p.tickets[tile_x], 1u, __ATOMIC_RELAXED, __HIP_MEMORY_SCOPE_AGENT);
-                is_last = t == p.split - 1 ? 1u : 0u;
-                if (is_last) __hip_atomic_store(&p.tickets[tile_x], 0u, __ATOMIC_RELAXED, __HIP_MEMORY_SCOPE_AGENT);
-            }
-            __syncthreads();
-            if (is_last) {
-                for (uint32_t slot = tid; slot < WAVE * K; slot += WAVE * W) {
-                    const uint32_t logical = recv_base + slot;
-                    if (logical >= p.n_recv) continue;
-                    float2 part[MAX_SPLIT];
-#pragma unroll
-                    for (uint32_t s = 0; s < (uint32_t)MAX_SPLIT; s++) {
-                        const uint64_t bits = __hip_atomic_load(reinterpret_cast<const uint64_t *>(&p.parts[(size_t)(s < p.split ? s : p.split - 1) * p.n_recv + logical]),
-                                                                __ATOMIC_RELAXED, __HIP_MEMORY_SCOPE_AGENT);
-                        part[s] = make_float2(__uint_as_float((uint32_t)bits), __uint_as_float((uint32_t)(bits >> 32)));
-                    }
-                    const uint32_t i = receiver_slot(p, logical);
-                    const float2 a0 = p.acc[i], v0 = p.vel[i], q0 = p.pos_in[i];
-                    float sx = 0.0f, sy = 0.0f;
-#pragma unroll
-                    for (uint32_t s = 0; s < (uint32_t)MAX_SPLIT; s++) add_part(sx, sy, part[s], s < p.split);
-                    finish_loaded(p, i, make_float2(sx, sy), a0, v0, q0, dt);
-                }
-            }
-        }
-    }
+#include "step_tile.inc"
+}
+
+template <int K, int W>
+__global__ __launch_bounds__(WAVE *W, 8) void dealt_kernel(const StepParams p) {
+    constexpr int VARIANT = VARIANT_SMEM;
+    constexpr bool FUSED = false;
+    constexpr bool SRC_CONSTANT = true;
+    __shared__ uint32_t drawn;
+    if (threadIdx.x == 0) {
+        const uint32_t t = __hip_atomic_fetch_add(p.deal, 1u, __ATOMIC_RELAXED, __HIP_MEMORY_SCOPE_AGENT);
+        if (t == gridDim.x - 1) __hip_atomic_store(p.deal, 0u, __ATOMIC_RELAXED, __HIP_MEMORY_SCOPE_AGENT);
+        drawn = t;
+    }
+    __syncthreads();
+    const uint32_t ticket = __builtin_amdgcn_readfirstlane(drawn);
+    const DealItem item = deal_item(ticket, p.deal_items / p.split, p.split);
+    if (!item.live) return;
+    const uint32_t tile_x = item.tile, part_y = item.part;
+#include "step_tile.inc"
 }
 
 template <int W, int H>
@@ -724,6 +579,13 @@
     return pick_fused(s.k, s.w);
 }
 
+const void *dealt_kernel_fn(LaunchShape s) {
+    if (s.lanes > 1 || s.variant != VARIANT_SMEM) return nullptr;
+    const int a = s.k, b = s.w;
+    NB_CASE(dealt_kernel, 1, 16) NB_CASE(dealt_kernel, 2, 16)
+    return nullptr;
+}
+
 const void *finish_kernel_fn() { return reinterpret_cast<const void *>(&finish_kernel); }
 
 const void *batch_lane_split_fn(int a, int b, bool listed) {
diff --git a/nbody_amd/csrc/launch_shape.h b/nbody_amd/csrc/launch_shape.h
--- a/nbody_amd/csrc/launch_shape.h
+++ b/nbody_amd/csrc/launch_shape.h
@@ -29,6 +29,11 @@
 
 bool fused_finish_rule(uint32_t n_recv, uint32_t n_src);
 
+uint32_t deal_items(LaunchShape s, uint32_t n_recv);
+uint32_t deal_extra(uint32_t items);
+bool deal_pays(uint32_t items, int compute_units);
+bool deal_rule(uint32_t n_recv, uint32_t n_src, int compute_units);
+
 dim3 step_grid(LaunchShape s, uint32_t n_recv);
 dim3 step_block(LaunchShape s);
 size_t step_lds_bytes(LaunchShape s, uint32_t n_src);
diff --git a/nbody_amd/csrc/launch_shape.hip b/nbody_amd/csrc/launch_shape.hip
--- a/nbody_amd/csrc/launch_shape.hip
+++ b/nbody_amd/csrc/launch_shape.hip
@@ -154,4 +154,25 @@
     return (double)n_recv * (double)n_src >= FUSED_FINISH_MIN_PAIRS && n_recv <= FUSED_FINISH_MAX_RECV;
 }
 
+uint32_t deal_items(LaunchShape s, uint32_t n_recv) {
+    const dim3 g = step_grid(s, n_recv);
+    return g.x * g.y;
 }
+
+uint32_t deal_extra(uint32_t items) { return items / 32 > 8 ? items / 32 : 8; }
+
+constexpr uint32_t DEAL_MIN_ROUNDS = 32;
+
+bool deal_pays(uint32_t items, int compute_units) {
+    if (compute_units <= 0) compute_units = 256;
+    return (uint64_t)items >= (uint64_t)DEAL_MIN_ROUNDS * 2u * (uint64_t)compute_units;
+}
+
+bool deal_rule(uint32_t n_recv, uint32_t n_src, int compute_units) {
+    const LaunchShape sh = choose_shape({.lanes = 1}, n_recv, n_src, compute_units);
+    if (dealt_kernel_fn(sh) == nullptr) return false;
+    if (sh.split > 1 && fused_finish_rule(n_recv, n_src)) return false;
+    return deal_pays(deal_items(sh, n_recv), compute_units);
+}
+
+}
diff --git a/nbody_amd/csrc/nbody_hip_tuning.h b/nbody_amd/csrc/nbody_hip_tuning.h
--- a/nbody_amd/csrc/nbody_hip_tuning.h
+++ b/nbody_amd/csrc/nbody_hip_tuning.h
@@ -19,6 +19,11 @@
 int nb_hip_plan_launch_lanes(uint32_t n_recv, uint32_t n_src, int *w);
 int nb_hip_plan_fused_finish(uint32_t n_recv, uint32_t n_src, int compute_units);
 int nb_hip_plan_launch_unit(uint32_t n_recv, uint32_t n_src, int compute_units);
+
+int nb_hip_last_deal(const SimPipeline *sim, uint32_t *items, uint32_t *extra);
+int nb_hip_plan_deal(uint32_t n_recv, uint32_t n_src, int compute_units);
+int nb_hip_deal_item(uint32_t ticket, uint32_t tiles, uint32_t split, uint32_t *tile, uint32_t *part);
+uint32_t nb_hip_deal_counter(SimPipeline *sim);
 
 double nb_hip_last_diag_ms(SimPipeline *sim);
 
diff --git a/nbody_amd/csrc/pipeline.hip b/nbody_amd/csrc/pipeline.hip
--- a/nbody_amd/csrc/pipeline.hip
+++ b/nbody_amd/csrc/pipeline.hip
@@ -78,6 +78,7 @@
     s->mass.alloc(cap);
     s->src_gm.alloc(s->n_src);
     s->dt_dev.alloc(1);
+    if (!s->sharded && N > 0) s->deal_counter.alloc(1);
     s->aos.alloc(N);
     if (!s->sharded) {
         s->src_pos[0] = s->pos[0];
@@ -153,6 +154,7 @@
     struct { const char *env, *key; } presets[] = {
         {"NB_HIP_K", "k"}, {"NB_HIP_W", "w"}, {"NB_HIP_SPLIT", "split"}, {"NB_HIP_UNIT", "unit"}, {"NB_HIP_PASSES", "passes"},
         {"NB_HIP_LANES", "lanes"}, {"NB_HIP_FUSED_CHAIN", "fused_chain"}, {"NB_HIP_FUSED_FINISH", "fused_finish"},
+        {"NB_HIP_DEAL", "deal"}, {"NB_HIP_DEAL_EXTRA", "deal_extra"},
         {"NB_HIP_READBACK", "readback"}, {"NB_HIP_ZERO_COPY_UPLOAD", "zero_copy_upload"},
     };
     for (const auto &p : presets)
@@ -224,6 +226,17 @@
     return sh.split > 1 && nb_hip_plan_launch_lanes(n_recv, n_src, nullptr) <= 1 && nb::fused_finish_rule(n_recv, n_src) ? 1 : 0;
 }
 
+int nb_hip_plan_deal(uint32_t n_recv, uint32_t n_src, int compute_units) {
+    return nb_hip_plan_launch_lanes(n_recv, n_src, nullptr) <= 1 && nb::deal_rule(n_recv, n_src, compute_units) ? 1 : 0;
+}
+
+int nb_hip_deal_item(uint32_t ticket, uint32_t tiles, uint32_t split, uint32_t *tile, uint32_t *part) {
+    const nb::DealItem it = nb::deal_item(ticket, tiles, split);
+    if (it.live && tile) *tile = it.tile;
+    if (it.live && part) *part = it.part;
+    return it.live ? 1 : 0;
+}
+
 int nb_hip_plan_launch_unit(uint32_t n_recv, uint32_t n_src, int compute_units) {
     return nb::choose_shape({.lanes = 1}, n_recv, n_src, compute_units).unit;
 }
@@ -434,6 +447,23 @@
 uint32_t nb_hip_last_fused_steps(const SimPipeline *s) {
     NB_ASSERT(s != nullptr, "NULL pipeline");
     return s->fused_steps;
+}
+
+int nb_hip_last_deal(const SimPipeline *s, uint32_t *items, uint32_t *extra) {
+    NB_ASSERT(s != nullptr, "NULL pipeline");
+    if (items) *items = s->last_deal_items;
+    if (extra) *extra = s->last_deal_extra;
+    return s->last_deal_items && !s->fused_steps ? 1 : 0;
+}
+
+uint32_t nb_hip_deal_counter(SimPipeline *s) {
+    NB_ASSERT(s != nullptr, "NULL pipeline");
+    if (!s->on_device || !s->deal_counter) return 0;
+    use_device();
+    uint32_t v = 0;
+    ASSERT_HIP(hipStreamSynchronize(s->stream), "sync before reading the deal counter");
+    ASSERT_HIP(hipMemcpy(&v, s->deal_counter, sizeof v, hipMemcpyDeviceToHost), "read the deal counter");
+    return v;
 }
 
 int nb_hip_launch_lanes(const SimPipeline *s) {
@@ -530,6 +560,14 @@
             s->graphs.clear();
         }
         s->fused_finish = value;
+    } else if (!strcmp(key, "deal")) {
+        NB_ASSERT(value >= 0 && value <= 2, "deal must be 0 (never), 1 (whenever the shape allows) or 2 (auto), got %d", value);
+        old = s->deal;
+        s->deal = value;
+    } else if (!strcmp(key, "deal_extra")) {
+        NB_ASSERT(value >= 0 && value <= (1 << 20), "deal_extra must be 0 (auto) .. 2^20 workgroups, got %d", value);
+        old = s->want_deal_extra;
+        s->want_deal_extra = value;
     } else if (!strcmp(key, "passes")) {
         NB_ASSERT(value >= 0 && value <= 64, "passes must be 0 (auto) .. 64, got %d", value);
         old = s->want_passes;
diff --git a/nbody_amd/csrc/pipeline_internal.h b/nbody_amd/csrc/pipeline_internal.h
--- a/nbody_amd/csrc/pipeline_internal.h
+++ b/nbody_amd/csrc/pipeline_internal.h
@@ -225,6 +225,7 @@
     std::vector<nb::StepParams> params;
     int phase = -1;
     nb::LaunchShape shape;
+    uint32_t dealt_groups = 0;
     uint64_t last_use = 0;
 };
 
@@ -288,6 +289,10 @@
     nbi::DevBuf<float2> parts;
     nbi::DevBuf<uint32_t> tickets;
     int fused_finish = 2;
+    nbi::DevBuf<uint32_t> deal_counter;
+    int deal = 2;
+    int want_deal_extra = 0;
+    uint32_t last_deal_items = 0, last_deal_extra = 0;
     int cur = 0;
 
     hipStream_t stream = nullptr;
@@ -362,6 +367,7 @@
 void launch_step(SimPipeline *s, nb::LaunchShape sh, const nb::StepParams &p, hipStream_t st);
 void upload_dt(SimPipeline *s, float dt);
 void zero_tickets(SimPipeline *s);
+bool deal_applies(const SimPipeline *s, nb::LaunchShape sh);
 void begin_call(SimPipeline *s);
 void end_call(SimPipeline *s, uint32_t launches);
 void enqueue_steps(SimPipeline *s, uint32_t n, float dt);
diff --git a/nbody_amd/csrc/step_chain.hip b/nbody_amd/csrc/step_chain.hip
--- a/nbody_amd/csrc/step_chain.hip
+++ b/nbody_amd/csrc/step_chain.hip
@@ -24,6 +24,8 @@
     g.nodes.clear();
     g.params.clear();
 }
+
+uint32_t dealt_extra(const SimPipeline *s, uint32_t items);
 
 nb::LaunchShape resolve_shape(SimPipeline *s) {
     nb::LaunchShape want = s->want;
@@ -45,6 +47,8 @@
     }
     s->last_shape = sh;
     s->last_groups = nb::step_grid(sh, s->n_real).x * nb::step_grid(sh, s->n_real).y;
+    s->last_deal_items = deal_applies(s, sh) ? nb::deal_items(sh, s->n_real) : 0u;
+    s->last_deal_extra = s->last_deal_items ? dealt_extra(s, s->last_deal_items) : 0u;
     return sh;
 }
 
@@ -67,10 +71,33 @@
     return s->fused_finish == 1 || nb::fused_finish_rule(s->n_real, s->n_src);
 }
 
+bool deal_applies(const SimPipeline *s, nb::LaunchShape sh) {
+    if (s->deal == 0 || s->sharded || !s->deal_counter || s->n_real == 0) return false;
+    if (sh.variant != nb::VARIANT_SMEM || sh.lanes > 1 || sh.w != 16 || (sh.k != 1 && sh.k != 2)) return false;
+    if (nb::dealt_kernel_fn(sh) == nullptr || fused_finish_applies(s, sh)) return false;
+    return s->deal == 1 || nb::deal_pays(nb::deal_items(sh, s->n_real), g_dev.compute_units);
+}
+
+uint32_t dealt_extra(const SimPipeline *s, uint32_t items) { return s->want_deal_extra > 0 ? (uint32_t)s->want_deal_extra : nb::deal_extra(items); }
+
+dim3 launch_grid(const SimPipeline *s, nb::LaunchShape sh, bool dealt) {
+    if (!dealt) return nb::step_grid(sh, s->n_real);
+    const uint32_t items = nb::deal_items(sh, s->n_real);
+    return dim3(items + dealt_extra(s, items));
+}
+
+const void *launch_fn(nb::LaunchShape sh, bool fused, bool dealt) {
+    return dealt ? nb::dealt_kernel_fn(sh) : fused ? nb::step_kernel_fused_fn(sh) : nb::step_kernel_fn(sh);
+}
+
 nb::StepParams shaped(const SimPipeline *s, nb::StepParams p, nb::LaunchShape sh) {
     p.split = sh.split > 1 ? (uint32_t)sh.split : 1u;
     p.parts = p.split > 1 ? s->parts : nullptr;
     p.tickets = s->tickets;
+    if (deal_applies(s, sh)) {
+        p.deal = s->deal_counter;
+        p.deal_items = nb::deal_items(sh, s->n_real);
+    }
     p.unit = (sh.unit >= 8 && sh.unit <= 64 && p.src_end[1] == p.src_begin[1]) ? (uint32_t)sh.unit : 64u;
     return p;
 }
@@ -106,13 +133,13 @@
 
 void launch_step(SimPipeline *s, nb::LaunchShape sh, const nb::StepParams &p, hipStream_t st) {
     if (s->n_real == 0) return;
-    const bool fused = fused_finish_applies(s, sh);
+    const bool fused = fused_finish_applies(s, sh), dealt = deal_applies(s, sh);
     for (nb::StepParams &copy : step_passes(s, p, sh)) {
         void *args[] = {&copy};
-        ASSERT_HIP(hipLaunchKernel(fused ? nb::step_kernel_fused_fn(sh) : nb::step_kernel_fn(sh), nb::step_grid(sh, s->n_real), nb::step_block(sh), args,
+        ASSERT_HIP(hipLaunchKernel(launch_fn(sh, fused, dealt), launch_grid(s, sh, dealt), nb::step_block(sh), args,
                                    nb::step_lds_bytes(sh, copy.src_end[0] - copy.src_begin[0]), st),
-                   "step kernel launch (k=%d w=%d variant=%d split=%d, %u receivers)", sh.k, sh.w, sh.variant, sh.split,
-                   s->n_real);
+                   "step kernel launch (k=%d w=%d variant=%d split=%d dealt=%d, %u receivers)", sh.k, sh.w, sh.variant, sh.split,
+                   (int)dealt, s->n_real);
         if (copy.split > 1 && !fused)
             ASSERT_HIP(hipLaunchKernel(nb::finish_kernel_fn(), nb::finish_grid(s->n_real), nb::finish_block(), args, 0, st),
                        "finish kernel launch (%u receivers, %u parts)", s->n_real, copy.split);
@@ -121,6 +148,7 @@
 
 void zero_tickets(SimPipeline *s) {
     if (s->tickets) ASSERT_HIP(hipMemsetAsync(s->tickets, 0, s->tickets.count() * sizeof(uint32_t), s->stream), "zero the tile tickets");
+    if (s->deal_counter) ASSERT_HIP(hipMemsetAsync(s->deal_counter, 0, sizeof(uint32_t), s->stream), "zero the deal counter");
 }
 
 void upload_dt(SimPipeline *s, float dt) {
@@ -143,15 +171,16 @@
 }
 
 StepGraph *find_graph(SimPipeline *s, uint32_t n, uint32_t passes, nb::LaunchShape sh, int phase) {
+    const uint32_t dealt_groups = deal_applies(s, sh) ? launch_grid(s, sh, true).x : 0u;
     for (auto &c : s->graphs)
-        if (c.n == n && c.passes == passes && c.phase == phase && c.shape == sh) return &c;
+        if (c.n == n && c.passes == passes && c.phase == phase && c.shape == sh && c.dealt_groups == dealt_groups) return &c;
     return nullptr;
 }
 
 StepGraph *find_or_build_graph(SimPipeline *s, uint32_t n, float dt, nb::LaunchShape sh) {
     const uint32_t passes = passes_for(s, whole_step(s, s->cur, dt));
     StepGraph *g = find_graph(s, n, passes, sh, s->cur);
-    const bool fused = fused_finish_applies(s, sh);
+    const bool fused = fused_finish_applies(s, sh), dealt = deal_applies(s, sh);
     const uint32_t per_pass = sh.split > 1 && !fused ? 2 : 1;
     const uint32_t per_step = passes * per_pass;
     const bool fresh = g == nullptr;
@@ -162,13 +191,14 @@
         g->n = n;
         g->passes = passes;
         g->shape = sh;
+        g->dealt_groups = dealt ? launch_grid(s, sh, true).x : 0u;
         ASSERT_HIP(hipGraphCreate(&g->graph, 0), "hipGraphCreate");
         g->nodes.resize((size_t)n * per_step);
         g->params.resize((size_t)n * passes);
     }
     g->last_use = ++s->use_clock;
     if (!fresh) return g;
-    if (fused) zero_tickets(s);
+    if (fused || dealt) zero_tickets(s);
     hipGraphNode_t prev = nullptr;
     for (uint32_t i = 0; i < n; i++) {
         const std::vector<nb::StepParams> launches = step_passes(s, whole_step(s, (s->cur + i) & 1, dt), sh);
@@ -178,7 +208,7 @@
             for (uint32_t j = 0; j < per_pass; j++) {
                 hipKernelNodeParams kp;
                 if (j == 0)
-                    fill_node(kp, args, fused ? nb::step_kernel_fused_fn(sh) : nb::step_kernel_fn(sh), nb::step_grid(sh, s->n_real), nb::step_block(sh),
+                    fill_node(kp, args, launch_fn(sh, fused, dealt), launch_grid(s, sh, dealt), nb::step_block(sh),
                               nb::step_lds_bytes(sh, launches[q].src_end[0] - launches[q].src_begin[0]));
                 else
                     fill_node(kp, args, nb::finish_kernel_fn(), nb::finish_grid(s->n_real), nb::finish_block());
diff --git a/nbody_amd/csrc/step_tile.inc b/nbody_amd/csrc/step_tile.inc
--- /dev/null
+++ b/nbody_amd/csrc/step_tile.inc
@@ -0,0 +1,167 @@
+    const uint32_t tid = threadIdx.x;
+    const uint32_t lane = tid & (WAVE - 1);
+    const uint32_t wid = __builtin_amdgcn_readfirstlane(tid >> 6);
+
+    __shared__ __attribute__((aligned(16))) float tile[VARIANT == VARIANT_LDS ? W : 1][2][3 * CHUNK];
+    __shared__ float2 partial[W > 1 ? W : 1][W > 1 ? WAVE * K : 1];
+
+    const float dt = *p.dt;
+
+    const uint32_t recv_base = tile_x * (WAVE * K);
+    Receivers<K> R;
+#pragma unroll
+    for (int k = 0; k < K; k++) {
+        uint32_t i = recv_base + k * WAVE + lane;
+        i = i < p.n_recv ? i : p.n_recv - 1;
+        i = receiver_slot(p, i);
+        const float2 q = p.pos_in[i];
+        R.p[k] = f2v{q.x, q.y};
+        R.r[k] = p.radius[i];
+    }
+    R.clear();
+
+    const uint32_t n0 = p.src_end[0] - p.src_begin[0];
+    const uint32_t n1 = p.src_end[1] - p.src_begin[1];
+    const uint32_t total = n0 + n1;
+    const SourceSlice wave_src = source_slice(total, p.unit, p.split, part_y, W, wid);
+    const uint32_t v_lo = wave_src.lo;
+    const uint32_t v_hi = wave_src.hi;
+
+    if constexpr (VARIANT == VARIANT_LDS) {
+        float(*T)[3 * CHUNK] = tile[wid];
+        float2 sp = make_float2(0.f, 0.f);
+        float sg = 0.f;
+        auto fetch = [&](uint32_t c) {
+            const uint32_t v = c * CHUNK + lane;
+            const bool live = v < total;
+            const uint32_t j = source_index(p, live ? v : total - 1, n0);
+            sp = p.src_pos[j];
+            sg = live ? p.src_gm[j] : 0.0f;
+        };
+        const uint32_t c_lo = v_lo / CHUNK, c_hi = (v_hi + CHUNK - 1) / CHUNK;
+        if (c_lo < c_hi) fetch(c_lo);
+        int buf = 0;
+        for (uint32_t c = c_lo; c < c_hi; c++) {
+            *reinterpret_cast<float2 *>(&T[buf][2 * lane]) = sp;
+            T[buf][2 * CHUNK + lane] = sg;
+            if (c + 1 < c_hi) fetch(c + 1);
+            __builtin_amdgcn_fence(__ATOMIC_RELEASE, "wavefront");
+            __builtin_amdgcn_wave_barrier();
+            __builtin_amdgcn_fence(__ATOMIC_ACQUIRE, "wavefront");
+            for (int jj = 0; jj < CHUNK; jj += 4) {
+                const v8f P = *reinterpret_cast<const v8f *>(&T[buf][2 * jj]);
+                const v4f G = *reinterpret_cast<const v4f *>(&T[buf][2 * CHUNK + jj]);
+#pragma unroll
+                for (int u = 0; u < 4; u++) interact<K, false>(R, f2v{P[2 * u], P[2 * u + 1]}, G[u]);
+            }
+            if (((c - c_lo) & (CLOSE_EVERY - 1)) == CLOSE_EVERY - 1) R.close_chunk();
+            buf ^= 1;
+        }
+        if ((c_hi - c_lo) & (CLOSE_EVERY - 1)) R.close_chunk();
+    } else {
+#pragma unroll
+        for (int range = 0; range < 2; range++) {
+            const uint32_t r_lo = range == 0 ? 0u : n0;
+            const uint32_t r_hi = range == 0 ? n0 : total;
+            const uint32_t a = max(v_lo, r_lo), b = min(v_hi, r_hi);
+            if (a >= b) continue;
+            uint32_t j = p.src_begin[range] + (a - r_lo);
+            const uint32_t j_end = p.src_begin[range] + (b - r_lo);
+            const float *sp = reinterpret_cast<const float *>(p.src_pos), *sg = p.src_gm;
+            const uint32_t groups = (j_end - j) / 8;
+            const uint32_t g0 = (a - v_lo) / 8;
+            if (groups > 0) {
+                const uint32_t j_last = j + (groups - 1) * 8;
+                v16f PA = src_load<v16f, SRC_CONSTANT>(sp + 2 * (size_t)j);
+                v8f GA = src_load<v8f, SRC_CONSTANT>(sg + j);
+                uint32_t g = 0;
+                while (g + 2 <= groups) {
+                    const uint32_t to_close = (8u * CLOSE_EVERY - ((g0 + g) & (8u * CLOSE_EVERY - 1))) / 2;
+                    const uint32_t pairs = min(to_close, (groups - g) / 2);
+                    for (uint32_t i = 0; i < pairs; i++) {
+                        asm("" : "+s"(j) : "s"(PA), "s"(GA));
+                        const v16f PB = src_load<v16f, SRC_CONSTANT>(sp + 2 * (size_t)(j + 8));
+                        const v8f GB = src_load<v8f, SRC_CONSTANT>(sg + j + 8);
+                        __builtin_amdgcn_sched_barrier(0);
+                        interact8<K, true>(R, PA, GA);
+                        __builtin_amdgcn_sched_barrier(0);
+                        j = min(j + 16, j_last);
+                        asm("" : "+s"(j) : "s"(PB), "s"(GB));
+                        PA = src_load<v16f, SRC_CONSTANT>(sp + 2 * (size_t)j);
+                        GA = src_load<v8f, SRC_CONSTANT>(sg + j);
+                        __builtin_amdgcn_sched_barrier(0);
+                        interact8<K, true>(R, PB, GB);
+                    }
+                    g += 2 * pairs;
+                    if (pairs == to_close) R.close_chunk();
+                }
+                if (g < groups) interact8<K, true>(R, PA, GA);
+                j = j_last + 8;
+            }
+            for (; j < j_end; j++) interact<K, true>(R, f2v{sp[2 * (size_t)j], sp[2 * (size_t)j + 1]}, sg[j]);
+        }
+        if ((v_hi - v_lo) & (CHUNK * CLOSE_EVERY - 1)) R.close_chunk();
+    }
+
+    auto finish = [&](uint32_t logical, float sx, float sy) {
+        if (p.split > 1) {
+            if (logical < p.n_recv) {
+                float2 *slot = &p.parts[(size_t)part_y * p.n_recv + logical];
+                if constexpr (FUSED) {
+                    const uint64_t bits = (uint64_t)__float_as_uint(sx) | ((uint64_t)__float_as_uint(sy) << 32);
+                    __hip_atomic_store(reinterpret_cast<uint64_t *>(slot), bits, __ATOMIC_RELAXED, __HIP_MEMORY_SCOPE_AGENT);
+                } else {
+                    *slot = make_float2(sx, sy);
+                }
+            }
+        } else {
+            finish_receiver(p, logical, sx, sy, dt);
+        }
+    };
+
+    if constexpr (W == 1) {
+#pragma unroll
+        for (int k = 0; k < K; k++) finish(recv_base + k * WAVE + lane, R.s[k].x, R.s[k].y);
+    } else {
+#pragma unroll
+        for (int k = 0; k < K; k++) partial[wid][k * WAVE + lane] = make_float2(R.s[k].x, R.s[k].y);
+        __syncthreads();
+#pragma unroll
+        for (uint32_t slot = tid; slot < WAVE * K; slot += WAVE * W) {
+            const float2 a = wave_sum(&partial[0][slot], WAVE * K, W);
+            finish(recv_base + slot, a.x, a.y);
+        }
+    }
+
+    if constexpr (FUSED) {
+        if (p.split > 1) {
+            __shared__ uint32_t is_last;
+            asm volatile("s_waitcnt vmcnt(0)" ::: "memory");
+            __syncthreads();
+            if (tid == 0) {
+                const uint32_t t = __hip_atomic_fetch_add(&p.tickets[tile_x], 1u, __ATOMIC_RELAXED, __HIP_MEMORY_SCOPE_AGENT);
+                is_last = t == p.split - 1 ? 1u : 0u;
+                if (is_last) __hip_atomic_store(&p.tickets[tile_x], 0u, __ATOMIC_RELAXED, __HIP_MEMORY_SCOPE_AGENT);
+            }
+            __syncthreads();
+            if (is_last) {
+                for (uint32_t slot = tid; slot < WAVE * K; slot += WAVE * W) {
+                    const uint32_t logical = recv_base + slot;
+                    if (logical >= p.n_recv) continue;
+                    float2 part[MAX_SPLIT];
+#pragma unroll
+                    for (uint32_t s = 0; s < (uint32_t)MAX_SPLIT; s++) {
+                        const uint64_t bits = __hip_atomic_load(reinterpret_cast<const uint64_t *>(&p.parts[(size_t)(s < p.split ? s : p.split - 1) * p.n_recv + logical]),
+                                                                __ATOMIC_RELAXED, __HIP_MEMORY_SCOPE_AGENT);
+                        part[s] = make_float2(__uint_as_float((uint32_t)bits), __uint_as_float((uint32_t)(bits >> 32)));
+                    }
+                    const uint32_t i = receiver_slot(p, logical);
+                    const float2 a0 = p.acc[i], v0 = p.vel[i], q0 = p.pos_in[i];
+                    float sx = 0.0f, sy = 0.0f;
+#pragma unroll
+                    for (uint32_t s = 0; s < (uint32_t)MAX_SPLIT; s++) add_part(sx, sy, part[s], s < p.split);
+                    finish_loaded(p, i, make_float2(sx, sy), a0, v0, q0, dt);
+                }
+            }
+        }
+    }
```
